# OChicken/GPQHE

Hardware: AMD Instinct MI355X
Metric: ciphertext he_mul/sec (RNS core: tensor 30 limbs + key-switch 45 limbs), N=2^16 (higher is better)
Workload: dtype u64; 1 GPU; he_mul RNS core, n=2^16, dimA=30, dimB=45, batch=64 ciphertexts per GPU (BASELINE configs[2]); he_rescale has no RNS-domain work in the reference; batch_per_gpu=64, total_batch=64, chunk=32, parallelism=ciphertext-per-GPU x1, no data-path collective, launcher=single process

## Files before the change

gpqhe_amd/_native.py:

```python
import ctypes as C
import os

_HERE = os.path.dirname(os.path.abspath(__file__))
LIB_PATH = os.path.join(_HERE, "libgpqhe_hip.so")


def use_variant(path):
    global LIB_PATH
    if _lib is not None:
        raise RuntimeError("use_variant(%r): the library is already loaded" % path)
    if not os.path.exists(path):
        raise FileNotFoundError(path)
    LIB_PATH = os.path.abspath(path)


u64 = C.c_uint64
vp = C.c_void_p

SIGNATURES = {
    "gpq_ctx_create": (C.c_int, [C.POINTER(vp), C.c_uint, C.c_uint, C.c_int]),
    "gpq_ctx_create_from_tables": (C.c_int, [C.POINTER(vp), C.c_uint, C.c_uint, C.POINTER(u64),
                                             C.POINTER(C.POINTER(u64)), C.POINTER(C.POINTER(u64)), C.c_int]),
    "gpq_ctx_destroy": (None, [vp]),
    "gpq_ctx_logn": (C.c_uint, [vp]),
    "gpq_ctx_nprimes": (C.c_uint, [vp]),
    "gpq_ctx_device": (C.c_int, [vp]),
    "gpq_ctx_const": (u64, [vp, C.c_uint, C.c_int]),
    "gpq_ctx_zetas": (C.POINTER(u64), [vp, C.c_uint, C.c_int]),
    "gpq_dimub": (C.c_uint, [C.c_uint, C.c_uint]),
    "gpq_last_error": (C.c_char_p, []),
    "gpq_malloc": (C.c_int, [C.POINTER(vp), C.c_size_t]),
    "gpq_free": (C.c_int, [vp]),
    "gpq_upload": (C.c_int, [vp, vp, C.c_size_t, vp]),
    "gpq_download": (C.c_int, [vp, vp, C.c_size_t, vp]),
    "gpq_copy": (C.c_int, [vp, vp, C.c_size_t, vp]),
    "gpq_stream_sync": (C.c_int, [vp]),
    "gpq_stream_wait": (C.c_int, [vp, vp]),
    "gpq_device_count": (C.c_int, []),
    "gpq_bind_thread_to_device": (C.c_int, [C.c_int]),
    "gpq_device_local_cpus": (C.c_int, [C.c_int, C.c_char_p, C.c_char_p, C.c_size_t]),
    "gpq_probe_stream": (C.c_int, [vp, vp, C.c_size_t, C.c_int, C.c_uint, C.c_uint, C.c_uint, vp]),
    "gpq_set_device": (C.c_int, [C.c_int]),
    "gpq_stream_create": (C.c_int, [C.POINTER(vp)]),
    "gpq_stream_destroy": (C.c_int, [vp]),
    "gpq_malloc_host": (C.c_int, [C.POINTER(vp), C.c_size_t]),
    "gpq_free_host": (C.c_int, [vp]),
    "gpq_ntt": (C.c_int, [vp, vp, C.c_uint, C.c_uint, vp]),
    "gpq_invntt": (C.c_int, [vp, vp, C.c_uint, C.c_uint, vp]),
    "gpq_ntt_reference": (C.c_int, [vp, vp, C.c_uint, C.c_uint, C.c_int, vp]),
    "gpq_rns_mul": (C.c_int, [vp, vp, vp, vp, C.c_uint, C.c_uint, vp]),
    "gpq_rns_add": (C.c_int, [vp, vp, vp, vp, C.c_uint, C.c_uint, vp]),
    "gpq_poly_mul_rns": (C.c_int, [vp, vp, vp, vp, C.c_uint, C.c_uint, vp]),
    "gpq_mulpt_rns": (C.c_int, [vp] * 6 + [C.c_uint, C.c_uint, vp]),
    "gpq_set_chunk": (C.c_int, [vp, C.c_uint]),
    "gpq_set_limb_block": (C.c_int, [vp, C.c_uint]),
    "gpq_set_limb_classes": (C.c_int, [vp, C.c_uint, C.c_uint]),
    "gpq_tensor_workspace_bytes": (C.c_size_t, [vp, C.c_uint, C.c_uint]),
    "gpq_keyswitch_workspace_bytes": (C.c_size_t, [vp, C.c_uint, C.c_uint]),
    "gpq_he_mul_tensor": (C.c_int, [vp] * 8 + [C.c_uint, C.c_uint, vp, vp]),
    "gpq_keyswitch": (C.c_int, [vp] * 6 + [C.c_uint, C.c_uint, vp, vp]),
    "gpq_big_words": (C.c_uint, [C.c_uint]),
    "gpq_ctx_phat_invmp": (u64, [vp, C.c_uint, C.c_uint]),
    "gpq_ctx_pbits": (C.c_uint, [vp, C.c_uint]),
    "gpq_rns_decompose": (C.c_int, [vp, vp, vp, C.c_uint, C.c_uint, C.c_uint, vp]),
    "gpq_rns_decompose_limbs": (C.c_int, [vp, vp, vp, C.c_uint, C.c_uint, C.c_uint, C.c_uint, vp]),
    "gpq_rns_reconstruct": (C.c_int, [vp, vp, C.c_uint, vp, C.c_uint, C.c_uint, C.c_uint, vp]),
    "gpq_rns_reconstruct_one": (C.c_int, [vp, C.POINTER(u64), C.c_uint, C.POINTER(u64), C.c_uint]),
    "gpq_set_exact_crt": (C.c_int, [vp, C.c_int]),
    "gpq_set_stream_bridge": (C.c_int, [vp, C.c_int]),
    "gpq_debug_force_redo": (C.c_int, [vp, C.c_uint]),
    "gpq_debug_zero_watch": (C.c_int, [vp, C.c_int]),
    "gpq_debug_zero_flags": (C.c_long, [vp, vp, vp, C.c_size_t]),
    "gpq_set_lazy_decompose": (C.c_int, [vp, C.c_int]),
    "gpq_set_nt_policy": (C.c_int, [vp, C.c_int]),
    "gpq_set_overlap": (C.c_int, [vp, C.c_int]),
    "gpq_last_lanes": (C.c_uint, [vp]),
    "gpq_debug_fail_peer": (C.c_int, [vp, C.c_int]),
    "gpq_debug_table_bytes": (C.c_size_t, [vp, C.c_int]),
    "gpq_set_fused_tail": (C.c_int, [vp, C.c_int]),
    "gpq_big_transpose": (C.c_int, [vp, vp, vp, C.c_uint, C.c_uint, C.c_int, vp]),
    "gpq_big_addsub": (C.c_int, [vp, vp, vp, vp, C.c_uint, C.c_uint, C.c_int, vp]),
    "gpq_set_prescale": (C.c_int, [vp, C.c_int]),
    "gpq_set_bridge_mfma": (C.c_int, [vp, C.c_int]),
    "gpq_poly_mul_workspace_bytes": (C.c_size_t, [vp, C.c_uint, C.c_uint]),
    "gpq_poly_mul": (C.c_int, [vp, vp, vp, vp, C.c_uint, C.c_uint, C.c_uint, C.c_uint, vp, vp]),
    "gpq_poly_mul_general_workspace_bytes": (C.c_size_t, [vp, C.c_uint, C.c_uint]),
    "gpq_rns_reconstruct_general": (C.c_int, [vp, vp, C.c_uint, vp, C.c_uint, C.c_uint, C.POINTER(u64), C.c_uint, vp, vp]),
    "gpq_poly_mul_general": (C.c_int, [vp, vp, vp, vp, C.c_uint, C.c_uint, C.POINTER(u64), C.c_uint, C.c_uint, vp, vp]),
    "gpq_he_rs": (C.c_int, [vp, vp, vp, C.c_uint, C.c_uint, C.c_uint, C.c_uint, vp]),
    "gpq_he_rescale": (C.c_int, [vp, vp, vp, C.c_uint, C.c_uint, C.c_uint, C.c_uint, vp]),
    "gpq_he_dims": (C.c_int, [vp, C.c_uint, C.c_uint] + [C.POINTER(C.c_uint)] * 4),
    "gpq_he_mul_workspace_bytes": (C.c_size_t, [vp, C.c_uint, C.c_uint, C.c_uint, C.c_uint, C.c_uint]),
    "gpq_he_mul": (C.c_int, [vp] * 9 + [C.c_uint] * 6 + [vp, vp]),
    "gpq_he_mul_rs": (C.c_int, [vp] * 9 + [C.c_uint] * 7 + [vp, vp]),
    "gpq_relin_tail_workspace_bytes": (C.c_size_t, [vp, C.c_uint, C.c_uint, C.c_uint, C.c_uint]),
    "gpq_relin_tail": (C.c_int, [vp, vp, vp, vp, C.c_uint, C.c_uint, C.c_uint, C.c_uint, C.c_uint, vp, vp]),
    "gpq_relin_tail_overwriting": (C.c_int, [vp, vp, vp, vp, C.c_uint, C.c_uint, C.c_uint, C.c_uint, C.c_uint, vp, vp]),
    "gpq_he_mulpt_workspace_bytes": (C.c_size_t, [vp, C.c_uint, C.c_uint]),
    "gpq_he_mulpt": (C.c_int, [vp] * 6 + [C.c_uint] * 4 + [vp, vp]),
    "gpq_poly_rot": (C.c_int, [vp, vp, vp, C.c_uint, C.c_uint, C.c_uint, vp]),
    "gpq_poly_conj": (C.c_int, [vp, vp, vp, C.c_uint, C.c_uint, vp]),
    "gpq_he_general_workspace_bytes": (C.c_size_t, [vp, C.c_uint, C.c_uint, C.c_uint, C.c_uint, C.c_uint]),
    "gpq_he_rs_general": (C.c_int, [vp, vp, vp, C.c_uint, C.c_ulonglong, C.POINTER(u64), C.c_uint, C.c_uint, vp, vp]),
    "gpq_relin_tail_general": (C.c_int, [vp, vp, vp, vp, C.c_uint, C.POINTER(u64), C.c_uint, C.c_uint, C.c_uint, C.c_uint, vp, vp]),
    "gpq_he_mul_general": (C.c_int, [vp] * 9 + [C.c_uint, C.POINTER(u64), C.c_uint, C.c_uint, C.c_uint, C.c_uint, C.c_uint, vp, vp]),
    "gpq_he_mulpt_general": (C.c_int, [vp] * 6 + [C.c_uint, C.POINTER(u64), C.c_uint, C.c_uint, C.c_uint, vp, vp]),
    "gpq_he_swk_general": (C.c_int, [vp] * 7 + [C.c_uint, C.POINTER(u64), C.c_uint, C.c_uint, C.c_uint, C.c_uint, vp, vp]),
    "gpq_big_add": (C.c_int, [vp, vp, vp, vp, C.c_uint, C.c_uint, C.c_uint, vp]),
    "gpq_big_sub": (C.c_int, [vp, vp, vp, vp, C.c_uint, C.c_uint, C.c_uint, vp]),
    "gpq_big_neg": (C.c_int, [vp, vp, vp, C.c_uint, C.c_uint, C.c_uint, vp]),
    "gpq_evk_pack": (C.c_int, [vp, vp, vp, C.c_uint, C.c_uint, C.c_uint, vp]),
    "gpq_he_genswk_workspace_bytes": (C.c_size_t, [vp, C.c_uint, C.c_uint, C.c_uint]),
    "gpq_he_genswk": (C.c_int, [vp] * 7 + [C.c_uint] * 4 + [vp, vp]),
    "gpq_he_swk_workspace_bytes": (C.c_size_t, [vp, C.c_uint, C.c_uint, C.c_uint, C.c_uint]),
    "gpq_he_swk": (C.c_int, [vp] * 7 + [C.c_uint] * 5 + [vp, vp]),
    "gpq_automorphism_index": (C.c_int, [C.c_uint, u64, vp]),
    "gpq_he_rot_hoisted_workspace_bytes": (C.c_size_t, [vp] + [C.c_uint] * 5),
    "gpq_he_rot_hoisted": (C.c_int, [vp] * 8 + [C.c_uint] * 6 + [vp, vp]),
    "gpq_he_gemv_workspace_bytes": (C.c_size_t, [vp] + [C.c_uint] * 6),
    "gpq_he_gemv": (C.c_int, [vp] * 8 + [C.c_uint] * 8 + [vp, vp]),
    "gpq_gemv_acc_dim": (C.c_uint, [C.c_uint] * 4),
    "gpq_gemv_plan_create": (C.c_int, [vp, C.POINTER(vp), vp, C.c_uint, C.c_uint, C.c_uint, C.c_uint, vp]),
    "gpq_gemv_plan_destroy": (None, [vp]),
    "gpq_gemv_plan_info": (C.c_int, [vp, C.POINTER(C.c_uint), C.POINTER(C.c_size_t), C.POINTER(C.c_uint), C.POINTER(C.c_int)]),
    "gpq_gemv_plan_rotations": (C.c_int, [vp, vp]),
    "gpq_shim_gemv_plan_cache": (None, [C.c_uint]),
    "gpq_gemv_inner_workspace_bytes": (C.c_size_t, [vp, vp, C.c_uint]),
    "gpq_gemv_inner": (C.c_int, [vp] * 6 + [C.c_uint] * 3 + [vp, vp]),
    "gpq_he_gemv_planned_workspace_bytes": (C.c_size_t, [vp, vp] + [C.c_uint] * 4),
    "gpq_he_gemv_planned": (C.c_int, [vp] * 8 + [C.c_uint] * 5 + [vp, vp]),
    "gpq_profile_enable": (C.c_int, [vp, C.c_int]),
    "gpq_profile_kernels": (C.c_int, []),
    "gpq_profile_kernel_name": (C.c_char_p, [C.c_int]),
    "gpq_profile_collect": (C.c_int, [vp, C.POINTER(C.c_double), C.POINTER(C.c_ulonglong)]),
    "gpq_timer_create": (C.c_int, [C.POINTER(vp)]),
    "gpq_timer_start": (C.c_int, [vp, vp]),
    "gpq_timer_stop": (C.c_int, [vp, vp]),
    "gpq_timer_elapsed_ms": (C.c_int, [vp, C.POINTER(C.c_float)]),
    "gpq_timer_destroy": (None, [vp]),
    "ntt": (None, [vp, vp]),
    "invntt": (None, [vp, vp]),
    "poly_ntt": (None, [vp, vp]),
    "poly_invntt": (None, [vp, vp]),
    "poly_rns_add": (None, [vp, vp, vp, vp]),
    "poly_rns_mul": (None, [vp, vp, vp, vp]),
    "montgomery_inv": (u64, [u64]),
    "barrett_inv": (u64, [u64]),
    "gpq_dropin_set_logn": (None, [C.c_uint]),
    "gpq_dropin_reset": (None, []),
    "gpq_mpi_shim_release": (None, []),
    "gpq_mpi_shim_forget_keys": (None, []),
    "gpq_mpi_shim_set_key_slots": (None, [C.c_uint]),
    "gpq_mpi_shim_set_key_check": (None, [C.c_int]),
    "gpq_mpi_shim_engine": (C.c_void_p, []),
    "gpq_compat_view": (C.c_void_p, [C.c_char_p]),
    "gpq_mpi_shim_resident_keys": (C.c_uint, []),
    "gpq_mpi_shim_set_poly_slots": (None, [C.c_uint]),
    "gpq_mpi_shim_resident_polys": (C.c_uint, []),
    "gpq_mpi_shim_poly_stats": (None, [C.POINTER(C.c_uint64), C.POINTER(C.c_uint64)]),
    "gpq_mpi_shim_forget_polys": (None, []),
    "gpq_mpi_shim_set_conversion_threads": (C.c_uint, [C.c_uint]),
    "gpq_mpi_shim_poly_bypass": (None, [C.c_int]),
    "gpq_mpi_shim_set_direct_mpi": (C.c_int, [C.c_int]),
    "gpq_mpi_shim_last_timing": (None, [C.POINTER(C.c_double)]),
    "gpq_fill_rns_chain": (C.c_int, [vp, C.c_uint, vp, C.c_int]),
    "gpq_release_rns_chain": (None, [vp]),
}
EXPORTED_ONLY = ["montgomery_reduce", "barrett_reduce",
                 "rns_decompose", "rns_reconstruct", "poly_rns2mpi", "poly_mul", "he_mul", "he_rs", "he_rescale", "he_moddown", "he_mulpt", "he_add", "he_sub", "he_addpt", "he_subpt", "he_neg", "he_copy_ct", "he_dec", "he_conj", "he_rot", "he_genrlk", "he_genck", "he_genrk",
                 "he_gemv", "he_sum", "he_idx",
                 ]
CTX_LIB_PATH = os.path.join(os.path.dirname(os.path.abspath(__file__)), "libgpqhe_hip_ctx.so")
CTX_EXPORTS = ["polyctx_init", "polyctx_exit", "hectx_init", "hectx_exit", "poly_mpi_alloc", "poly_mpi_free", "poly_rns_alloc", "poly_rns_free",
               "polyctx", "hectx", "GPQHE_TWO"]

_lib = None


def load():
    global _lib
    if _lib is not None:
        return _lib
    if not os.path.exists(LIB_PATH):
        raise ImportError(
            "gpqhe_amd: %s is missing -- build it with `make -C gpqhe_amd/csrc` "
            "(or __graft_entry__.build()); there is no CPU fallback" % LIB_PATH)
    try:
        import torch
    except ImportError:
        pass
    lib = C.CDLL(LIB_PATH)
    for name, (res, args) in SIGNATURES.items():
        fn = getattr(lib, name)
        fn.restype = res
        fn.argtypes = args
    for name in EXPORTED_ONLY:
        getattr(lib, name)
    _lib = lib
    return lib


class GpqError(RuntimeError):
    pass


def check(rc, what):
    if rc != 0:
        raise GpqError("%s failed (%d): %s" % (what, rc, load().gpq_last_error().decode()))
```

gpqhe_amd/csrc/bridge.hip:

```cpp
#include "../../include/gpqhe_hip.h"
#include "engine_internal.hpp"
#include "bridge_kernels.hpp"
#include "bridge_mfma.hpp"
#include "bridge_stream.hpp"

#include <algorithm>
#include <cstdlib>
#include <cstring>
#include <memory>
#include <new>

using namespace gpq;

#define HIP_TRY(expr)                                                                      \
  do {                                                                                     \
    hipError_t e_ = (expr);                                                                \
    if (e_ != hipSuccess) return gpq_fail(GPQ_ERR_HIP, "%s: %s", #expr, hipGetErrorString(e_)); \
  } while (0)

namespace {

typedef unsigned __int128 u128h;
typedef std::vector<uint64_t> Big;

struct LdsRaised {
  bool dev[64] = {};
  int raise(const void *fn, int bytes) {
    int d = 0;
    HIP_TRY(hipGetDevice(&d));
    if (d < 0 || d >= 64 || !dev[d]) {
      HIP_TRY(hipFuncSetAttribute(fn, hipFuncAttributeMaxDynamicSharedMemorySize, bytes));
      if (d >= 0 && d < 64) dev[d] = true;
    }
    return GPQ_OK;
  }
};


void mul_small(Big &a, uint64_t m) {
  uint64_t carry = 0;
  for (auto &w : a) { u128h t = (u128h)w * m + carry; w = (uint64_t)t; carry = (uint64_t)(t >> 64); }
  if (carry) a.push_back(carry);
}
uint64_t divmod_small(Big &a, uint64_t m) {
  uint64_t rem = 0;
  for (size_t i = a.size(); i-- > 0;) { u128h t = ((u128h)rem << 64) | a[i]; a[i] = (uint64_t)(t / m); rem = (uint64_t)(t % m); }
  while (a.size() > 1 && a.back() == 0) a.pop_back();
  return rem;
}
uint64_t mod_small(const Big &a, uint64_t m) { Big t = a; return divmod_small(t, m); }
void shr1(Big &a) {
  for (size_t i = 0; i < a.size(); ++i) a[i] = (a[i] >> 1) | (i + 1 < a.size() ? a[i + 1] << 63 : 0);
}
uint64_t powm(uint64_t b, uint64_t e, uint64_t m) {
  uint64_t r = 1;
  while (e) { if (e & 1) r = (uint64_t)((u128h)r * b % m); b = (uint64_t)((u128h)b * b % m); e >>= 1; }
  return r;
}
void put(std::vector<uint64_t> &dst, size_t off, const Big &v, size_t words) {
  for (size_t j = 0; j < words; ++j) dst[off + j] = j < v.size() ? v[j] : 0;
}

const int kWP[] = {8, 16, 32, 48, 56};

int cmp_big(const Big &a, const Big &b) {
  size_t na = a.size(), nb = b.size();
  while (na > 1 && a[na - 1] == 0) --na;
  while (nb > 1 && b[nb - 1] == 0) --nb;
  if (na != nb) return na < nb ? -1 : 1;
  for (size_t i = na; i-- > 0;) if (a[i] != b[i]) return a[i] < b[i] ? -1 : 1;
  return 0;
}
void sub_big(Big &a, const Big &b) {
  uint64_t bor = 0;
  for (size_t i = 0; i < a.size(); ++i) {
    const u128h d = (u128h)a[i] - (i < b.size() ? b[i] : 0) - bor;
    a[i] = (uint64_t)d; bor = (uint64_t)(d >> 64) & 1;
  }
}
Big floor_pow2_div(unsigned bits, const Big &m) {
  Big q((bits + 64) / 64, 0), rem(m.size() + 1, 0);
  for (int b = (int)bits; b >= 0; --b) {
    uint64_t c = b == (int)bits ? 1 : 0;
    for (size_t i = 0; i < rem.size(); ++i) { const uint64_t n = rem[i] >> 63; rem[i] = (rem[i] << 1) | c; c = n; }
    if (cmp_big(rem, m) >= 0) { sub_big(rem, m); q[b >> 6] |= 1ull << (b & 63); }
  }
  return q;
}

int get_basis(gpq_ctx *c, unsigned first, unsigned dim, gpq_bridge_basis **out) {
  const auto key = std::make_pair(first, dim);
  auto it = c->cache->bases.find(key);
  if (it != c->cache->bases.end()) { *out = &it->second; return GPQ_OK; }
  if (dim < 1 || first + dim > c->nprimes || dim > 63)
    return gpq_fail(GPQ_ERR_INVALID, "bridge: limbs %u..%u outside the chain of %u (at most 63 per basis)", first, first + dim, c->nprimes);
  Big P{1};
  for (unsigned d = 0; d < dim; ++d) mul_small(P, c->p[first + d]);
  int WP = 0;
  for (int w : kWP) if ((size_t)w >= P.size()) { WP = w; break; }
  if (!WP) return gpq_fail(GPQ_ERR_UNSUPPORTED, "bridge: P of %u limbs needs %zu words", dim, P.size());
  gpq_bridge_basis b;
  b.first = first; b.dim = dim; b.WP = WP; b.pbits = 64 * (unsigned)(P.size() - 1) + (64 - __builtin_clzll(P.back()));
  std::vector<uint64_t> phat((size_t)dim * WP), pinv(dim), pmult((size_t)6 * (WP + 1)), phalf(WP + 1);
  for (unsigned d = 0; d < dim; ++d) {
    const uint64_t pd = c->p[first + d];
    Big q = P;
    divmod_small(q, pd);
    put(phat, (size_t)d * WP, q, WP);
    pinv[d] = powm(mod_small(q, pd), pd - 2, pd);
  }
  Big h = P; shr1(h);
  put(phalf, 0, h, WP + 1);
  Big m = P;
  for (int k = 5; k >= 0; --k) { put(pmult, (size_t)k * (WP + 1), m, WP + 1); mul_small(m, 2); }
  DeviceScope on_device(c->device);
  HIP_TRY(gpq_table_malloc(c, (void **)&b.d_phat, phat.size() * 8));
  HIP_TRY(gpq_table_malloc(c, (void **)&b.d_phat_inv, pinv.size() * 8));
  HIP_TRY(gpq_table_malloc(c, (void **)&b.d_pmult, pmult.size() * 8));
  HIP_TRY(gpq_table_malloc(c, (void **)&b.d_phalf, phalf.size() * 8));
  HIP_TRY(hipMemcpy(b.d_phat, phat.data(), phat.size() * 8, hipMemcpyHostToDevice));
  HIP_TRY(hipMemcpy(b.d_phat_inv, pinv.data(), pinv.size() * 8, hipMemcpyHostToDevice));
  HIP_TRY(hipMemcpy(b.d_pmult, pmult.data(), pmult.size() * 8, hipMemcpyHostToDevice));
  HIP_TRY(hipMemcpy(b.d_phalf, phalf.data(), phalf.size() * 8, hipMemcpyHostToDevice));
  std::vector<uint64_t> inv128(2 * (size_t)dim);
  for (unsigned d = 0; d < dim; ++d) {
    const u128h q = ~(u128h)0 / c->p[first + d];
    inv128[2 * d] = (uint64_t)q; inv128[2 * d + 1] = (uint64_t)(q >> 64);
  }
  HIP_TRY(gpq_table_malloc(c, (void **)&b.d_inv128, inv128.size() * 8));
  HIP_TRY(hipMemcpy(b.d_inv128, inv128.data(), inv128.size() * 8, hipMemcpyHostToDevice));
  b.h_phat_inv = pinv;
  b.h_P = P;
  b.h_phat = phat;
  *out = &(c->cache->bases[key] = b);
  return GPQ_OK;
}

int get_relin(gpq_ctx *c, unsigned dimP, unsigned dimB, gpq_relin_tables **out) {
  const auto key = std::make_pair(dimP, dimB);
  auto it = c->cache->relins.find(key);
  if (it != c->cache->relins.end()) { *out = &it->second; return GPQ_OK; }
  gpq_bridge_basis *bp;
  int rc = get_basis(c, 0, dimP, &bp);
  if (rc) return rc;
  std::vector<uint64_t> pinv(dimB - dimP);
  for (unsigned d = dimP; d < dimB; ++d) pinv[d - dimP] = powm(mod_small(bp->h_P, c->p[d]), c->p[d] - 2, c->p[d]);
  gpq_relin_tables t;
  HIP_TRY(gpq_table_malloc(c, (void **)&t.d_pinv, pinv.size() * 8));
  HIP_TRY(hipMemcpy(t.d_pinv, pinv.data(), pinv.size() * 8, hipMemcpyHostToDevice));
  *out = &(c->cache->relins[key] = t);
  return GPQ_OK;
}

int get_scaled_tabs(gpq_ctx *c, gpq_bridge_basis *b, const LimbTab **out) {
  if (!b->d_tabs_scaled) {
    std::vector<LimbTab> t = c->h_tabs;
    auto pair_of = [](uint64_t w, uint64_t p) { return TwS{p - w, p - (uint64_t)(((u128h)w << 31) % p)}; };
    for (unsigned d = 0; d < b->dim; ++d) {
      LimbTab &e = t[b->first + d];
      const uint64_t p = e.k.p, s = b->h_phat_inv[d];
      e.ninv = (uint64_t)((u128h)e.ninv * s % p);
      e.winv1_ninv = (uint64_t)((u128h)e.winv1_ninv * s % p);
      if (b->first + d < c->nsplit_tables) { e.ninv_s = pair_of(e.ninv, p); e.winv1_ninv_s = pair_of(e.winv1_ninv, p); }
    }
    DeviceScope on_device(c->device);
    HIP_TRY(gpq_table_malloc(c, (void **)&b->d_tabs_scaled, t.size() * sizeof(LimbTab)));
    HIP_TRY(hipMemcpy(b->d_tabs_scaled, t.data(), t.size() * sizeof(LimbTab), hipMemcpyHostToDevice));
  }
  *out = b->d_tabs_scaled;
  return GPQ_OK;
}
struct ScaledInverse {
  gpq_ctx *c;
  ScaledInverse(gpq_ctx *ctx, const LimbTab *tabs) : c(ctx) { c->inv_tabs_override = tabs; }
  ~ScaledInverse() { c->inv_tabs_override = nullptr; }
};
inline bool can_prescale(const gpq_ctx *c) { return c->prescale && c->logn > 12 && !c->h_tabs.empty(); }

inline dim3 masked_grid(const FlagScope &sc, unsigned threads, unsigned n, unsigned polys) {
  if (sc.wave_any) return dim3((sc.waves + threads / 64 - 1) / (threads / 64));
  return dim3((n + threads - 1) / threads, polys);
}
template <int WP>
void launch_exact(const ReconstructArgs &a, unsigned n, unsigned batch, hipStream_t s) {
  hipLaunchKernelGGL((bridge_reconstruct<WP>), masked_grid(a.scope, 128, n, batch), dim3(128), 0, s, a);
}
template <int WL>
void launch_low(const ReconstructArgs &a, unsigned WPstride, unsigned char *redo, unsigned n, unsigned batch, hipStream_t s) {
  hipLaunchKernelGGL((bridge_reconstruct_low<WL>), dim3((n + 255) / 256, batch), dim3(256), 0, s, a, WPstride, redo);
}

void balanced_digits(const uint64_t *words, size_t nwords, int8_t *out, size_t nd) {
  unsigned carry = 0;
  for (size_t i = 0; i < nd; ++i) {
    const unsigned byte = i / 8 < nwords ? (unsigned)((words[i / 8] >> (8 * (i % 8))) & 0xff) : 0;
    const unsigned t = byte + carry;
    if (t >= 128) { out[i] = (int8_t)((int)t - 256); carry = 1; } else { out[i] = (int8_t)t; carry = 0; }
  }
}

int build_recon_mfma(gpq_ctx *c, const std::vector<uint64_t> &primes, const std::vector<uint64_t> &weight_inv, const std::vector<Big> &weight,
                     const Big &Pw, int WL, gpq_recon_mfma *tp, unsigned KSpad = 0, unsigned fcol0 = 0) {
  gpq_recon_mfma &t = *tp;
  const unsigned dim = (unsigned)primes.size(), NT = (8 * WL + 14 + 31) / 32, ncol = 32 * NT;
  t.KS = std::max((dim + 3) / 4, KSpad);
  if (!fcol0) fcol0 = 8u * WL;
  t.lds_bytes = (size_t)t.KS * NT * 1024 + (size_t)t.KS * 64;
  if (t.lds_bytes <= 156 * 1024) {
    std::vector<int8_t> bf((size_t)t.KS * NT * 1024, 0);
    std::vector<uint64_t> lk((size_t)t.KS * 8, 0), kc(WL + 2, 0), pm((size_t)65 * WL, 0);
    std::vector<int8_t> beta(8 * (size_t)WL), phi(8);
    Big sum_phat(WL, 0);
    u128h sum_inv = 0;
    for (unsigned d = 0; d < dim; ++d) {
      const uint64_t pd = primes[d];
      lk[2 * (size_t)d] = pd;
      lk[2 * (size_t)d + 1] = weight_inv[d];
      const Big &ph = weight[d];
      balanced_digits(ph.data(), ph.size() < (size_t)WL ? ph.size() : (size_t)WL, beta.data(), beta.size());
      const uint64_t inv = (uint64_t)((((u128h)1) << 104) / pd);
      balanced_digits(&inv, 1, phi.data(), 8);
      uint64_t cy = 0;
      for (int j = 0; j < WL; ++j) {
        const u128h s2 = (u128h)sum_phat[j] + ((size_t)j < ph.size() ? ph[j] : 0) + cy;
        sum_phat[j] = (uint64_t)s2; cy = (uint64_t)(s2 >> 64);
      }
      sum_inv += inv;
      for (unsigned i = 0; i < 8; ++i) {
        const unsigned k = 8 * d + i, s = k / 32, h = (k % 32) / 16, tt = k % 16;
        for (unsigned col = 0; col < ncol; ++col) {
          int8_t v = 0;
          if (col < 8u * WL) { if (col >= i) v = beta[col - i]; }
          else if (col >= fcol0) { const unsigned m = col - fcol0; if (m >= i && m - i < 8 && m < 14) v = phi[m - i]; }
          if (!v) continue;
          const unsigned nt = col / 32, lane = 32 * h + col % 32;
          bf[(((size_t)s * NT + nt) * 64 + lane) * 16 + tt] = v;
        }
      }
    }
    Big kcS = sum_phat;
    mul_small(kcS, 0x8080808080808080ull);
    for (int j = 0; j < WL; ++j) kc[j] = (size_t)j < kcS.size() ? kcS[j] : 0;
    const u128h lo = (u128h)(uint64_t)sum_inv * 0x8080808080808080ull;
    const u128h hi = (u128h)(uint64_t)(sum_inv >> 64) * 0x8080808080808080ull;
    const u128h kf = lo + (hi << 64);
    kc[WL] = (uint64_t)kf; kc[WL + 1] = (uint64_t)(kf >> 64);
    Big mP{0};
    for (unsigned m = 0; m <= 64; ++m) {
      uint64_t bw = 0;
      for (int j = 0; j < WL; ++j) {
        const u128h d2 = (u128h)((size_t)j < mP.size() ? mP[j] : 0) - kc[j] - bw;
        pm[(size_t)m * WL + j] = (uint64_t)d2; bw = (uint64_t)(d2 >> 64) & 1;
      }
      Big nxt(std::max(mP.size(), Pw.size()) + 1, 0);
      uint64_t cy = 0;
      for (size_t j = 0; j < nxt.size(); ++j) {
        const u128h s2 = (u128h)(j < mP.size() ? mP[j] : 0) + (j < Pw.size() ? Pw[j] : 0) + cy;
        nxt[j] = (uint64_t)s2; cy = (uint64_t)(s2 >> 64);
      }
      mP = nxt;
    }
    DeviceScope on_device(c->device);
    HIP_TRY(gpq_table_malloc(c, (void **)&t.d_bfrag, bf.size()));
    HIP_TRY(gpq_table_malloc(c, (void **)&t.d_lk, lk.size() * 8));
    HIP_TRY(gpq_table_malloc(c, (void **)&t.d_kc, kc.size() * 8));
    HIP_TRY(gpq_table_malloc(c, (void **)&t.d_pm, pm.size() * 8));
    HIP_TRY(hipMemcpy(t.d_bfrag, bf.data(), bf.size(), hipMemcpyHostToDevice));
    HIP_TRY(hipMemcpy(t.d_lk, lk.data(), lk.size() * 8, hipMemcpyHostToDevice));
    HIP_TRY(hipMemcpy(t.d_kc, kc.data(), kc.size() * 8, hipMemcpyHostToDevice));
    HIP_TRY(hipMemcpy(t.d_pm, pm.data(), pm.size() * 8, hipMemcpyHostToDevice));
  }
  return GPQ_OK;
}

int get_recon_mfma(gpq_ctx *c, gpq_bridge_basis *b, int WL, gpq_recon_mfma **out, unsigned KSpad = 0) {
  if (KSpad <= (b->dim + 3) / 4) KSpad = 0;
  const int key = WL + 1000 * (int)KSpad;
  auto it = b->mfma.find(key);
  if (it != b->mfma.end()) { *out = &it->second; return GPQ_OK; }
  gpq_recon_mfma t;
  std::vector<uint64_t> primes(b->dim);
  std::vector<Big> weight(b->dim);
  for (unsigned d = 0; d < b->dim; ++d) {
    primes[d] = c->p[b->first + d];
    weight[d].assign(b->h_phat.begin() + (size_t)d * b->WP, b->h_phat.begin() + (size_t)(d + 1) * b->WP);
  }
  if (int rc = build_recon_mfma(c, primes, b->h_phat_inv, weight, b->h_P, WL, &t, KSpad)) return rc;
  *out = &(b->mfma[key] = t);
  return GPQ_OK;
}

int get_addend_rows(gpq_ctx *c, gpq_bridge_basis *b, unsigned KSpad, gpq_recon_mfma **out) {
  const int key = 100016 + 1000 * (int)KSpad;
  auto it = b->mfma.find(key);
  if (it != b->mfma.end()) { *out = &it->second; return GPQ_OK; }
  auto shifted = [](const Big &v) {
    Big r = v;
    r.insert(r.begin(), 0);
    mul_small(r, 1ull << 40);
    return r;
  };
  std::vector<uint64_t> primes(b->dim);
  std::vector<Big> weight(b->dim);
  for (unsigned d = 0; d < b->dim; ++d) {
    primes[d] = c->p[b->first + d];
    weight[d] = shifted(Big(b->h_phat.begin() + (size_t)d * b->WP, b->h_phat.begin() + (size_t)(d + 1) * b->WP));
    weight[d].resize(weight[d].size() < 16 ? 16 : weight[d].size(), 0);
  }
  gpq_recon_mfma t;
  if (int rc = build_recon_mfma(c, primes, b->h_phat_inv, weight, shifted(b->h_P), 16, &t, KSpad, 144)) return rc;
  *out = &(b->mfma[key] = t);
  return GPQ_OK;
}

template <int WL>
int launch_low_mfma(const ReconMfmaArgs &a, size_t lds, hipStream_t s);
int launch_low_mfma16(const ReconMfmaArgs &a, size_t lds, hipStream_t s) { return launch_low_mfma<16>(a, lds, s); }
template <int WL>
int launch_low_mfma(const ReconMfmaArgs &a, size_t lds, hipStream_t s) {
  static LdsRaised raised;
  if (int rc = raised.raise(reinterpret_cast<const void *>(&bridge_reconstruct_low_mfma<WL>), 156 * 1024)) return rc;
  unsigned blocks = 256;
  if (blocks > (a.total_groups + 7) / 8) blocks = (a.total_groups + 7) / 8;
  hipLaunchKernelGGL((bridge_reconstruct_low_mfma<WL>), dim3(blocks), dim3(512), lds, s, a);
  return GPQ_OK;
}

// ... 409 lines not shown
}

extern "C" int gpq_rns_decompose_limbs(gpq_ctx *c, uint64_t *slab, const uint64_t *big, unsigned W, unsigned first, unsigned count,
                                       unsigned batch, void *stream) {
  int rc = check(c, count, batch, "gpq_rns_decompose_limbs");
  if (rc) return rc;
  if (!slab || !big || W < 1 || first + count > c->nprimes) return gpq_fail(GPQ_ERR_INVALID, "gpq_rns_decompose_limbs: bad arguments");
  if ((rc = launch_decompose(c, slab, big, W, first, count, batch, (hipStream_t)stream))) return rc;
  return launched("gpq_rns_decompose_limbs");
}

extern "C" size_t gpq_poly_mul_workspace_bytes(const gpq_ctx *c, unsigned dim, unsigned batch) {
  return 3ull * batch * ((size_t)dim << c->logn) * 8;
}

extern "C" int gpq_poly_mul(gpq_ctx *c, uint64_t *r, const uint64_t *a, const uint64_t *b, unsigned W, unsigned dim, unsigned logq,
                            unsigned batch, void *workspace, void *stream) {
  int rc = check(c, dim, batch, "gpq_poly_mul");
  if (rc) return rc;
  if (!r || !a || !b || !workspace || !logq) return gpq_fail(GPQ_ERR_INVALID, "gpq_poly_mul: bad arguments (q must be 2^logq, logq > 0)");
  const size_t poly = (size_t)dim << c->logn;
  uint64_t *sa = (uint64_t *)workspace, *sb = sa + batch * poly, *sr = sb + batch * poly;
  if ((rc = gpq_rns_decompose(c, sa, a, W, dim, batch, stream))) return rc;
  if ((rc = gpq_rns_decompose(c, sb, b, W, dim, batch, stream))) return rc;
  if ((rc = gpq_poly_mul_rns(c, sr, sa, sb, dim, batch, stream))) return rc;
  return gpq_rns_reconstruct(c, r, W, sr, dim, batch, logq, stream);
}

extern "C" int gpq_he_rs(gpq_ctx *c, uint64_t *c0, uint64_t *c1, unsigned W, unsigned logDelta, unsigned logql, unsigned batch, void *stream) {
  if (!c || !c0 || !c1 || W < 1 || batch < 1 || logql < 1 || logql > 64 * W)
    return gpq_fail(GPQ_ERR_INVALID, "gpq_he_rs: bad arguments");
  const dim3 grid((c->n + 255) / 256, batch), block(256);
  for (uint64_t *p : {c0, c1}) {
    RescaleArgs a{p, W, c->logn, logDelta, logql};
    ProfScope prof(c, GPQ_K_RESCALE, (hipStream_t)stream);
    hipLaunchKernelGGL(bridge_rescale, grid, block, 0, (hipStream_t)stream, a);
  }
  return launched("gpq_he_rs");
}
extern "C" int gpq_he_rescale(gpq_ctx *c, uint64_t *c0, uint64_t *c1, unsigned W, unsigned logDelta, unsigned logql, unsigned batch, void *stream) {
  return gpq_he_rs(c, c0, c1, W, logDelta, logql, batch, stream);
}

namespace {

struct TailPlan { unsigned Wr, cnt; size_t words, bytes; };

int tail_plan(gpq_ctx *c, unsigned W, unsigned dimP, unsigned dimB, unsigned polys, TailPlan *p) {
  gpq_bridge_basis *bp;
  int rc = get_basis(c, 0, dimP, &bp);
  if (rc) return rc;
  if (dimB <= dimP) return gpq_fail(GPQ_ERR_INVALID, "relin: dimB=%u must exceed dimP=%u", dimB, dimP);
  p->Wr = bp->pbits / 64 + 1;
  p->cnt = dimB - dimP;
  p->words = (size_t)polys * ((size_t)(p->Wr + 2 * p->cnt + W) << c->logn);
  p->bytes = p->words * 8 + ((size_t)polys << c->logn);
  return GPQ_OK;
}

int get_relin_front(gpq_ctx *c, unsigned dimP, unsigned dimB, gpq_relin_tables *rt, gpq_bridge_basis *bp, gpq_bridge_basis *bq) {
  if (rt->front_tried) return GPQ_OK;
  rt->front_tried = true;
  const unsigned cnt = dimB - dimP;
  if (dimP < 4 || dimP > 32 || cnt < 4 || bp->pbits < 160) return GPQ_OK;
  const unsigned KS = dimP <= 8 ? 2 : dimP <= 16 ? 4 : 8, NTp = (cnt + 3) / 4, NT = NTp + 1;
  const size_t lds = (size_t)NT * KS * 1024 + (size_t)(8 * KS + 12 * NTp) * 8;
  if (lds > kMfmaLdsMax) return GPQ_OK;
  std::vector<int8_t> bf((size_t)NT * KS * 1024, 0);
  std::vector<uint64_t> lk((size_t)8 * KS, 0), pk((size_t)12 * NTp, 0), tkp((size_t)cnt * 64, 0), kf(2, 0);
  std::vector<int8_t> bfw;
  std::vector<uint64_t> pkw((size_t)12 * NTp, 0), tkpw((size_t)cnt * 64, 0), wscale(cnt, 1);
  u128h sum_inv = 0;
  for (unsigned d = 0; d < dimP; ++d) {
    const uint64_t pd = c->p[d];
    lk[2 * (size_t)d] = pd;
    lk[2 * (size_t)d + 1] = bp->h_phat_inv[d];
    const uint64_t inv = (uint64_t)((((u128h)1) << 104) / pd);
    sum_inv += inv;
    int8_t phi[8];
    balanced_digits(&inv, 1, phi, 8);
    for (unsigned i = 0; i < 8; ++i) {
      const unsigned k = 8 * d + i, s = k / 32, h = (k % 32) / 16, tt = k % 16;
      for (unsigned m = i; m < 14 && m - i < 8; ++m)
        bf[(((size_t)(NT - 1) * KS + s) * 64 + 32 * h + m) * 16 + tt] = phi[m - i];
    }
  }
  const u128h kfv = (u128h)(uint64_t)sum_inv * 0x8080808080808080ull;
  kf[0] = (uint64_t)kfv; kf[1] = (uint64_t)(kfv >> 64);
  bfw = bf;
  for (int scaled = 0; scaled < 2; ++scaled) {
    std::vector<int8_t> &B = scaled ? bfw : bf;
    std::vector<uint64_t> &PK = scaled ? pkw : pk, &TK = scaled ? tkpw : tkp;
    for (unsigned j = 0; j < cnt; ++j) {
      const uint64_t pj = c->p[dimP + j];
      const uint64_t Pm0 = mod_small(bp->h_P, pj);
      const uint64_t Pinv = powm(Pm0, pj - 2, pj);
      const uint64_t wj = (uint64_t)((u128h)Pinv * bq->h_phat_inv[j] % pj);
      const uint64_t mulw = scaled ? wj : 1;
      const uint64_t Pm = (uint64_t)((u128h)Pm0 * mulw % pj);
      wscale[j] = wj;
      uint64_t sum_ph = 0;
      const unsigned nt = j / 4, pq = j % 4;
      for (unsigned d = 0; d < dimP; ++d) {
        Big ph(bp->h_phat.begin() + (size_t)d * bp->WP, bp->h_phat.begin() + (size_t)(d + 1) * bp->WP);
        uint64_t T = (uint64_t)((u128h)mod_small(ph, pj) * mulw % pj);
        sum_ph = (uint64_t)(((u128h)sum_ph + T) % pj);
        for (unsigned i = 0; i < 8; ++i) {
          int8_t dig[8];
          balanced8(T, dig);
          const unsigned k = 8 * d + i, s = k / 32, h = (k % 32) / 16, tt = k % 16;
          for (unsigned b = 0; b < 8; ++b) B[(((size_t)nt * KS + s) * 64 + 32 * h + 8 * pq + b) * 16 + tt] = dig[b];
          T = (uint64_t)(((u128h)T << 8) % pj);
        }
      }
      const uint64_t K = (uint64_t)((u128h)(0x8080808080808080ull % pj) * sum_ph % pj);
      const uint64_t off = 1ull << 50;
      PK[3 * (size_t)j] = pj;
      PK[3 * (size_t)j + 1] = off + (K + pj - off % pj) % pj;
      PK[3 * (size_t)j + 2] = wj;
      for (unsigned k = 0; k < 64; ++k) TK[(size_t)j * 64 + k] = (pj - (uint64_t)((u128h)k * Pm % pj)) % pj;
    }
  }
  std::vector<LimbTab> tw = c->h_tabs;
  if (!tw.empty()) {
    auto pair_of = [](uint64_t w, uint64_t p) { return TwS{p - w, p - (uint64_t)(((u128h)w << 31) % p)}; };
    for (unsigned d = 0; d < dimB; ++d) {
      LimbTab &e = tw[d];
      const uint64_t p = e.k.p, sc = d < dimP ? bp->h_phat_inv[d] : wscale[d - dimP];
      e.ninv = (uint64_t)((u128h)e.ninv * sc % p);
      e.winv1_ninv = (uint64_t)((u128h)e.winv1_ninv * sc % p);
      if (d < c->nsplit_tables) { e.ninv_s = pair_of(e.ninv, p); e.winv1_ninv_s = pair_of(e.winv1_ninv, p); }
    }
  }
  DeviceScope on_device(c->device);
  HIP_TRY(gpq_table_malloc(c, (void **)&rt->d_bfrag, bf.size()));
  HIP_TRY(gpq_table_malloc(c, (void **)&rt->d_lk, lk.size() * 8));
  HIP_TRY(gpq_table_malloc(c, (void **)&rt->d_pk, pk.size() * 8));
  HIP_TRY(gpq_table_malloc(c, (void **)&rt->d_tkp, tkp.size() * 8));
  HIP_TRY(gpq_table_malloc(c, (void **)&rt->d_kf, kf.size() * 8));
  HIP_TRY(hipMemcpy(rt->d_bfrag, bf.data(), bf.size(), hipMemcpyHostToDevice));
  HIP_TRY(hipMemcpy(rt->d_lk, lk.data(), lk.size() * 8, hipMemcpyHostToDevice));
  HIP_TRY(hipMemcpy(rt->d_pk, pk.data(), pk.size() * 8, hipMemcpyHostToDevice));
  HIP_TRY(hipMemcpy(rt->d_tkp, tkp.data(), tkp.size() * 8, hipMemcpyHostToDevice));
  HIP_TRY(hipMemcpy(rt->d_kf, kf.data(), kf.size() * 8, hipMemcpyHostToDevice));
  if (!tw.empty()) {
    HIP_TRY(gpq_table_malloc(c, (void **)&rt->d_bfrag_w, bfw.size()));
    HIP_TRY(gpq_table_malloc(c, (void **)&rt->d_pk_w, pkw.size() * 8));
    HIP_TRY(gpq_table_malloc(c, (void **)&rt->d_tkp_w, tkpw.size() * 8));
    HIP_TRY(gpq_table_malloc(c, (void **)&rt->d_tabs_w, tw.size() * sizeof(LimbTab)));
    HIP_TRY(hipMemcpy(rt->d_bfrag_w, bfw.data(), bfw.size(), hipMemcpyHostToDevice));
    HIP_TRY(hipMemcpy(rt->d_pk_w, pkw.data(), pkw.size() * 8, hipMemcpyHostToDevice));
    HIP_TRY(hipMemcpy(rt->d_tkp_w, tkpw.data(), tkpw.size() * 8, hipMemcpyHostToDevice));
    HIP_TRY(hipMemcpy(rt->d_tabs_w, tw.data(), tw.size() * sizeof(LimbTab), hipMemcpyHostToDevice));
  }
  rt->NT = NT; rt->KS = KS; rt->lds_bytes = lds;
  return GPQ_OK;
}

int get_tail_direct(gpq_ctx *c, unsigned dimP, unsigned dimB, gpq_relin_tables *rt) {
  if (rt->direct_tried) return GPQ_OK;
  rt->direct_tried = true;
  gpq_bridge_basis *bB, *bq;
  int rc;
  if (dimB > 60 || dimB - dimP < 4) return GPQ_OK;
  if ((rc = get_basis(c, 0, dimB, &bB)) || (rc = get_basis(c, dimP, dimB - dimP, &bq))) return rc;
  if (c->h_tabs.empty()) return GPQ_OK;
  constexpr int WL = 16;
  Big num = bq->h_P;
  num.insert(num.begin(), 0);
  mul_small(num, 1ull << 40);
  std::vector<uint64_t> primes(dimB), scale(dimB), unscale(dimB);
  std::vector<Big> weight(dimB);
  for (unsigned d = 0; d < dimB; ++d) {
    primes[d] = c->p[d];
    Big q = num;
    (void)divmod_small(q, primes[d]);
    q.resize(WL < (int)q.size() ? q.size() : WL, 0);
    weight[d] = q;
    scale[d] = bB->h_phat_inv[d];
    Big ph(bB->h_phat.begin() + (size_t)d * bB->WP, bB->h_phat.begin() + (size_t)(d + 1) * bB->WP);
    unscale[d] = mod_small(ph, primes[d]);
  }
  if ((rc = build_recon_mfma(c, primes, scale, weight, num, WL, &rt->direct))) return rc;
  if (!rt->direct.d_bfrag) return GPQ_OK;
  const LimbTab *tabs;
  if ((rc = get_scaled_tabs(c, bB, &tabs))) return rc;
  rt->d_tabs_direct = tabs;
  DeviceScope on_device(c->device);
  HIP_TRY(gpq_table_malloc(c, (void **)&rt->d_scale, dimB * 8));
  HIP_TRY(gpq_table_malloc(c, (void **)&rt->d_unscale, dimB * 8));
  HIP_TRY(hipMemcpy(rt->d_scale, scale.data(), dimB * 8, hipMemcpyHostToDevice));
  HIP_TRY(hipMemcpy(rt->d_unscale, unscale.data(), dimB * 8, hipMemcpyHostToDevice));
  return GPQ_OK;
}

int tail_prescale_mode(gpq_ctx *c, unsigned dimP, unsigned dimB, const LimbTab **tabs, int *mode) {
  *tabs = nullptr; *mode = 0;
  if (!can_prescale(c)) return GPQ_OK;
  gpq_bridge_basis *bp, *bq;
  gpq_relin_tables *rt;
  int rc;
  if ((rc = get_basis(c, 0, dimP, &bp)) || (rc = get_basis(c, dimP, dimB - dimP, &bq)) || (rc = get_relin(c, dimP, dimB, &rt))) return rc;
  if (c->bridge_mfma && c->logn >= 6 && (rc = get_relin_front(c, dimP, dimB, rt, bp, bq))) return rc;
  if (c->bridge_mfma && c->logn >= 6 && rt->d_bfrag && c->tail_direct && !c->exact_crt && !c->fuse_tail) {
    if ((rc = get_tail_direct(c, dimP, dimB, rt))) return rc;
    if (rt->direct.d_bfrag && rt->d_tabs_direct) { *tabs = rt->d_tabs_direct; *mode = 3; return GPQ_OK; }
  }
  if (c->bridge_mfma && c->logn >= 6 && rt->d_bfrag && rt->d_tabs_w && c->prescale_upper) { *tabs = rt->d_tabs_w; *mode = 2; return GPQ_OK; }
  *mode = 1;
  return get_scaled_tabs(c, bp, tabs);
}

template <int KS, int WL>
int launch_relin_tail_t(const RelinTailArgs &a, size_t lds, hipStream_t s) {
  static LdsRaised raised;
  if (int rc = raised.raise(reinterpret_cast<const void *>(&bridge_relin_tail_mfma<KS, WL>), (int)kMfmaLdsMax)) return rc;
  unsigned blocks = 256 * GPQ_TAIL_WAVES;
  if (blocks > (a.f.total_groups + 3) / 4) blocks = (a.f.total_groups + 3) / 4;
  hipLaunchKernelGGL((bridge_relin_tail_mfma<KS, WL>), dim3(blocks), dim3(256), lds, s, a);
  return GPQ_OK;
}

template <int KS>
int launch_relin_front_t(const RelinFrontArgs &a, size_t lds, hipStream_t s) {
  static LdsRaised raised;
  if (int rc = raised.raise(reinterpret_cast<const void *>(&bridge_relin_front_mfma<KS>), (int)kMfmaLdsMax)) return rc;
  unsigned per_cu = (unsigned)((160 * 1024) / lds);
  if (per_cu > 3) per_cu = 3;
  if (per_cu < 1) per_cu = 1;
  unsigned blocks = 256 * per_cu;
  if (blocks > (a.total_groups + 3) / 4) blocks = (a.total_groups + 3) / 4;
  if (a.scope.wave_any) blocks = (a.scope.waves + 3) / 4;
  hipLaunchKernelGGL((bridge_relin_front_mfma<KS>), dim3(blocks), dim3(256), lds, s, a);
  return GPQ_OK;
}
int launch_relin_front(const gpq_ctx *c, unsigned KS, const RelinFrontArgs &f, size_t lds, hipStream_t s) {
  ProfScope prof(c, f.only ? GPQ_K_BRIDGE_EXACT : GPQ_K_RELIN_FRONT, s);
  switch (KS) {
    case 2: return launch_relin_front_t<2>(f, lds, s);
    case 4: return launch_relin_front_t<4>(f, lds, s);
    default: return launch_relin_front_t<8>(f, lds, s);
  }
}

struct TailD { const uint64_t *hat; gpq_bridge_basis *bA; unsigned dimA; uint64_t *scratch; };

template <int KST, int KSD, bool DCRT, int R>
int launch_tail_stream_t(const TailStreamArgs &a, size_t lds, unsigned blocks, hipStream_t s) {
  static LdsRaised raised;
  if (int rc = raised.raise(reinterpret_cast<const void *>(&bridge_tail_stream<KST, KSD, DCRT, R>), (int)kStreamLdsMax)) return rc;
  hipLaunchKernelGGL((bridge_tail_stream<KST, KSD, DCRT, R>), dim3(blocks), dim3(512), lds, s, a);
  return GPQ_OK;
}

int get_tail_direct_padded(gpq_ctx *c, unsigned dimP, unsigned dimB, gpq_relin_tables *rt, unsigned KST, gpq_recon_mfma **out) {
  if (KST <= (dimB + 3) / 4) { *out = &rt->direct; return GPQ_OK; }
  auto it = rt->direct_padded.find(KST);
  if (it != rt->direct_padded.end()) { *out = &it->second; return GPQ_OK; }
  gpq_bridge_basis *bB, *bq;
  int rc;
  if ((rc = get_basis(c, 0, dimB, &bB)) || (rc = get_basis(c, dimP, dimB - dimP, &bq))) return rc;
  Big num = bq->h_P;
  num.insert(num.begin(), 0);
  mul_small(num, 1ull << 40);
  std::vector<uint64_t> primes(dimB), scale(dimB);
  std::vector<Big> weight(dimB);
  for (unsigned d = 0; d < dimB; ++d) {
    primes[d] = c->p[d];
    Big q = num;
    (void)divmod_small(q, primes[d]);
    q.resize(16 < q.size() ? q.size() : 16, 0);
    weight[d] = q;
    scale[d] = bB->h_phat_inv[d];
  }
  gpq_recon_mfma t;
  if ((rc = build_recon_mfma(c, primes, scale, weight, num, 16, &t, KST))) return rc;
  *out = &(rt->direct_padded[KST] = t);
  return GPQ_OK;
}

int tail_stream(gpq_ctx *c, gpq_relin_tables *rt, Two<uint64_t> out, const uint64_t *chat, Two<const uint64_t> dbig, const TailD *dh, unsigned W,
                unsigned dimP, unsigned dimB, unsigned logql, unsigned polys, unsigned char *tie, unsigned char *amb, hipStream_t s, FlagScope *scope, bool *done,
                unsigned rs = 0) {
  *done = false;
  const unsigned need = (logql + 63) / 64;
  if (!c->stream_bridge || W > 14 || W < need || logql > 896) return GPQ_OK;
  int KST, KSD = 0;
  if (dh) {
    if (!stream_fast_ok(c, dh->bA, logql)) return GPQ_OK;
    if (dimB <= 32 && dh->dimA <= 16) { KST = 8; KSD = 4; }
    else if (dimB <= 48 && dh->dimA <= 32) { KST = 12; KSD = 8; }
    else return GPQ_OK;
  } else {
    if (dimB <= 24) KST = 6; else if (dimB <= 48) KST = 12; else return GPQ_OK;
  }
  gpq_recon_mfma *tt, *td = nullptr;
  int rc;
  if ((rc = get_tail_direct_padded(c, dimP, dimB, rt, KST, &tt))) return rc;
  if (dh && (rc = get_addend_rows(c, dh->bA, KSD, &td))) return rc;
  if (!tt->d_bfrag || tt->KS != (unsigned)KST || (dh && (!td->d_bfrag || td->KS != (unsigned)KSD))) return GPQ_OK;
  const size_t lds = (size_t)(KST + KSD) * 5 * 1024 + (size_t)2 * 65 * kTailRow * 8;
  if (lds > kStreamLdsMax) return GPQ_OK;
  if ((rc = ensure_redo(c, (size_t)polys << c->logn, s)) || (rc = ensure_wave_any(c, s))) return rc;
  const unsigned groups = (c->n >> 6) * polys, blocks = stream_blocks(groups);
  const size_t chat_bytes = ((size_t)polys * dimB << c->logn) * 8, dhat_bytes = dh ? ((size_t)polys * dh->dimA << c->logn) * 8 : 0;
  if (chat_bytes >= 0xfffff000ull || dhat_bytes >= 0xfffff000ull) return GPQ_OK;
// ... 1002 lines not shown
```

gpqhe_amd/csrc/engine.hip:

```cpp
#include "../../include/gpqhe_hip.h"
#include "engine_internal.hpp"
#include "ntt_kernels.hpp"

#include <cmath>
#include <cstdlib>
#include <cstdarg>
#include <cstdio>
#include <cstring>
#include <new>
#include <type_traits>

using namespace gpq;

static thread_local char g_err[512] = "";

int gpq_fail(int code, const char *fmt, ...) {
  va_list ap;
  va_start(ap, fmt);
  vsnprintf(g_err, sizeof g_err, fmt, ap);
  va_end(ap);
  return code;
}
extern "C" const char *gpq_last_error(void) { return g_err; }

#include <dlfcn.h>
#include <atomic>
namespace {
typedef int (*roctx_push_t)(const char *);
typedef int (*roctx_pop_t)(void);
std::atomic<int> g_roctx_state{0};
roctx_push_t g_roctx_push = nullptr;
roctx_pop_t g_roctx_pop = nullptr;
bool roctx_ready() {
  int st = g_roctx_state.load(std::memory_order_acquire);
  if (st == 0) {
    void *h = RTLD_DEFAULT;
    void *push = dlsym(h, "roctxRangePushA");
    for (const char *lib : {"librocprofiler-sdk-roctx.so.1", "libroctx64.so.4"}) {
      if (push) break;
      if ((h = dlopen(lib, RTLD_NOW | RTLD_NOLOAD))) push = dlsym(h, "roctxRangePushA");
    }
    if (push) {
      g_roctx_push = (roctx_push_t)push;
      g_roctx_pop = (roctx_pop_t)dlsym(h, "roctxRangePop");
    }
    st = (g_roctx_push && g_roctx_pop) ? 1 : 2;
    g_roctx_state.store(st, std::memory_order_release);
  }
  return st == 1;
}
}
void gpq_range_push(const char *name) { if (roctx_ready()) (void)g_roctx_push(name); }
void gpq_range_pop() { if (roctx_ready()) (void)g_roctx_pop(); }

#define HIP_TRY(expr)                                                                      \
  do {                                                                                     \
    hipError_t e_ = (expr);                                                                \
    if (e_ != hipSuccess) return gpq_fail(GPQ_ERR_HIP, "%s: %s", #expr, hipGetErrorString(e_)); \
  } while (0)

constexpr unsigned kMaxPolysPerLaunch = 16384;

namespace {

typedef unsigned __int128 u128h;

inline uint64_t mulm(uint64_t a, uint64_t b, uint64_t m) { return (uint64_t)((u128h)a * b % m); }

uint64_t powm(uint64_t b, uint64_t e, uint64_t m) {
  uint64_t r = 1 % m;
  b %= m;
  while (e) {
    if (e & 1) r = mulm(r, b, m);
    b = mulm(b, b, m);
    e >>= 1;
  }
  return r;
}

bool is_prime_u64(uint64_t n) {
  if (n < 2) return false;
  for (uint64_t sp : {2ull, 3ull, 5ull, 7ull, 11ull, 13ull}) {
    if (n % sp == 0) return n == sp;
  }
  uint64_t d = n - 1;
  int s = __builtin_ctzll(d);
  d >>= s;
  for (uint64_t a : {2ull, 325ull, 9375ull, 28178ull, 450775ull, 9780504ull, 1795265022ull}) {
    uint64_t x = powm(a, d, n);
    if (x == 0 || x == 1 || x == n - 1) continue;
    bool witness = true;
    for (int r = 1; r < s && witness; ++r) {
      x = mulm(x, x, n);
      if (x == n - 1) witness = false;
    }
    if (witness) return false;
  }
  return true;
}

std::vector<uint64_t> prime_factors(uint64_t m) {
  std::vector<uint64_t> f;
  auto strip = [&](uint64_t d) {
    if (m % d == 0) {
      f.push_back(d);
      while (m % d == 0) m /= d;
    }
  };
  strip(2);
  strip(3);
  for (uint64_t d = 5; d * d <= m; d += 6) {
    strip(d);
    strip(d + 2);
  }
  if (m > 1) f.push_back(m);
  return f;
}

uint64_t least_generator(uint64_t p) {
  const std::vector<uint64_t> f = prime_factors(p - 1);
  for (uint64_t g = 2; g < p; ++g) {
    bool ok = true;
    for (uint64_t q : f)
      if (powm(g, (p - 1) / q, p) == 1) { ok = false; break; }
    if (ok) return g;
  }
  return 0;
}

inline uint32_t bitrev(uint32_t v, unsigned bits) {
  return bits ? (__builtin_bitreverse32(v) >> (32 - bits)) : 0;
}

uint64_t inv_mod_2_64(uint64_t q) {
  uint64_t x = q;
  for (int i = 0; i < 6; ++i) x *= 2 - q * x;
  return x;
}

}

static int alloc_zero_flags(gpq_ctx *c);
static int upload_tables(gpq_ctx *c) {
  const size_t n = c->n, np = c->nprimes;
  int ndev = 0;
  HIP_TRY(hipGetDeviceCount(&ndev));
  if (c->device < 0 || c->device >= ndev) return gpq_fail(GPQ_ERR_INVALID, "device %d outside 0..%d", c->device, ndev - 1);
  DeviceScope on_device(c->device);
  if (!c->cache) c->cache = new (std::nothrow) gpq_table_cache();
  if (!c->cache) return gpq_fail(GPQ_ERR_NOMEM, "out of host memory");
  HIP_TRY(gpq_table_malloc(c, (void **)&c->d_w, np * n * sizeof(uint64_t)));
  HIP_TRY(gpq_table_malloc(c, (void **)&c->d_winv, np * n * sizeof(uint64_t)));
  HIP_TRY(gpq_table_malloc(c, (void **)&c->d_tabs, np * sizeof(LimbTab)));
  std::vector<uint64_t> wstd(np * n), wistd(np * n);
  std::vector<LimbTab> tabs(np);
  for (size_t d = 0; d < np; ++d) {
    const uint64_t p = c->p[d];
    if (p <= (1ull << 59) || p - (1ull << 59) >= GPQ_FOLD_CMAX)
      return gpq_fail(GPQ_ERR_UNSUPPORTED, "prime %llu is not 2^59 + c with c < %u", (unsigned long long)p, GPQ_FOLD_CMAX);
    const uint64_t pinv = c->pinv_mont[d];
    auto from_mont = [&](uint64_t z) {
      const uint64_t u = z * pinv;
      const uint64_t t = (uint64_t)(((u128h)u * p) >> 64);
      return t ? p - t : 0;
    };
    for (size_t i = 0; i < n; ++i) {
      wstd[d * n + i] = from_mont(c->zetas[d * n + i]);
      wistd[d * n + i] = from_mont(c->zetas_inv[d * n + i]);
    }
    LimbTab &t = tabs[d];
    t.k.p = p; t.k.p2 = 2 * p; t.k.p4 = 4 * p; t.k.c = (uint32_t)(p - (1ull << 59)); t.k.c1 = t.k.c + 1;
    t.k.kx0 = t.k.c1; t.k.kx1 = (uint64_t)t.k.c1 - 4 * p; t.k.ky = 4 * p - 2 * (uint64_t)t.k.c1;
    t.k.kys = 2 * p - 2 * (uint64_t)t.k.c1;
    t.k.p3 = 3 * p; t.k.np3 = (uint64_t)0 - 3 * p; t.k.kx1x = (uint64_t)t.k.c1 - 3 * p; t.k.kyx = 3 * p - 2 * (uint64_t)t.k.c1;
    t.k.np = (uint64_t)0 - p; t.k.np2 = (uint64_t)0 - 2 * p; t.k.np4 = (uint64_t)0 - 4 * p;
    t.ninv = from_mont(c->ninv_mont[d]);
    t.winv1_ninv = n >= 2 ? mulm(wistd[d * n + 1], t.ninv, p) : t.ninv;
    t.ninv_s = t.winv1_ninv_s = TwS{0, 0};
  }
  c->nsplit = 0;
  while (c->nsplit < np && c->p[c->nsplit] - (1ull << 59) < GPQ_SPLIT_CMAX) ++c->nsplit;
  c->nwide = 0;
  while (c->nwide < c->nsplit && c->p[c->nwide] - (1ull << 59) < GPQ_WIDE_CMAX) ++c->nwide;
  c->nsplit_tables = c->nsplit; c->nwide_max = c->nwide;
  c->low9 = c->logn == 17;
  if (c->nsplit) {
    const size_t ns = c->nsplit;
    std::vector<TwS> ws(ns * n), wis(ns * n);
    auto pair_of = [](uint64_t w, uint64_t p) { return TwS{p - w, p - (uint64_t)(((u128h)w << 31) % p)}; };
    for (size_t d = 0; d < ns; ++d) {
      const uint64_t p = c->p[d];
      for (size_t i = 0; i < n; ++i) {
        ws[d * n + i] = pair_of(wstd[d * n + i], p);
        wis[d * n + i] = pair_of(wistd[d * n + i], p);
      }
      tabs[d].ninv_s = pair_of(tabs[d].ninv, p);
      tabs[d].winv1_ninv_s = pair_of(tabs[d].winv1_ninv, p);
    }
    HIP_TRY(gpq_table_malloc(c, (void **)&c->d_ws, ns * n * sizeof(TwS)));
    HIP_TRY(gpq_table_malloc(c, (void **)&c->d_winvs, ns * n * sizeof(TwS)));
    HIP_TRY(hipMemcpy(c->d_ws, ws.data(), ns * n * sizeof(TwS), hipMemcpyHostToDevice));
    HIP_TRY(hipMemcpy(c->d_winvs, wis.data(), ns * n * sizeof(TwS), hipMemcpyHostToDevice));
  }
  HIP_TRY(hipMemcpy(c->d_w, wstd.data(), np * n * 8, hipMemcpyHostToDevice));
  HIP_TRY(hipMemcpy(c->d_winv, wistd.data(), np * n * 8, hipMemcpyHostToDevice));
  HIP_TRY(hipMemcpy(c->d_tabs, tabs.data(), np * sizeof(LimbTab), hipMemcpyHostToDevice));
  c->h_tabs = tabs;
  return alloc_zero_flags(c);
}

static int alloc_zero_flags(gpq_ctx *c) {
  DeviceScope on_device(c->device);
  HIP_TRY(hipMalloc((void **)&c->d_zflag, 4096 * sizeof(unsigned)));
  HIP_TRY(hipMemset(c->d_zflag, 0, 4096 * sizeof(unsigned)));
  HIP_TRY(hipStreamSynchronize(nullptr));
  c->zflag_cap = 4096;
  return GPQ_OK;
}

static void fill_scalar_constants(gpq_ctx *c, size_t d) {
  const uint64_t p = c->p[d];
  c->pinv_mont[d] = inv_mod_2_64(p);
  c->pinv_barr[d] = (uint64_t)(((u128h)1 << (2 * (64 - __builtin_clzll(p)))) / p);
  const uint64_t r_mod_p = (uint64_t)(((u128h)1 << 64) % p);
  c->ninv_mont[d] = mulm(powm(c->n, p - 2, p), r_mod_p, p);
}

extern "C" int gpq_ctx_create(gpq_ctx **out, unsigned logn, unsigned nprimes, int device) {
  if (!out || logn < 1 || logn > 17 || nprimes < 1 || nprimes > 4096)
    return gpq_fail(GPQ_ERR_INVALID, "gpq_ctx_create: logn=%u nprimes=%u out of range", logn, nprimes);
  gpq_ctx *c = new (std::nothrow) gpq_ctx();
  if (!c) return gpq_fail(GPQ_ERR_NOMEM, "out of host memory");
  c->device = device; c->logn = logn; c->n = 1u << logn; c->nprimes = nprimes;
  const size_t n = c->n;
  c->p.resize(nprimes); c->pinv_mont.resize(nprimes); c->pinv_barr.resize(nprimes);
  c->ninv_mont.resize(nprimes); c->psi.resize(nprimes);
  c->zetas.resize((size_t)nprimes * n); c->zetas_inv.resize((size_t)nprimes * n);
  uint64_t p = (1ull << 59) + 1;
  for (size_t d = 0; d < nprimes; ++d) {
    do p += 2 * n; while (!is_prime_u64(p));
    c->p[d] = p;
    fill_scalar_constants(c, d);
    const uint64_t psi = powm(least_generator(p), (p - 1) / (2 * n), p);
    const uint64_t psi_inv = powm(psi, p - 2, p);
    const uint64_t r_mod_p = (uint64_t)(((u128h)1 << 64) % p);
    c->psi[d] = psi;
    uint64_t pw = r_mod_p, pwi = r_mod_p;
    for (uint32_t i = 0; i < n; ++i) {
      const uint32_t j = bitrev(i, logn);
      c->zetas[d * n + j] = pw;
      c->zetas_inv[d * n + j] = pwi;
      pw = mulm(pw, psi, p);
      pwi = mulm(pwi, psi_inv, p);
    }
  }
  int rc = upload_tables(c);
  if (rc != GPQ_OK) { gpq_ctx_destroy(c); return rc; }
  *out = c;
  return GPQ_OK;
}

extern "C" int gpq_ctx_create_from_tables(gpq_ctx **out, unsigned logn, unsigned nprimes, const uint64_t *primes,
                                          const uint64_t *const *zetas_mont, const uint64_t *const *zetas_inv_mont,
                                          int device) {
  if (!out || !primes || !zetas_mont || !zetas_inv_mont || logn < 1 || logn > 17 || nprimes < 1)
    return gpq_fail(GPQ_ERR_INVALID, "gpq_ctx_create_from_tables: bad arguments");
  gpq_ctx *c = new (std::nothrow) gpq_ctx();
  if (!c) return gpq_fail(GPQ_ERR_NOMEM, "out of host memory");
  c->device = device; c->logn = logn; c->n = 1u << logn; c->nprimes = nprimes;
  const size_t n = c->n;
  c->p.assign(primes, primes + nprimes);
  c->pinv_mont.resize(nprimes); c->pinv_barr.resize(nprimes); c->ninv_mont.resize(nprimes); c->psi.assign(nprimes, 0);
  c->zetas.resize((size_t)nprimes * n); c->zetas_inv.resize((size_t)nprimes * n);
  for (size_t d = 0; d < nprimes; ++d) {
    if (!(c->p[d] & 1)) { delete c; return gpq_fail(GPQ_ERR_INVALID, "even modulus"); }
    fill_scalar_constants(c, d);
    memcpy(&c->zetas[d * n], zetas_mont[d], n * 8);
    memcpy(&c->zetas_inv[d * n], zetas_inv_mont[d], n * 8);
  }
  int rc = upload_tables(c);
  if (rc != GPQ_OK) { gpq_ctx_destroy(c); return rc; }
  *out = c;
  return GPQ_OK;
}

int gpq_ctx_clone(const gpq_ctx *c, gpq_ctx **out) {
  gpq_ctx *q = new (std::nothrow) gpq_ctx();
  if (!q) return gpq_fail(GPQ_ERR_NOMEM, "out of host memory");
  q->device = c->device; q->logn = c->logn; q->n = c->n; q->nprimes = c->nprimes;
  q->p = c->p; q->pinv_mont = c->pinv_mont; q->pinv_barr = c->pinv_barr; q->ninv_mont = c->ninv_mont; q->psi = c->psi;
  q->overlap = 0;
  q->tables_of = c;
  q->d_w = c->d_w; q->d_winv = c->d_winv; q->d_ws = c->d_ws; q->d_winvs = c->d_winvs; q->d_tabs = c->d_tabs;
  q->h_tabs = c->h_tabs;
  q->nsplit = c->nsplit; q->nsplit_tables = c->nsplit_tables; q->nwide = c->nwide; q->nwide_max = c->nwide_max; q->low9 = c->low9;
  q->cache = c->cache;
  int rc = alloc_zero_flags(q);
  if (rc != GPQ_OK) { gpq_ctx_destroy(q); return rc; }
  *out = q;
  return GPQ_OK;
}

extern "C" void gpq_ctx_destroy(gpq_ctx *c) {
  if (!c) return;
  if (c->peer) {
    if (c->peer_stream) (void)hipStreamSynchronize(c->peer_stream);
    gpq_ctx_destroy(c->peer);
  }
  if (c->peer_stream) (void)hipStreamDestroy(c->peer_stream);
  if (c->ev_fork) (void)hipEventDestroy(c->ev_fork);
  if (c->ev_join) (void)hipEventDestroy(c->ev_join);
  if (c->peer_ws) (void)hipFree(c->peer_ws);
  if (!c->tables_of) {
    if (c->d_w) (void)hipFree(c->d_w);
    if (c->d_winv) (void)hipFree(c->d_winv);
    if (c->d_ws) (void)hipFree(c->d_ws);
    if (c->d_winvs) (void)hipFree(c->d_winvs);
    if (c->d_tabs) (void)hipFree(c->d_tabs);
  }
  if (c->d_zflag) (void)hipFree(c->d_zflag);
  if (c->d_zwatch) (void)hipFree(c->d_zwatch);
  gpq_bridge_release(c);
  for (gpq_prof_rec &r : c->prof) { (void)hipEventDestroy(r.a); (void)hipEventDestroy(r.b); }
  for (hipEvent_t e : c->prof_pool) (void)hipEventDestroy(e);
  delete c;
}

extern "C" size_t gpq_debug_table_bytes(const gpq_ctx *c, int which) {
  if (!c) return 0;
  if (which == 0) return c->cache && !c->tables_of ? c->cache->device_bytes : 0;
  if (which == 1) return c->peer && !c->peer->tables_of && c->peer->cache ? c->peer->cache->device_bytes : 0;
  if (which == 2) return c->peer ? 1 : 0;
  if (which == 3) return c->peer ? (size_t)(c->peer->d_w == c->d_w && c->peer->d_winv == c->d_winv && c->peer->d_ws == c->d_ws && c->peer->d_winvs == c->d_winvs &&
                                            c->peer->d_tabs == c->d_tabs && c->peer->cache == c->cache) : 0;
  return 0;
}

extern "C" unsigned gpq_ctx_logn(const gpq_ctx *c) { return c->logn; }
extern "C" unsigned gpq_ctx_nprimes(const gpq_ctx *c) { return c->nprimes; }
extern "C" int gpq_ctx_device(const gpq_ctx *c) { return c->device; }
extern "C" uint64_t gpq_ctx_const(const gpq_ctx *c, unsigned d, int which) {
  if (d >= c->nprimes) return 0;
  switch (which) {
    case 0: return c->p[d];
    case 1: return c->pinv_mont[d];
    case 2: return c->pinv_barr[d];
    case 3: return c->ninv_mont[d];
    case 4: return c->psi[d];
  }
  return 0;
}
extern "C" const uint64_t *gpq_ctx_zetas(const gpq_ctx *c, unsigned d, int inverse) {
  if (d >= c->nprimes) return nullptr;
  return (inverse ? c->zetas_inv.data() : c->zetas.data()) + (size_t)d * c->n;
}
extern "C" unsigned gpq_dimub(unsigned logn, unsigned logq) { return (1 + logn + 4 * logq) / 59 + 1; }
// ... 517 lines not shown
  for (unsigned k0 = 0; k0 < batch; k0 += chunk) {
    const unsigned polys = (batch - k0 < chunk) ? batch - k0 : chunk;
    if (lane.c && ((k0 / chunk) & 1)) {
      const size_t o = k0 * poly;
      if ((rc = gpq_keyswitch(lane.c, c0 + o, c1 + o, x + o, evk0, evk1, dim, polys, lane.ws, lane.s))) return rc;
      continue;
    }
    for (unsigned l0 = 0; l0 < dim; l0 += lblock) {
      const unsigned limbs = dim - l0 < lblock ? dim - l0 : lblock;
      const size_t loff = (size_t)l0 << c->logn;
      StageRange stage("gpq_keyswitch: strided fwd / keyswitch_mid8x2 / strided inv x2");
      const unsigned nt = nt_for(c, polys, limbs, 3);
      PassArgs f = make_args(c, dim, 1, nt);
      f.limb0 = l0;
      f.src[0] = x + k0 * poly + loff; f.dst[0] = ws + loff;
      if ((rc = launch_strided<false>(c, f, limbs, polys, s))) return rc;
      KeyswitchArgs m;
      m.p = make_args(c, dim, 1, nt);
      m.p.limb0 = l0;
      m.p.src[0] = f.dst[0]; m.p.dst[0] = c0 + k0 * poly + loff; m.p.dst[1] = c1 + k0 * poly + loff;
      m.evk0 = evk0 + loff; m.evk1 = evk1 + loff;
      if ((rc = for_limb_ranges<true>(c, m.p, limbs, &m.evk0, &m.evk1, [&](auto tag, const PassArgs &a, unsigned nl) {
            using TW = decltype(tag);
            KeyswitchArgs ka{a, m.evk0, m.evk1};
            ProfScope prof(c, GPQ_K_KEYSWITCH_MID, s);
            const dim3 block(CONTIG_WAVES * 64);
            with_nt(a.nt, [&](auto nt) {
              constexpr bool NT = decltype(nt)::value;
              if (polys / 2) {
                if (c->low9) hipLaunchKernelGGL((keyswitch_mid8x2<TW, 9, true, NT>), dim3(c->n >> 11, polys / 2, nl), block, 0, s, ka, 0u);
                else hipLaunchKernelGGL((keyswitch_mid8x2<TW, 8, true, NT>), dim3(c->n >> 11, polys / 2, nl), block, 0, s, ka, 0u);
              }
              if (polys & 1) {
                if (c->low9) hipLaunchKernelGGL((keyswitch_mid8x2<TW, 9, false, NT>), dim3(c->n >> 11, 1, nl), block, 0, s, ka, polys - 1);
                else hipLaunchKernelGGL((keyswitch_mid8x2<TW, 8, false, NT>), dim3(c->n >> 11, 1, nl), block, 0, s, ka, polys - 1);
              }
            });
            return (int)GPQ_OK;
          }))) return rc;
      PassArgs b = make_args(c, dim, 2, nt);
      b.limb0 = l0;
      if (c->inv_tabs_override) b.tabs = c->inv_tabs_override;
      for (int i = 0; i < 2; ++i) { b.src[i] = m.p.dst[i]; b.dst[i] = m.p.dst[i]; }
      if ((rc = launch_strided<true>(c, b, limbs, polys, s))) return rc;
    }
  }
  const unsigned lanes_used = lane.c ? 2u : 1u;
  if ((rc = gpq_peer_join(c, s, lane))) return rc;
  c->last_lanes = lanes_used;
  return after_launch("gpq_keyswitch");
}

extern "C" int gpq_automorphism_index(unsigned logn, uint64_t g, uint32_t *idx) {
  if (logn < 1 || logn > 17 || !(g & 1) || !idx) return gpq_fail(GPQ_ERR_INVALID, "gpq_automorphism_index: logn in [1, 17], odd g, idx");
  const uint64_t n = 1ull << logn, m = 2 * n, gm = g & (m - 1);
  auto brv = [logn](uint64_t x) { uint64_t r = 0; for (unsigned b = 0; b < logn; ++b) r |= ((x >> b) & 1) << (logn - 1 - b); return r; };
  for (uint64_t j = 0; j < n; ++j) idx[j] = (uint32_t)brv((((2 * brv(j) + 1) * gm) & (m - 1)) >> 1);
  return GPQ_OK;
}

int gpq_hoist_forward(gpq_ctx *c, uint64_t *slab, unsigned dim, unsigned polys, hipStream_t s) {
  PassArgs a = make_args(c, dim, 1, nt_for(c, polys, dim, 1));
  a.src[0] = a.dst[0] = slab;
  int rc;
  if (!two_pass(c)) {
    for (unsigned k0 = 0; k0 < polys; k0 += kMaxPolysPerLaunch) {
      const unsigned cnt = polys - k0 < kMaxPolysPerLaunch ? polys - k0 : kMaxPolysPerLaunch;
      a.src[0] = a.dst[0] = slab + (size_t)k0 * ((size_t)dim << c->logn);
      if ((rc = launch_small<false>(c, a, dim, cnt, s))) return rc;
    }
    return after_launch("gpq_he_rot_hoisted: forward transform");
  }
  if ((rc = launch_strided<false>(c, a, dim, polys, s))) return rc;
  if ((rc = launch_contig<false>(c, a, dim, polys, s))) return rc;
  return after_launch("gpq_he_rot_hoisted: forward transform");
}

int gpq_keyswitch_rotated(gpq_ctx *c, uint64_t *c0, uint64_t *c1, const uint64_t *X, const uint64_t *evk0, const uint64_t *evk1,
                          unsigned dim, unsigned polys, unsigned g, void *workspace, hipStream_t s) {
  const size_t poly = (size_t)dim << c->logn;
  int rc;
  if (!two_pass(c)) {
    uint64_t *ws = (uint64_t *)workspace;
    const size_t rows = (size_t)polys * dim;
    for (size_t r0 = 0; r0 < rows; r0 += 65535) {
      const unsigned cnt = rows - r0 < 65535 ? (unsigned)(rows - r0) : 65535u;
      ProfScope prof(c, GPQ_K_AUTOMORPHISM_GATHER, s);
      hipLaunchKernelGGL(automorphism_gather, dim3((c->n + 255) / 256, cnt), dim3(256), 0, s, X + (r0 << c->logn), ws + (r0 << c->logn), c->logn, g);
    }
    for (unsigned k = 0; k < polys; ++k) {
      if ((rc = gpq_rns_mul(c, c0 + k * poly, ws + k * poly, evk0, dim, 1, s))) return rc;
      if ((rc = gpq_rns_mul(c, c1 + k * poly, ws + k * poly, evk1, dim, 1, s))) return rc;
    }
    if ((rc = gpq_invntt(c, c0, dim, polys, s))) return rc;
    return gpq_invntt(c, c1, dim, polys, s);
  }
  const unsigned nt = nt_for(c, polys, dim, 3);
  KeyswitchArgs m;
  m.p = make_args(c, dim, 1, nt);
  m.p.src[0] = X; m.p.dst[0] = c0; m.p.dst[1] = c1;
  m.evk0 = evk0; m.evk1 = evk1;
  if ((rc = for_limb_ranges<true>(c, m.p, dim, &m.evk0, &m.evk1, [&](auto tag, const PassArgs &a, unsigned nl) {
        using TW = decltype(tag);
        KeyswitchArgs ka{a, m.evk0, m.evk1};
        ProfScope prof(c, GPQ_K_KEYSWITCH_ROT_MID, s);
        const dim3 block(CONTIG_WAVES * 64);
        with_nt(a.nt, [&](auto ntv) {
          constexpr bool NT = decltype(ntv)::value;
          if (polys / 2) {
            if (c->low9) hipLaunchKernelGGL((keyswitch_rot_mid8x2<TW, 9, true, NT>), dim3(c->n >> 11, polys / 2, nl), block, 0, s, ka, 0u, g);
            else hipLaunchKernelGGL((keyswitch_rot_mid8x2<TW, 8, true, NT>), dim3(c->n >> 11, polys / 2, nl), block, 0, s, ka, 0u, g);
          }
          if (polys & 1) {
            if (c->low9) hipLaunchKernelGGL((keyswitch_rot_mid8x2<TW, 9, false, NT>), dim3(c->n >> 11, 1, nl), block, 0, s, ka, polys - 1, g);
            else hipLaunchKernelGGL((keyswitch_rot_mid8x2<TW, 8, false, NT>), dim3(c->n >> 11, 1, nl), block, 0, s, ka, polys - 1, g);
          }
        });
        return (int)GPQ_OK;
      }))) return rc;
  PassArgs b = make_args(c, dim, 2, nt);
  if (c->inv_tabs_override) b.tabs = c->inv_tabs_override;
  b.src[0] = b.dst[0] = c0; b.src[1] = b.dst[1] = c1;
  if ((rc = launch_strided<true>(c, b, dim, polys, s))) return rc;
  return after_launch("gpq_he_rot_hoisted: key switch");
}

int gpq_gemv_mac(gpq_ctx *c, uint64_t *acc0, uint64_t *acc1, const uint64_t *r0, const uint64_t *r1, const uint64_t *diag,
                 const void *terms, unsigned nterms, unsigned dim, unsigned polys, hipStream_t s) {
  constexpr int BT = 4;
  GemvMacArgs a{c->d_tabs, r0, r1, diag, acc0, acc1, (const uint2 *)terms, nterms, polys, dim, c->logn};
  const dim3 grid((polys + BT - 1) / BT, c->n >= 512 ? c->n / 512 : 1, dim);
  ProfScope prof(c, GPQ_K_GEMV_MAC, s);
  with_nt(nt_for(c, (size_t)polys * (nterms ? nterms : 1), dim, 2), [&](auto nt) {
    hipLaunchKernelGGL((gemv_mac<BT, decltype(nt)::value>), grid, dim3(256), 0, s, a);
  });
  return after_launch("gemv_mac");
}

extern "C" int gpq_set_nt_policy(gpq_ctx *c, int mode) {
  if (!c) return gpq_fail(GPQ_ERR_INVALID, "gpq_set_nt_policy: null context");
  if (mode < -1 || mode > 1) return gpq_fail(GPQ_ERR_INVALID, "gpq_set_nt_policy: mode %d (want -1 by working set, 0 never, 1 always)", mode);
  c->nt_mode = mode;
  return GPQ_OK;
}

extern "C" int gpq_set_limb_classes(gpq_ctx *c, unsigned wide, unsigned split) {
  if (!c) return gpq_fail(GPQ_ERR_INVALID, "gpq_set_limb_classes: null context");
  c->nsplit = split < c->nsplit_tables ? split : c->nsplit_tables;
  c->nwide = wide < c->nwide_max ? wide : c->nwide_max;
  if (c->nwide > c->nsplit) c->nwide = c->nsplit;
  return GPQ_OK;
}

extern "C" int gpq_set_limb_block(gpq_ctx *c, unsigned limbs) {
  if (!c) return gpq_fail(GPQ_ERR_INVALID, "gpq_set_limb_block: null context");
  c->limb_block = limbs;
  return GPQ_OK;
}

extern "C" int gpq_set_chunk(gpq_ctx *c, unsigned chunk) {
  if (!c || chunk < 1 || chunk > kMaxPolysPerLaunch) return gpq_fail(GPQ_ERR_INVALID, "gpq_set_chunk: bad arguments");
  c->chunk = chunk;
  return GPQ_OK;
}

extern "C" int gpq_profile_enable(gpq_ctx *c, int on) {
  if (!c) return gpq_fail(GPQ_ERR_INVALID, "gpq_profile_enable: null context");
  c->prof_on = on != 0;
  return GPQ_OK;
}
namespace {
typedef unsigned v4w __attribute__((ext_vector_type(4)));
template <int U, int KIND>
__global__ void probe_stream(v4w *__restrict__ dst, const v4w *__restrict__ src, size_t n16) {
  const size_t stride = (size_t)gridDim.x * blockDim.x;
  size_t i = (size_t)blockIdx.x * blockDim.x + threadIdx.x;
  v4w sink = v4w{0, 0, 0, 0};
  for (; i + (U - 1) * stride < n16; i += U * stride) {
    v4w v[U];
#pragma unroll
    for (int u = 0; u < U; ++u) v[u] = KIND == 2 ? v4w{(unsigned)i, 1u, 2u, 3u} : __builtin_nontemporal_load(&src[i + u * stride]);
#pragma unroll
    for (int u = 0; u < U; ++u) {
      if (KIND == 1) sink ^= v[u];
      else __builtin_nontemporal_store(v[u], &dst[i + u * stride]);
    }
  }
  for (; i < n16; i += stride) {
    if (KIND == 1) sink ^= src[i];
    else dst[i] = KIND == 2 ? v4w{(unsigned)i, 1u, 2u, 3u} : src[i];
  }
  if (KIND == 1 && (sink[0] ^ sink[1] ^ sink[2] ^ sink[3]) == 0x9e3779b9u) dst[0] = sink;
}
template <int KIND>
int launch_probe(void *dst, const void *src, size_t bytes, unsigned blocks, unsigned threads, unsigned unroll, hipStream_t s) {
  const size_t n16 = bytes / 16;
  switch (unroll) {
    case 1: hipLaunchKernelGGL((probe_stream<1, KIND>), dim3(blocks), dim3(threads), 0, s, (v4w *)dst, (const v4w *)src, n16); break;
    case 2: hipLaunchKernelGGL((probe_stream<2, KIND>), dim3(blocks), dim3(threads), 0, s, (v4w *)dst, (const v4w *)src, n16); break;
    case 4: hipLaunchKernelGGL((probe_stream<4, KIND>), dim3(blocks), dim3(threads), 0, s, (v4w *)dst, (const v4w *)src, n16); break;
    case 8: hipLaunchKernelGGL((probe_stream<8, KIND>), dim3(blocks), dim3(threads), 0, s, (v4w *)dst, (const v4w *)src, n16); break;
    default: return gpq_fail(GPQ_ERR_INVALID, "gpq_probe_stream: unroll must be 1, 2, 4 or 8");
  }
  return GPQ_OK;
}
}

extern "C" int gpq_probe_stream(void *dst, const void *src, size_t bytes, int kind, unsigned blocks, unsigned threads, unsigned unroll, void *stream) {
  if (!dst || !src || bytes < 16 || (bytes & 15) || blocks < 1 || threads < 64 || threads > 1024 || (threads & 63) || kind < 0 || kind > 2)
    return gpq_fail(GPQ_ERR_INVALID, "gpq_probe_stream: bad arguments");
  int rc = kind == 0 ? launch_probe<0>(dst, src, bytes, blocks, threads, unroll, (hipStream_t)stream)
         : kind == 1 ? launch_probe<1>(dst, src, bytes, blocks, threads, unroll, (hipStream_t)stream)
                     : launch_probe<2>(dst, src, bytes, blocks, threads, unroll, (hipStream_t)stream);
  if (rc) return rc;
  hipError_t e = hipGetLastError();
  return e == hipSuccess ? GPQ_OK : gpq_fail(GPQ_ERR_HIP, "gpq_probe_stream: launch failed: %s", hipGetErrorString(e));
}

extern "C" int gpq_profile_kernels(void) { return GPQ_K_COUNT; }
extern "C" const char *gpq_profile_kernel_name(int k) { return (k >= 0 && k < GPQ_K_COUNT) ? kKernelNames[k] : ""; }

extern "C" int gpq_profile_collect(gpq_ctx *c, double *total_ms, unsigned long long *launches) {
  if (!c || !total_ms || !launches) return gpq_fail(GPQ_ERR_INVALID, "gpq_profile_collect: bad arguments");
  for (int k = 0; k < GPQ_K_COUNT; ++k) { total_ms[k] = 0; launches[k] = 0; }
  for (gpq_prof_rec &r : c->prof) {
    float ms = 0;
    HIP_TRY(hipEventSynchronize(r.b));
    HIP_TRY(hipEventElapsedTime(&ms, r.a, r.b));
    total_ms[r.kernel] += ms;
    launches[r.kernel] += 1;
    c->prof_pool.push_back(r.a);
    c->prof_pool.push_back(r.b);
  }
  c->prof.clear();
  return GPQ_OK;
}

struct gpq_timer { hipEvent_t a, b; };

extern "C" int gpq_timer_create(gpq_timer **t) {
  gpq_timer *x = new (std::nothrow) gpq_timer();
  if (!x) return gpq_fail(GPQ_ERR_NOMEM, "out of host memory");
  HIP_TRY(hipEventCreate(&x->a));
  HIP_TRY(hipEventCreate(&x->b));
  *t = x;
  return GPQ_OK;
}
extern "C" int gpq_timer_start(gpq_timer *t, void *stream) { HIP_TRY(hipEventRecord(t->a, (hipStream_t)stream)); return GPQ_OK; }
extern "C" int gpq_timer_stop(gpq_timer *t, void *stream) { HIP_TRY(hipEventRecord(t->b, (hipStream_t)stream)); return GPQ_OK; }
extern "C" int gpq_timer_elapsed_ms(gpq_timer *t, float *ms) {
  HIP_TRY(hipEventSynchronize(t->b));
  HIP_TRY(hipEventElapsedTime(ms, t->a, t->b));
  return GPQ_OK;
}
extern "C" void gpq_timer_destroy(gpq_timer *t) {
  if (!t) return;
  (void)hipEventDestroy(t->a);
  (void)hipEventDestroy(t->b);
  delete t;
}
```

gpqhe_amd/csrc/engine_internal.hpp:

```cpp
#pragma once
#include <cstdio>
#include <map>
#include <set>
#include <string>
#include <vector>
#include "tables.hpp"

struct gpq_prof_rec { int kernel; hipEvent_t a, b; };
enum { GPQ_K_STRIDED_FWD = 0, GPQ_K_STRIDED_INV, GPQ_K_CONTIG_FWD, GPQ_K_CONTIG_INV, GPQ_K_TENSOR_MID,
       GPQ_K_KEYSWITCH_MID, GPQ_K_POINTWISE, GPQ_K_SMALL, GPQ_K_REFERENCE,
       GPQ_K_DECOMPOSE, GPQ_K_RECONSTRUCT, GPQ_K_RELIN_FRONT, GPQ_K_RELIN_TAIL_FUSED, GPQ_K_BRIDGE_EXACT, GPQ_K_RESCALE, GPQ_K_RELIN_TAIL_DIRECT,
       GPQ_K_CRT_DECOMPOSE, GPQ_K_TAIL_STREAM,
       GPQ_K_KEYSWITCH_ROT_MID, GPQ_K_AUTOMORPHISM_GATHER,
       GPQ_K_GEMV_MAC, GPQ_K_COUNT };

struct gpq_recon_mfma {
  void *d_bfrag = nullptr;
  uint64_t *d_lk = nullptr, *d_kc = nullptr, *d_pm = nullptr;
  unsigned KS = 0;
  size_t lds_bytes = 0;
};

struct gpq_bridge_basis {
  unsigned first = 0, dim = 0, pbits = 0;
  int WP = 0;
  uint64_t *d_phat = nullptr, *d_phat_inv = nullptr, *d_pmult = nullptr, *d_phalf = nullptr, *d_inv128 = nullptr;
  std::vector<uint64_t> h_phat_inv;
  std::vector<uint64_t> h_P;
  std::vector<uint64_t> h_phat;
  std::map<int, gpq_recon_mfma> mfma;
  gpq::LimbTab *d_tabs_scaled = nullptr;
};

struct gpq_decomp_mfma {
  void *d_bfrag = nullptr;
  uint64_t *d_pk = nullptr;
  unsigned NT = 0, KS = 0;
  size_t lds_bytes = 0;
};

struct gpq_relin_tables {
  uint64_t *d_pinv = nullptr;
  bool front_tried = false;
  void *d_bfrag = nullptr;
  uint64_t *d_lk = nullptr, *d_pk = nullptr, *d_tkp = nullptr, *d_kf = nullptr;
  unsigned NT = 0, KS = 0;
  size_t lds_bytes = 0;
  void *d_bfrag_w = nullptr;
  uint64_t *d_pk_w = nullptr, *d_tkp_w = nullptr;
  gpq::LimbTab *d_tabs_w = nullptr;
  bool direct_tried = false;
  gpq_recon_mfma direct;
  std::map<unsigned, gpq_recon_mfma> direct_padded;
  const gpq::LimbTab *d_tabs_direct = nullptr;
  uint64_t *d_scale = nullptr, *d_unscale = nullptr;
};

struct gpq_table_cache {
  std::map<std::pair<unsigned, unsigned>, gpq_bridge_basis> bases;
  std::map<std::pair<unsigned, unsigned>, gpq_relin_tables> relins;
  std::map<std::pair<std::pair<unsigned, unsigned>, unsigned>, gpq_decomp_mfma> decomps;
  size_t device_bytes = 0;
};

struct gpq_ctx {
  int device = 0;
  unsigned logn = 0, n = 0, nprimes = 0;
  unsigned chunk = 32;
  unsigned limb_block = 0;
  std::vector<uint64_t> p, pinv_mont, pinv_barr, ninv_mont, psi;
  std::vector<uint64_t> zetas, zetas_inv;
  uint64_t *d_w = nullptr, *d_winv = nullptr;
  gpq::TwS *d_ws = nullptr, *d_winvs = nullptr;
  unsigned nsplit = 0;
  unsigned nsplit_tables = 0;
  bool low9 = false;
  unsigned nwide = 0, nwide_max = 0;
  gpq::LimbTab *d_tabs = nullptr;
  std::vector<gpq::LimbTab> h_tabs;
  const gpq::LimbTab *inv_tabs_override = nullptr;
  gpq_table_cache *cache = nullptr;
  const gpq_ctx *tables_of = nullptr;
  bool bridge_mfma = true;
  unsigned char *d_redo = nullptr;
  size_t redo_cap = 0;
  std::vector<void *> retired;
  unsigned *d_wave_any = nullptr;
  bool lazy_decompose = true;
  unsigned debug_force_redo = 0;
  int nt_mode = -1;
  bool stream_bridge = true;
  bool exact_crt = false;
  bool prescale = true;
  bool prescale_upper = true;
  bool tail_direct = true;
  bool fuse_tail = false;
  int overlap = -1;
  bool peer_failed = false;
  size_t peer_ws_declined = 0;
  int debug_peer_fail = 0;
  unsigned last_lanes = 1;
  std::set<unsigned long long> peer_warm;
  gpq_ctx *peer = nullptr;
  hipStream_t peer_stream = nullptr;
  hipEvent_t ev_fork = nullptr, ev_join = nullptr;
  void *peer_ws = nullptr;
  size_t peer_ws_bytes = 0;
  unsigned *d_zflag = nullptr;
  size_t zflag_cap = 0;
  unsigned *d_zwatch = nullptr;
  size_t zwatch_cap = 0, zwatch_count = 0;
  bool prof_on = false;
  std::vector<gpq_prof_rec> prof;
  std::vector<hipEvent_t> prof_pool;
};

struct DeviceScope {
  int prev = -1;
  explicit DeviceScope(int device) { if (hipGetDevice(&prev) != hipSuccess) prev = -1; (void)hipSetDevice(device); }
  ~DeviceScope() { if (prev >= 0) (void)hipSetDevice(prev); }
};

void gpq_range_push(const char *name);
void gpq_range_pop();
struct StageRange {
  explicit StageRange(const char *name) { gpq_range_push(name); }
  ~StageRange() { gpq_range_pop(); }
  StageRange(const StageRange &) = delete;
  StageRange &operator=(const StageRange &) = delete;
};

struct ProfScope {
  gpq_ctx *c; hipStream_t s; gpq_prof_rec r; bool on;
  ProfScope(const gpq_ctx *cc, int kernel, hipStream_t st) : c(const_cast<gpq_ctx *>(cc)), s(st), on(cc->prof_on) {
    if (!on) return;
    auto get = [&]() { hipEvent_t e; if (!c->prof_pool.empty()) { e = c->prof_pool.back(); c->prof_pool.pop_back(); } else (void)hipEventCreate(&e); return e; };
    r.kernel = kernel; r.a = get(); r.b = get();
    (void)hipEventRecord(r.a, s);
  }
  ~ProfScope() {
    if (!on) return;
    (void)hipEventRecord(r.b, s);
    c->prof.push_back(r);
  }
  ProfScope(const ProfScope &) = delete;
  ProfScope &operator=(const ProfScope &) = delete;
};

int gpq_fail(int code, const char *fmt, ...);
int gpq_ctx_clone(const gpq_ctx *c, gpq_ctx **out);
int gpq_hoist_forward(gpq_ctx *c, uint64_t *slab, unsigned dim, unsigned polys, hipStream_t s);
int gpq_keyswitch_rotated(gpq_ctx *c, uint64_t *c0, uint64_t *c1, const uint64_t *X, const uint64_t *evk0, const uint64_t *evk1,
                          unsigned dim, unsigned polys, unsigned g, void *workspace, hipStream_t s);
int gpq_gemv_mac(gpq_ctx *c, uint64_t *acc0, uint64_t *acc1, const uint64_t *r0, const uint64_t *r1, const uint64_t *diag,
                 const void *terms, unsigned nterms, unsigned dim, unsigned polys, hipStream_t s);
inline hipError_t gpq_table_malloc(gpq_ctx *c, void **p, size_t bytes) {
  hipError_t e = hipMalloc(p, bytes);
  if (e == hipSuccess && c->cache) c->cache->device_bytes += bytes;
  return e;
}
void gpq_bridge_release(gpq_ctx *c);

struct PeerLane {
  gpq_ctx *c = nullptr;
  hipStream_t s = nullptr;
  void *ws = nullptr;
  gpq_ctx *owner = nullptr;
  hipStream_t caller = nullptr;
  PeerLane() = default;
  PeerLane(const PeerLane &) = delete;
  PeerLane &operator=(const PeerLane &) = delete;
  inline int join();
  ~PeerLane() { (void)join(); }
};
inline void gpq_mirror_settings(gpq_ctx *q, const gpq_ctx *c) {
  q->chunk = c->chunk; q->limb_block = c->limb_block; q->nsplit = c->nsplit; q->nwide = c->nwide;
  q->bridge_mfma = c->bridge_mfma; q->lazy_decompose = c->lazy_decompose; q->debug_force_redo = c->debug_force_redo; q->nt_mode = c->nt_mode;
  q->stream_bridge = c->stream_bridge; q->exact_crt = c->exact_crt; q->prescale = c->prescale; q->prescale_upper = c->prescale_upper;
  q->tail_direct = c->tail_direct; q->fuse_tail = c->fuse_tail;
}
constexpr size_t kPeerAutoWorkspaceBytes = (size_t)16 << 30;
template <typename Bytes>
int gpq_peer_lane(gpq_ctx *c, hipStream_t s, unsigned long long key, Bytes bytes, PeerLane *lane) {
  if (c->overlap == 0 || c->peer_failed || c->prof_on || c->inv_tabs_override) return GPQ_OK;
  hipStreamCaptureStatus cap = hipStreamCaptureStatusNone;
  if (hipStreamIsCapturing(s, &cap) != hipSuccess) { (void)hipGetLastError(); return GPQ_OK; }
  const bool capturing = cap != hipStreamCaptureStatusNone;
  if (capturing && (!c->peer || !c->peer_warm.count(key))) return GPQ_OK;
  const size_t need = bytes(c);
  if (!need) return GPQ_OK;
  if (c->overlap < 0 && need > kPeerAutoWorkspaceBytes) return GPQ_OK;
  if (c->peer_ws_declined && need >= c->peer_ws_declined) return GPQ_OK;
  auto give_up = [&](const char *what) {
    (void)hipGetLastError();
    c->peer_failed = true;
    fprintf(stderr, "gpqhe_hip: second lane unavailable (%s): this context continues on one lane\n", what);
    return (int)GPQ_OK;
  };
  if (!c->peer) {
    if (c->debug_peer_fail == 1) return give_up("gpq_debug_fail_peer");
    if (!c->peer_stream && hipStreamCreateWithFlags(&c->peer_stream, hipStreamNonBlocking) != hipSuccess) return give_up("hipStreamCreateWithFlags");
    if (!c->ev_fork && hipEventCreateWithFlags(&c->ev_fork, hipEventDisableTiming) != hipSuccess) return give_up("hipEventCreateWithFlags");
    if (!c->ev_join && hipEventCreateWithFlags(&c->ev_join, hipEventDisableTiming) != hipSuccess) return give_up("hipEventCreateWithFlags");
    if (gpq_ctx_clone(c, &c->peer) != GPQ_OK) { c->peer = nullptr; return give_up("peer context"); }
  }
  gpq_mirror_settings(c->peer, c);
  if (need > c->peer_ws_bytes) {
    if (capturing) return GPQ_OK;
    void *fresh = nullptr;
    if (c->debug_peer_fail == 2 || hipMalloc(&fresh, need) != hipSuccess) {
      (void)hipGetLastError();
      c->peer_ws_declined = need;
      fprintf(stderr, "gpqhe_hip: no room for a second lane's workspace of %zu bytes: shapes of this size run on one lane\n", need);
      return GPQ_OK;
    }
// ... 25 lines not shown
```

gpqhe_amd/csrc/modarith.hpp:

```cpp
#pragma once
#include <hip/hip_runtime.h>
#include <stdint.h>

#define GPQ_FOLD_CMAX 319000000u
#define GPQ_SPLIT_CMAX 306000000u
#define GPQ_WIDE_CMAX 134217000u
static_assert(7ull * (1ull << 29) * GPQ_SPLIT_CMAX < (1ull << 60), "GPQ_SPLIT_CMAX: the single fold of mulmod_split no longer finishes below 3p");
static_assert(12ull * GPQ_SPLIT_CMAX < (1ull << 32), "GPQ_SPLIT_CMAX: th of mulmod_lazy(left < 2p, right < 6p) no longer fits 32 bits");
static_assert(12ull * GPQ_SPLIT_CMAX * GPQ_SPLIT_CMAX < (1ull << 60), "GPQ_SPLIT_CMAX: a product of the split class no longer leaves below 4p");
static_assert(GPQ_WIDE_CMAX <= (1u << 27) && GPQ_WIDE_CMAX <= GPQ_SPLIT_CMAX && GPQ_SPLIT_CMAX <= GPQ_FOLD_CMAX, "butterfly classes must nest: wide <= split <= 7-mad");

#ifndef GPQ_PIN_VOLATILE
#define GPQ_PIN_VOLATILE volatile
#endif

namespace gpq {

typedef unsigned __int128 u128;

struct PrimeK {
  uint64_t p;
  uint64_t p2, p4;
  uint64_t kx0, kx1;
  uint64_t ky;
  uint64_t kys;
  uint64_t p3, np3;
  uint64_t kx1x, kyx;
  uint64_t np, np2, np4;
  uint32_t c;
  uint32_t c1;
};

__device__ __forceinline__ uint64_t mad_u64(uint32_t a, uint32_t b, uint64_t acc) {
  return (uint64_t)a * b + acc;
}
__device__ __forceinline__ uint64_t pack64(uint32_t lo, uint32_t hi) { return ((uint64_t)hi << 32) | lo; }
__device__ __forceinline__ uint32_t not_low27(uint32_t x) { return __builtin_amdgcn_bitop3_b32(x, 0x7ffffffu, x, 0x0c); }

template <bool PIN>
__device__ __forceinline__ uint64_t mulmod_raw_t(uint64_t a, uint64_t w, const PrimeK &k) {
  const uint32_t a0 = (uint32_t)a, a1 = (uint32_t)(a >> 32), w0 = (uint32_t)w, w1 = (uint32_t)(w >> 32);
  const uint64_t m00 = mad_u64(a0, w0, 0);
  uint64_t mid = mad_u64(a0, w1, (uint32_t)(m00 >> 32));
  if (PIN) asm GPQ_PIN_VOLATILE("" : "+v"(mid));
  mid = mad_u64(a1, w0, mid);
  const uint64_t hi = mad_u64(a1, w1, (uint32_t)(mid >> 32));
  const uint32_t midlo = (uint32_t)mid, hilo = (uint32_t)hi, hihi = (uint32_t)(hi >> 32);
  const uint32_t xh0 = __builtin_amdgcn_alignbit(hilo, midlo, 27);
  const uint32_t xh1 = __builtin_amdgcn_alignbit(hihi, hilo, 27);
  const uint64_t xl = pack64((uint32_t)m00, midlo & 0x7ffffffu);
  const uint64_t t0 = mad_u64(k.c, xh0, 0);
  const uint64_t t1 = mad_u64(k.c, xh1, (uint32_t)(t0 >> 32));
  const uint32_t t1lo = (uint32_t)t1, t1hi = (uint32_t)(t1 >> 32);
  const uint32_t th = __builtin_amdgcn_alignbit(t1hi, t1lo, 27);
  const uint64_t ntl = pack64(~(uint32_t)t0, not_low27(t1lo));
  return mad_u64(k.c, th, xl) + ntl;
}

#ifndef GPQ_PIN_CT
#define GPQ_PIN_CT true
#endif
#ifndef GPQ_PIN_GS
#define GPQ_PIN_GS true
#endif
__device__ __forceinline__ uint64_t mulmod_raw(uint64_t a, uint64_t w, const PrimeK &k) { return mulmod_raw_t<false>(a, w, k); }

__device__ __forceinline__ uint64_t mulmod_lazy(uint64_t a, uint64_t w, const PrimeK &k) {
  return mulmod_raw(a, w, k) + k.c1;
}

__device__ __forceinline__ uint64_t csub_by(uint64_t x, uint64_t m, uint64_t neg_m) { return x + (x >= m ? neg_m : (uint64_t)0); }
__device__ __forceinline__ uint64_t csub1(uint64_t x, const PrimeK &k) { return csub_by(x, k.p, k.np); }
__device__ __forceinline__ uint64_t csub2(uint64_t x, const PrimeK &k) { return csub_by(x, k.p2, k.np2); }
__device__ __forceinline__ uint64_t csub4(uint64_t x, const PrimeK &k) { return csub_by(x, k.p4, k.np4); }
__device__ __forceinline__ uint64_t csub3(uint64_t x, const PrimeK &k) { return csub_by(x, k.p3, k.np3); }

__device__ __forceinline__ uint64_t canon8(uint64_t x, const PrimeK &k) {
  return csub1(csub2(csub4(x, k), k), k);
}
__device__ __forceinline__ uint64_t canon4(uint64_t x, const PrimeK &k) {
  return csub1(csub2(x, k), k);
}

__device__ __forceinline__ void ct_bfly(uint64_t &x, uint64_t &y, uint64_t w, const PrimeK &k) {
  const uint64_t t = mulmod_raw_t<GPQ_PIN_CT>(y, w, k);
  const uint64_t xs = x + (x >= k.p4 ? k.kx1 : k.kx0);
  x = xs + t;
  y = xs + k.ky - t;
}

__device__ __forceinline__ void gs_bfly(uint64_t &x, uint64_t &y, uint64_t w, const PrimeK &k) {
  const uint64_t v = x + y;
  const uint64_t d = x + k.p4 - y;
  x = csub4(v, k);
  y = mulmod_raw_t<GPQ_PIN_GS>(d, w, k) + k.c1;
}

typedef ulonglong2 TwS;

struct alignas(16) TwW { uint64_t x, y; };

template <typename W>
__device__ __forceinline__ uint64_t mulmod_split(uint64_t a, const W &w, const PrimeK &k) {
  const uint32_t al = (uint32_t)a & 0x7fffffffu;
  const uint32_t ah = __builtin_amdgcn_alignbit((uint32_t)(a >> 32), (uint32_t)a, 31);
  uint64_t t0 = mad_u64(al, (uint32_t)w.x, 0);
  t0 = mad_u64(ah, (uint32_t)w.y, t0);
  asm GPQ_PIN_VOLATILE("" : "+v"(t0));
  uint64_t t1 = mad_u64(al, (uint32_t)(w.x >> 32), (uint32_t)(t0 >> 32));
  asm GPQ_PIN_VOLATILE("" : "+v"(t1));
  t1 = mad_u64(ah, (uint32_t)(w.y >> 32), t1);
  const uint32_t t1lo = (uint32_t)t1, t1hi = (uint32_t)(t1 >> 32);
  const uint32_t th = __builtin_amdgcn_alignbit(t1hi, t1lo, 27);
  const uint64_t ntl = pack64(~(uint32_t)t0, not_low27(t1lo));
  return mad_u64(k.c, th, ntl);
}

__device__ __forceinline__ void ct_bfly(uint64_t &x, uint64_t &y, const TwS &w, const PrimeK &k) {
  const uint64_t t = mulmod_split(y, w, k);
  const uint64_t xs = x + (x >= k.p3 ? k.kx1x : k.kx0);
  x = xs + t;
  y = xs + k.kyx - t;
}
template <typename W>
__device__ __forceinline__ void gs_bfly_split(uint64_t &x, uint64_t &y, const W &w, const PrimeK &k) {
  const uint64_t v = x + y;
  const uint64_t d = x + k.p3 - y;
  x = csub3(v, k);
  y = mulmod_split(d, w, k) + k.c1;
}
__device__ __forceinline__ void gs_bfly(uint64_t &x, uint64_t &y, const TwS &w, const PrimeK &k) { gs_bfly_split(x, y, w, k); }

template <bool CSUB>
__device__ __forceinline__ void gs_bfly_wide(uint64_t &x, uint64_t &y, const TwW &w, const PrimeK &k) {
  const uint64_t v = x + y;
  const uint64_t d = x + k.p4 - y;
  x = CSUB ? csub4(v, k) : v;
  y = mulmod_split(d, w, k) + k.c1;
}
__device__ __forceinline__ void gs_bfly(uint64_t &x, uint64_t &y, const TwW &w, const PrimeK &k) { gs_bfly_wide<true>(x, y, w, k); }

template <bool CSUB>
__device__ __forceinline__ void ct_bfly_wide(uint64_t &x, uint64_t &y, const TwW &w, const PrimeK &k) {
  const uint64_t t = mulmod_split(y, w, k);
  const uint64_t xs = x + (CSUB ? (x >= k.p4 ? k.kx1 : k.kx0) : k.kx0);
  x = xs + t;
  y = xs + k.kys - t;
}

__device__ __forceinline__ uint64_t mulmod_canon(uint64_t a, uint64_t b, const PrimeK &k) {
  return canon4(mulmod_lazy(a, b, k), k);
}
__device__ __forceinline__ uint64_t canon_fold(uint64_t v, uint64_t p, uint32_t c) {
  const int q = (int)(v >> 59);
  int64_t r = (int64_t)(-(int)c) * q + (int64_t)(v & ((1ull << 59) - 1));
  r += (r >> 63) & (int64_t)p;
  return (uint64_t)r;
}

__device__ __forceinline__ uint64_t mulmod_canon_lazy(uint64_t a, uint64_t b, const PrimeK &k) {
  return canon4(mulmod_lazy(a, b, k), k);
}
__device__ __forceinline__ uint64_t addmod_canon(uint64_t a, uint64_t b, const PrimeK &k) {
  return canon4(a + b, k);
}

}
```

gpqhe_amd/csrc/ntt_kernels.hpp:

```cpp
#pragma once
#include "modarith.hpp"
#include "tables.hpp"

namespace gpq {

template <bool NT> __device__ __forceinline__ uint64_t slab_ld(const uint64_t *p) {
  if constexpr (NT) return __builtin_nontemporal_load(p);
  else return *p;
}
template <bool NT> __device__ __forceinline__ void slab_st(uint64_t *p, uint64_t v) {
  if constexpr (NT) __builtin_nontemporal_store(v, p);
  else *p = v;
}


constexpr int tw_count(int EL, int BHI, int BLO) { return (1 << (EL - BLO)) - (1 << (EL - BHI - 1)); }

constexpr int tw_off(int EL, int BHI, int b) { return (1 << (EL - b - 1)) - (1 << (EL - BHI - 1)); }

template <int EL, int BHI, int B, int BLO, bool UNIFORM, int NTW, typename TW>
__device__ __forceinline__ void load_tw_bits(TW (&tw)[NTW], unsigned ibase, int rs, unsigned logn,
                                             const TW *__restrict__ w) {
  const int sh = rs + B + 1;
  const TW *wp = w + (1u << (logn - sh)) + (UNIFORM ? 0u : (ibase >> sh));
#pragma unroll
  for (int j = 0; j < (1 << (EL - B - 1)); ++j) tw[tw_off(EL, BHI, B) + j] = wp[j];
  if constexpr (B > BLO) load_tw_bits<EL, BHI, B - 1, BLO, UNIFORM>(tw, ibase, rs, logn, w);
}

template <int EL, int BHI, int BLO, bool UNIFORM, typename TW>
__device__ __forceinline__ void load_tw(TW (&tw)[tw_count(EL, BHI, BLO)], unsigned ibase, int rs, unsigned logn,
                                        const TW *__restrict__ w) {
  load_tw_bits<EL, BHI, BHI, BLO, UNIFORM>(tw, ibase, rs, logn, w);
}

template <int S, typename TW>
__device__ __forceinline__ void ct_stage(uint64_t &x, uint64_t &y, const TW &w, const PrimeK &k) { ct_bfly(x, y, w, k); }
template <int S>
__device__ __forceinline__ void ct_stage(uint64_t &x, uint64_t &y, const TwW &w, const PrimeK &k) { ct_bfly_wide<(S & 1) == 0>(x, y, w, k); }

template <int EL, int BHI, int B, int BLO, int RS, int NTW, typename TW>
__device__ __forceinline__ void ct_bits(uint64_t (&x)[1 << EL], const TW (&tw)[NTW], const PrimeK &k) {
#pragma unroll
  for (int e = 0; e < (1 << EL); ++e)
    if (!(e & (1 << B))) ct_stage<RS + B>(x[e], x[e + (1 << B)], tw[tw_off(EL, BHI, B) + (e >> (B + 1))], k);
  if constexpr (B > BLO) ct_bits<EL, BHI, B - 1, BLO, RS>(x, tw, k);
}
template <int EL, int BHI, int BLO, int RS, typename TW>
__device__ __forceinline__ void ct_group(uint64_t (&x)[1 << EL], const TW (&tw)[tw_count(EL, BHI, BLO)],
                                         const PrimeK &k) {
  ct_bits<EL, BHI, BHI, BLO, RS>(x, tw, k);
}

template <bool BOTH_PRODUCT_LEGS, typename TW>
__device__ __forceinline__ void gs_stage(uint64_t &x, uint64_t &y, const TW &w, const PrimeK &k) { gs_bfly(x, y, w, k); }
template <bool BOTH_PRODUCT_LEGS>
__device__ __forceinline__ void gs_stage(uint64_t &x, uint64_t &y, const TwW &w, const PrimeK &k) { gs_bfly_wide<!BOTH_PRODUCT_LEGS>(x, y, w, k); }

template <int EL, int BHI, int B, int NTH, bool CANON_IN, int NTW, typename TW>
__device__ __forceinline__ void gs_bits(uint64_t (&x)[1 << EL], const TW (&tw)[NTW], const PrimeK &k) {
#pragma unroll
  for (int e = 0; e < (1 << EL); ++e)
    if (!(e & (1 << B))) {
      const TW &w = tw[tw_off(EL, BHI, B) + (e >> (B + 1))];
      if ((CANON_IN && NTH < 2) || (NTH > 0 && B > 0 && ((e >> (B > 0 ? B - 1 : 0)) & 1))) gs_stage<true>(x[e], x[e + (1 << B)], w, k);
      else gs_stage<false>(x[e], x[e + (1 << B)], w, k);
    }
  if constexpr (B < BHI) gs_bits<EL, BHI, B + 1, NTH + 1, CANON_IN>(x, tw, k);
}
template <int EL, int BHI, int BLO, bool CANON_IN = false, typename TW>
__device__ __forceinline__ void gs_group(uint64_t (&x)[1 << EL], const TW (&tw)[tw_count(EL, BHI, BLO)],
                                         const PrimeK &k) {
  gs_bits<EL, BHI, BLO, 0, CANON_IN>(x, tw, k);
}

template <typename TW> struct LastK;
template <> struct LastK<uint64_t> {
  uint64_t ninv, winv1_ninv;
  __device__ __forceinline__ explicit LastK(const LimbTab &t) : ninv(t.ninv), winv1_ninv(t.winv1_ninv) {}
};
template <> struct LastK<TwS> {
  TwS ninv, winv1_ninv;
  __device__ __forceinline__ explicit LastK(const LimbTab &t) : ninv(t.ninv_s), winv1_ninv(t.winv1_ninv_s) {}
};
__device__ __forceinline__ void gs_last(uint64_t &x, uint64_t &y, const LastK<uint64_t> &t, const PrimeK &k) {
  const uint64_t s = x + y;
  const uint64_t d = x + k.p4 - y;
  x = canon4(mulmod_lazy(s, t.ninv, k), k);
  y = canon4(mulmod_lazy(d, t.winv1_ninv, k), k);
}
__device__ __forceinline__ void gs_last(uint64_t &x, uint64_t &y, const LastK<TwS> &t, const PrimeK &k) {
  const uint64_t s = x + y;
  const uint64_t d = x + k.p3 - y;
  x = canon4(mulmod_split(s, t.ninv, k) + k.c1, k);
  y = canon4(mulmod_split(d, t.winv1_ninv, k) + k.c1, k);
}

template <typename TW> struct TwTraits;
template <> struct TwTraits<uint64_t> {
  __device__ static __forceinline__ const uint64_t *table(const PassArgs &a, bool inv) { return inv ? a.winv : a.w; }
  __device__ static __forceinline__ uint64_t canon_fwd(uint64_t x, const PrimeK &k) { return canon8(x, k); }
  __device__ static __forceinline__ uint64_t canon_inv(uint64_t x, const PrimeK &k) { return canon4(x, k); }
  __device__ static __forceinline__ uint64_t inv_from4(uint64_t x, const PrimeK &) { return x; }
  __device__ static __forceinline__ uint64_t inv_from8(uint64_t x, const PrimeK &k) { return csub4(x, k); }
  __device__ static __forceinline__ uint64_t left(uint64_t x, const PrimeK &k) { return csub2(csub4(x, k), k); }
  __device__ static __forceinline__ uint64_t right(uint64_t x, const PrimeK &k) { return csub4(x, k); }
};
template <> struct TwTraits<TwS> {
  __device__ static __forceinline__ const TwS *table(const PassArgs &a, bool inv) { return inv ? a.winvs : a.ws; }
  __device__ static __forceinline__ uint64_t canon_fwd(uint64_t x, const PrimeK &k) { return canon_fold(x, k.p, k.c); }
  __device__ static __forceinline__ uint64_t canon_inv(uint64_t x, const PrimeK &k) { return canon4(x, k); }
  __device__ static __forceinline__ uint64_t inv_from4(uint64_t x, const PrimeK &k) { return csub2(x, k); }
  __device__ static __forceinline__ uint64_t inv_from8(uint64_t x, const PrimeK &k) { return csub2(csub4(x, k), k); }
  __device__ static __forceinline__ uint64_t left(uint64_t x, const PrimeK &k) { return csub2(csub4(x, k), k); }
  __device__ static __forceinline__ uint64_t right(uint64_t x, const PrimeK &) { return x; }
};

template <> struct LastK<TwW> : LastK<TwS> {
  __device__ __forceinline__ explicit LastK(const LimbTab &t) : LastK<TwS>(t) {}
};
__device__ __forceinline__ void gs_last(uint64_t &x, uint64_t &y, const LastK<TwW> &t, const PrimeK &k) {
  const uint64_t s = x + y;
  const uint64_t d = x + k.p4 - y;
  x = csub1(mulmod_split(s, t.ninv, k) + k.c1, k);
  y = csub1(mulmod_split(d, t.winv1_ninv, k) + k.c1, k);
}
template <> struct TwTraits<TwW> {
  __device__ static __forceinline__ const TwW *table(const PassArgs &a, bool inv) { return reinterpret_cast<const TwW *>(inv ? a.winvs : a.ws); }
  __device__ static __forceinline__ uint64_t canon_fwd(uint64_t x, const PrimeK &k) { return canon_fold(x, k.p, k.c); }
  __device__ static __forceinline__ uint64_t canon_inv(uint64_t x, const PrimeK &k) { return canon4(x, k); }
  __device__ static __forceinline__ uint64_t inv_from4(uint64_t x, const PrimeK &) { return x; }
  __device__ static __forceinline__ uint64_t inv_from8(uint64_t x, const PrimeK &k) { return csub4(x, k); }
  __device__ static __forceinline__ uint64_t left(uint64_t x, const PrimeK &k) { return csub4(x, k); }
  __device__ static __forceinline__ uint64_t right(uint64_t x, const PrimeK &) { return x; }
};

__device__ __forceinline__ void zero_watch(uint32_t &m, uint64_t x) {
  const uint32_t t = (uint32_t)x | (uint32_t)(x >> 32);
  m = t < m ? t : m;
}
__device__ __forceinline__ void zero_note(const PassArgs &a, uint32_t m, unsigned poly, unsigned limb_in_launch) {
  if (m == 0 && a.zflag) atomicOr(a.zflag + (size_t)poly * a.zstride + limb_in_launch, 1u);
}

#ifndef GPQ_STRIDED_CB
#define GPQ_STRIDED_CB 4
#endif
template <int M1, int EL>
struct StridedGeom {
  static constexpr int CB = M1 <= 8 ? GPQ_STRIDED_CB : 4;
  static constexpr int C = 1 << CB;
  static constexpr int E = 1 << EL;
  static constexpr int T = 1 << (M1 + CB - EL);
  static constexpr int S2 = M1 - EL;
  static constexpr int BB = S2 > 0 ? S2 - 1 : 0;
  static constexpr int LDS_ELEMS = (1 << (M1 + CB)) + ((S2 > 0) ? (C << S2) : 0);
  __device__ static __forceinline__ unsigned pad(unsigned l) { return l + ((l >> (EL + CB)) << CB); }
};

template <int M1, int EL, bool INV, bool CANON_OUT, typename TW, int CW = 8, bool NT = false>
__global__ __launch_bounds__((StridedGeom<M1, EL>::T)) void strided_pass(PassArgs a) {
  using G = StridedGeom<M1, EL>;
  constexpr int E = G::E;
  constexpr unsigned logn = M1 + CW;
  __shared__ uint64_t lds[G::S2 > 0 ? G::LDS_ELEMS : 1];

  unsigned bx = blockIdx.x, by = blockIdx.y, bz = blockIdx.z;
  if (!INV) {
    const unsigned lin = blockIdx.x + gridDim.x * (blockIdx.y + gridDim.y * blockIdx.z), tot = gridDim.x * gridDim.y * gridDim.z;
    const unsigned logical = (lin & 7) * (tot >> 3) + (lin >> 3);
    bx = logical % gridDim.x; by = (logical / gridDim.x) % gridDim.y; bz = logical / (gridDim.x * gridDim.y);
  }
  const unsigned limb = a.limb0 + bz;
  const LimbTab &tab = a.tabs[limb];
  const PrimeK k = tab.k;
  const LastK<TW> last(tab);
  const TW *__restrict__ wt = TwTraits<TW>::table(a, INV) + ((size_t)limb << logn);
  const unsigned slab = by % a.nslab, poly = by / a.nslab;
  const size_t off = (size_t)poly * a.poly_stride + ((size_t)bz << logn);
  const uint64_t *__restrict__ src = a.src[slab] + off;
  uint64_t *__restrict__ dst = a.dst[slab] + off;

  const unsigned tid = threadIdx.x;
  constexpr int CB = G::CB;
  const unsigned col = (bx << CB) + (tid & (G::C - 1));
  const unsigned q = tid >> CB;
  const unsigned iA = (q << CW) + col, iB = (q << (EL + CW)) + col;
  constexpr unsigned strideA = 1u << (G::S2 + CW), strideB = 1u << CW;
  uint64_t x[E];
  TW twB[tw_count(EL, G::BB, 0)];

  if (!INV) {
    TW twA[tw_count(EL, EL - 1, 0)];
#pragma unroll
    for (int e = 0; e < E; ++e) x[e] = slab_ld<NT>(&src[iA + e * strideA]);
    load_tw<EL, EL - 1, 0, true>(twA, iA, G::S2 + CW, logn, wt);
    if (G::S2 > 0) load_tw<EL, G::BB, 0, false>(twB, iB, CW, logn, wt);
    ct_group<EL, EL - 1, 0, G::S2 + CW>(x, twA, k);
    if (G::S2 > 0) {
#pragma unroll
      for (int e = 0; e < E; ++e) lds[G::pad(tid + e * G::T)] = x[e];
      __syncthreads();
#pragma unroll
      for (int e = 0; e < E; ++e) x[e] = lds[G::pad((q << (EL + CB)) + (e << CB) + (tid & (G::C - 1)))];
      ct_group<EL, G::BB, 0, CW>(x, twB, k);
#pragma unroll
      for (int e = 0; e < E; ++e) slab_st<NT>(&dst[iB + e * strideB], CANON_OUT ? TwTraits<TW>::canon_fwd(x[e], k) : x[e]);
    } else {
#pragma unroll
      for (int e = 0; e < E; ++e) slab_st<NT>(&dst[iA + e * strideA], CANON_OUT ? TwTraits<TW>::canon_fwd(x[e], k) : x[e]);
    }
  } else {
    TW twA[tw_count(EL, (EL > 1 ? EL - 2 : 0), 0)];
    if (G::S2 > 0) {
#pragma unroll
      for (int e = 0; e < E; ++e) x[e] = slab_ld<NT>(&src[iB + e * strideB]);
      load_tw<EL, G::BB, 0, false>(twB, iB, CW, logn, wt);
      if (EL > 1) load_tw<EL, (EL > 1 ? EL - 2 : 0), 0, true>(twA, iA, G::S2 + CW, logn, wt);
      gs_group<EL, G::BB, 0>(x, twB, k);
#pragma unroll
      for (int e = 0; e < E; ++e) lds[G::pad((q << (EL + CB)) + (e << CB) + (tid & (G::C - 1)))] = x[e];
      __syncthreads();
#pragma unroll
      for (int e = 0; e < E; ++e) x[e] = lds[G::pad(tid + e * G::T)];
    } else {
#pragma unroll
      for (int e = 0; e < E; ++e) x[e] = slab_ld<NT>(&src[iA + e * strideA]);
      if (EL > 1) load_tw<EL, (EL > 1 ? EL - 2 : 0), 0, true>(twA, iA, G::S2 + CW, logn, wt);
    }
    if (EL > 1) gs_group<EL, (EL > 1 ? EL - 2 : 0), 0>(x, twA, k);
#pragma unroll
    for (int e = 0; e < E / 2; ++e) gs_last(x[e], x[e + E / 2], last, k);
#pragma unroll
    for (int e = 0; e < E; ++e) slab_st<NT>(&dst[iA + e * strideA], x[e]);
  }
}

constexpr int CONTIG_WAVES = 4;
constexpr int CONTIG_LDS_PER_WAVE = 1024 + 64;

__device__ __forceinline__ void wave_lds_sync() {
  __builtin_amdgcn_fence(__ATOMIC_RELEASE, "wavefront");
  __builtin_amdgcn_wave_barrier();
  __builtin_amdgcn_fence(__ATOMIC_ACQUIRE, "wavefront");
}

struct ContigLane {
  unsigned j, blk, hbase, lbase;
  uint64_t *lds;
  __device__ __forceinline__ ContigLane(uint64_t *wave_lds) {
    const unsigned lane = threadIdx.x & 63;
    j = lane & 15; blk = lane >> 4;
    hbase = (blk << 8) + j;
    lbase = (blk << 8) + (j << 4);
    lds = wave_lds;
  }
  __device__ static __forceinline__ unsigned pad(unsigned l) { return l + (l >> 4); }
  __device__ __forceinline__ void h_to_l(uint64_t (&x)[16]) const {
#pragma unroll
    for (int e = 0; e < 16; ++e) lds[pad(hbase + 16 * e)] = x[e];
    wave_lds_sync();
#pragma unroll
    for (int e = 0; e < 16; ++e) x[e] = lds[pad(lbase + e)];
    wave_lds_sync();
  }
  __device__ __forceinline__ void l_to_h(uint64_t (&x)[16]) const {
#pragma unroll
    for (int e = 0; e < 16; ++e) lds[pad(lbase + e)] = x[e];
    wave_lds_sync();
#pragma unroll
    for (int e = 0; e < 16; ++e) x[e] = lds[pad(hbase + 16 * e)];
    wave_lds_sync();
  }
};

template <typename TW>
struct ContigTw {
  TW t[15];
  __device__ __forceinline__ void load_h(const ContigLane &ln, unsigned wave0, unsigned logn, const TW *__restrict__ w) {
    load_tw<4, 3, 0, false>(t, wave0 + ln.hbase, 4, logn, w);
  }
  __device__ __forceinline__ void load_l(const ContigLane &ln, unsigned wave0, unsigned logn, const TW *__restrict__ w) {
    load_tw<4, 3, 0, false>(t, wave0 + ln.lbase, 0, logn, w);
  }
};

template <bool NT> __device__ __forceinline__ void load_h(uint64_t (&x)[16], const uint64_t *__restrict__ p, const ContigLane &ln) {
#pragma unroll
  for (int e = 0; e < 16; ++e) x[e] = slab_ld<NT>(&p[ln.hbase + 16 * e]);
}
template <bool NT> __device__ __forceinline__ void store_h(uint64_t *__restrict__ p, const uint64_t (&x)[16], const ContigLane &ln) {
#pragma unroll
  for (int e = 0; e < 16; ++e) slab_st<NT>(&p[ln.hbase + 16 * e], x[e]);
}
__device__ __forceinline__ void load_l(uint64_t (&x)[16], const uint64_t *__restrict__ p, const ContigLane &ln) {
  const ulonglong2 *v = reinterpret_cast<const ulonglong2 *>(p + ln.lbase);
#pragma unroll
  for (int e = 0; e < 8; ++e) { ulonglong2 t = v[e]; x[2 * e] = t.x; x[2 * e + 1] = t.y; }
}
struct ContigBlock {
  unsigned wave0;
  unsigned limb;
  size_t off;
  size_t toff;
  unsigned slab, poly;
  __device__ __forceinline__ ContigBlock(const PassArgs &a) {
    const unsigned wave = threadIdx.x >> 6;
    wave0 = (blockIdx.x * CONTIG_WAVES + wave) << 10;
    limb = a.limb0 + blockIdx.z;
    slab = blockIdx.y % a.nslab; poly = blockIdx.y / a.nslab;
    off = (size_t)poly * a.poly_stride + ((size_t)blockIdx.z << a.logn) + wave0;
    toff = (size_t)limb << a.logn;
  }
};

#ifndef GPQ_CONTIG_POLYS
#define GPQ_CONTIG_POLYS 2
#endif
constexpr int CONTIG_POLYS = GPQ_CONTIG_POLYS;

#ifndef GPQ_CONTIG_MINWAVES
#define GPQ_CONTIG_MINWAVES 3
#endif
template <bool INV, typename TW, bool NT = false>
__global__ __launch_bounds__(CONTIG_WAVES * 64, (sizeof(TW) == 8 ? 2 : GPQ_CONTIG_MINWAVES)) void contig_pass(PassArgs a, unsigned polys) {
  using TT = TwTraits<TW>;
  __shared__ uint64_t lds[CONTIG_WAVES * CONTIG_LDS_PER_WAVE];
  ContigLane ln(lds + (threadIdx.x >> 6) * CONTIG_LDS_PER_WAVE);
  const unsigned wave0 = (blockIdx.x * CONTIG_WAVES + (threadIdx.x >> 6)) << 10;
  const unsigned limb = a.limb0 + blockIdx.z;
  const LimbTab &tab = a.tabs[limb];
  const PrimeK k = tab.k;
  const unsigned p0 = blockIdx.y * CONTIG_POLYS;
  const unsigned cnt = polys - p0 < CONTIG_POLYS ? polys - p0 : CONTIG_POLYS;
  const size_t off = (size_t)p0 * a.poly_stride + ((size_t)blockIdx.z << a.logn) + wave0;
  const uint64_t *__restrict__ src = a.src[0] + off;
  uint64_t *__restrict__ dst = a.dst[0] + off;
  const TW *__restrict__ wt = TT::table(a, INV) + ((size_t)limb << a.logn);
  if constexpr (sizeof(TW) == 8) {
    uint64_t x[16], nx[16];
    ContigTw<TW> twh, twl;
    load_h<NT>(x, src, ln);
    twh.load_h(ln, wave0, a.logn, wt);
    twl.load_l(ln, wave0, a.logn, wt);
    for (unsigned i = 0; i < cnt; ++i) {
      if (i + 1 < cnt) load_h<NT>(nx, src + (size_t)(i + 1) * a.poly_stride, ln);
      if (!INV) {
        ct_group<4, 3, 0, 4>(x, twh.t, k);
        ln.h_to_l(x);
        ct_group<4, 3, 0, 0>(x, twl.t, k);
        ln.l_to_h(x);
        uint32_t zm = ~0u;
#pragma unroll
        for (int e = 0; e < 16; ++e) { x[e] = TT::canon_fwd(x[e], k); zero_watch(zm, x[e]); }
        zero_note(a, zm, p0 + i, blockIdx.z);
      } else {
        ln.h_to_l(x);
        gs_group<4, 3, 0, true>(x, twl.t, k);
        ln.l_to_h(x);
        gs_group<4, 3, 0>(x, twh.t, k);
      }
      store_h<NT>(dst + (size_t)i * a.poly_stride, x, ln);
#pragma unroll
      for (int e = 0; e < 16; ++e) x[e] = nx[e];
    }
  } else {
    uint64_t x[CONTIG_POLYS][16];
    ContigTw<TW> tw;
#pragma unroll
    for (int j = 0; j < CONTIG_POLYS; ++j)
      if (j < (int)cnt) load_h<NT>(x[j], src + (size_t)j * a.poly_stride, ln);
    if (!INV) {
      tw.load_h(ln, wave0, a.logn, wt);
#pragma unroll
      for (int j = 0; j < CONTIG_POLYS; ++j) if (j < (int)cnt) ct_group<4, 3, 0, 4>(x[j], tw.t, k);
      tw.load_l(ln, wave0, a.logn, wt);
#pragma unroll
      for (int j = 0; j < CONTIG_POLYS; ++j)
        if (j < (int)cnt) {
          ln.h_to_l(x[j]);
          ct_group<4, 3, 0, 0>(x[j], tw.t, k);
          ln.l_to_h(x[j]);
          uint32_t zm = ~0u;
#pragma unroll
          for (int e = 0; e < 16; ++e) { x[j][e] = TT::canon_fwd(x[j][e], k); zero_watch(zm, x[j][e]); }
          zero_note(a, zm, p0 + j, blockIdx.z);
          store_h<NT>(dst + (size_t)j * a.poly_stride, x[j], ln);
        }
    } else {
      tw.load_l(ln, wave0, a.logn, wt);
#pragma unroll
      for (int j = 0; j < CONTIG_POLYS; ++j)
        if (j < (int)cnt) {
          ln.h_to_l(x[j]);
          gs_group<4, 3, 0, true>(x[j], tw.t, k);
          ln.l_to_h(x[j]);
        }
      tw.load_h(ln, wave0, a.logn, wt);
#pragma unroll
      for (int j = 0; j < CONTIG_POLYS; ++j)
        if (j < (int)cnt) {
          gs_group<4, 3, 0>(x[j], tw.t, k);
          store_h<NT>(dst + (size_t)j * a.poly_stride, x[j], ln);
        }
    }
  }
}

struct KeyswitchArgs { PassArgs p; const uint64_t *evk0; const uint64_t *evk1; };

constexpr int LANE8_LDS_PER_WAVE = 576;

template <int LOW>
struct Lane8 {
  static constexpr int JB = LOW - 3;
  static constexpr int MB = LOW - 6;
  static constexpr int LHI = LOW - 7;
  unsigned hk, mk, lk;
  uint64_t *lds;
  __device__ __forceinline__ Lane8(uint64_t *wave_lds) {
    const unsigned lane = threadIdx.x & 63, j = lane & ((1u << JB) - 1), blk = lane >> JB;
    hk = (blk << LOW) + j;
    mk = (blk << LOW) + ((j >> MB) << JB) + (j & ((1u << MB) - 1));
    lk = (blk << LOW) + (j << 3);
    lds = wave_lds;
  }
  __device__ static __forceinline__ unsigned pad1(unsigned l) { return l + ((l >> JB) << MB); }
  __device__ static __forceinline__ unsigned pad2(unsigned l) { return l + (l >> 3); }
  __device__ __forceinline__ void h_to_m(uint64_t (&x)[8]) const {
#pragma unroll
    for (int e = 0; e < 8; ++e) lds[pad1(hk + (e << JB))] = x[e];
    wave_lds_sync();
#pragma unroll
    for (int e = 0; e < 8; ++e) x[e] = lds[pad1(mk + (e << MB))];
    wave_lds_sync();
  }
  __device__ __forceinline__ void m_to_l(uint64_t (&x)[8]) const {
#pragma unroll
    for (int e = 0; e < 8; ++e) lds[pad2(mk + (e << MB))] = x[e];
    wave_lds_sync();
#pragma unroll
    for (int e = 0; e < 8; ++e) x[e] = lds[pad2(lk + e)];
    wave_lds_sync();
  }
  __device__ __forceinline__ void l_to_m(uint64_t (&x)[8]) const {
#pragma unroll
    for (int e = 0; e < 8; ++e) lds[pad2(lk + e)] = x[e];
    wave_lds_sync();
#pragma unroll
    for (int e = 0; e < 8; ++e) x[e] = lds[pad2(mk + (e << MB))];
    wave_lds_sync();
  }
  __device__ __forceinline__ void m_to_h(uint64_t (&x)[8]) const {
#pragma unroll
    for (int e = 0; e < 8; ++e) lds[pad1(mk + (e << MB))] = x[e];
    wave_lds_sync();
#pragma unroll
    for (int e = 0; e < 8; ++e) x[e] = lds[pad1(hk + (e << JB))];
    wave_lds_sync();
  }
  __device__ __forceinline__ void l_to_h(uint64_t (&x)[8]) const {
#pragma unroll
    for (int e = 0; e < 8; ++e) lds[pad2(lk + e)] = x[e];
    wave_lds_sync();
#pragma unroll
    for (int e = 0; e < 8; ++e) x[e] = lds[pad2(hk + (e << JB))];
    wave_lds_sync();
  }
  __device__ __forceinline__ void h_to_l(uint64_t (&x)[8]) const {
#pragma unroll
    for (int e = 0; e < 8; ++e) lds[pad2(hk + (e << JB))] = x[e];
    wave_lds_sync();
#pragma unroll
    for (int e = 0; e < 8; ++e) x[e] = lds[pad2(lk + e)];
    wave_lds_sync();
  }
  __device__ __forceinline__ void load_l(uint64_t (&x)[8], const uint64_t *__restrict__ p) const {
    const ulonglong2 *v = reinterpret_cast<const ulonglong2 *>(p + lk);
#pragma unroll
    for (int e = 0; e < 4; ++e) { ulonglong2 t = v[e]; x[2 * e] = t.x; x[2 * e + 1] = t.y; }
  }
  template <typename TW> __device__ static __forceinline__ void ct_h(uint64_t (&x)[8], const TW (&t)[7], const PrimeK &k) { ct_group<3, 2, 0, LOW - 3>(x, t, k); }
  template <typename TW> __device__ static __forceinline__ void ct_m(uint64_t (&x)[8], const TW (&t)[7], const PrimeK &k) { ct_group<3, 2, 0, LOW - 6>(x, t, k); }
  template <typename TW> __device__ static __forceinline__ void ct_l(uint64_t (&x)[8], const TW (&u)[tw_count(3, LHI, 0)], const PrimeK &k) { ct_group<3, LHI, 0, 0>(x, u, k); }
  template <typename TW> __device__ static __forceinline__ void gs_hm(uint64_t (&x)[8], const TW (&t)[7], const PrimeK &k) { gs_group<3, 2, 0>(x, t, k); }
  template <typename TW> __device__ static __forceinline__ void gs_l(uint64_t (&x)[8], const TW (&u)[tw_count(3, LHI, 0)], const PrimeK &k) { gs_group<3, LHI, 0>(x, u, k); }
  template <typename TW> __device__ static __forceinline__ void gs_l_canon(uint64_t (&x)[8], const TW (&u)[tw_count(3, LHI, 0)], const PrimeK &k) { gs_group<3, LHI, 0, true>(x, u, k); }
};

template <int LOW, bool NT>
struct Lane8N : Lane8<LOW> {
  using Lane8<LOW>::hk;
  using Lane8<LOW>::JB;
  __device__ __forceinline__ Lane8N(uint64_t *wave_lds) : Lane8<LOW>(wave_lds) {}
  __device__ __forceinline__ void load_h(uint64_t (&x)[8], const uint64_t *__restrict__ p) const {
#pragma unroll
    for (int e = 0; e < 8; ++e) x[e] = slab_ld<NT>(&p[hk + (e << JB)]);
  }
  __device__ __forceinline__ void store_h(uint64_t *__restrict__ p, const uint64_t (&x)[8]) const {
#pragma unroll
    for (int e = 0; e < 8; ++e) slab_st<NT>(&p[hk + (e << JB)], x[e]);
  }
};

template <typename TW, int LOW>
struct Tw8 {
  using L8 = Lane8<LOW>;
  TW t[7];
  TW u[tw_count(3, L8::LHI, 0)];
  __device__ __forceinline__ void load_h(const L8 &ln, unsigned wave0, unsigned logn, const TW *__restrict__ w) {
    load_tw<3, 2, 0, false>(t, wave0 + ln.hk, LOW - 3, logn, w);
  }
  __device__ __forceinline__ void load_m(const L8 &ln, unsigned wave0, unsigned logn, const TW *__restrict__ w) {
    load_tw<3, 2, 0, false>(t, wave0 + ln.mk, LOW - 6, logn, w);
  }
  __device__ __forceinline__ void load_l(const L8 &ln, unsigned wave0, unsigned logn, const TW *__restrict__ w) {
    load_tw<3, L8::LHI, 0, false>(u, wave0 + ln.lk, 0, logn, w);
  }
};

struct Block8 {
  unsigned wave0, limb;
  size_t off, toff;
  __device__ __forceinline__ Block8(const PassArgs &a) {
    wave0 = (blockIdx.x * CONTIG_WAVES + (threadIdx.x >> 6)) << 9;
    limb = a.limb0 + blockIdx.z;
    off = (size_t)blockIdx.y * a.poly_stride + ((size_t)blockIdx.z << a.logn) + wave0;
    toff = (size_t)limb << a.logn;
  }
};

#ifndef GPQ_MID8_MINWAVES
#define GPQ_MID8_MINWAVES 3
#endif
template <typename TW, int LOW, bool NT = false>
__global__ __launch_bounds__(CONTIG_WAVES * 64, GPQ_MID8_MINWAVES) void tensor_mid8(PassArgs a) {
  using TT = TwTraits<TW>;
  using L8 = Lane8N<LOW, NT>;
  __shared__ uint64_t lds[CONTIG_WAVES * LANE8_LDS_PER_WAVE];
  L8 ln(lds + (threadIdx.x >> 6) * LANE8_LDS_PER_WAVE);
  const Block8 cb(a);
  const PrimeK k = a.tabs[cb.limb].k;
  const TW *__restrict__ wf = TT::table(a, false) + cb.toff, *__restrict__ wi = TT::table(a, true) + cb.toff;
  uint64_t a0[8], a1[8], b0[8], b1[8];
  Tw8<TW, LOW> tw;
  ln.load_h(a0, a.src[0] + cb.off);
  tw.load_h(ln, cb.wave0, a.logn, wf);
  ln.load_h(b0, a.src[2] + cb.off);
  ln.load_h(a1, a.src[1] + cb.off);
  ln.load_h(b1, a.src[3] + cb.off);
  L8::ct_h(a0, tw.t, k);
  L8::ct_h(b0, tw.t, k);
  L8::ct_h(a1, tw.t, k);
  L8::ct_h(b1, tw.t, k);
  tw.load_m(ln, cb.wave0, a.logn, wf);
  ln.h_to_m(a0); L8::ct_m(a0, tw.t, k);
  ln.h_to_m(b0); L8::ct_m(b0, tw.t, k);
  ln.h_to_m(a1); L8::ct_m(a1, tw.t, k);
  ln.h_to_m(b1); L8::ct_m(b1, tw.t, k);
  tw.load_l(ln, cb.wave0, a.logn, wf);
  ln.m_to_l(a0); L8::ct_l(a0, tw.u, k);
  ln.m_to_l(b0); L8::ct_l(b0, tw.u, k);
  ln.m_to_l(a1); L8::ct_l(a1, tw.u, k);
  ln.m_to_l(b1); L8::ct_l(b1, tw.u, k);
  tw.load_l(ln, cb.wave0, a.logn, wi);
  uint64_t d1[8];
#pragma unroll
  for (int e = 0; e < 8; ++e) {
    const uint64_t u0 = TT::left(a0[e], k), u1 = TT::left(a1[e], k);
    const uint64_t v0 = TT::right(b0[e], k), v1 = TT::right(b1[e], k);
    a0[e] = TT::inv_from4(mulmod_lazy(u0, v0, k), k);
    d1[e] = TT::inv_from8(mulmod_lazy(u0, v1, k) + mulmod_lazy(u1, v0, k), k);
    a1[e] = TT::inv_from4(mulmod_lazy(u1, v1, k), k);
  }
  L8::gs_l(a0, tw.u, k); ln.l_to_m(a0);
  L8::gs_l(d1, tw.u, k); ln.l_to_m(d1);
  L8::gs_l(a1, tw.u, k); ln.l_to_m(a1);
  tw.load_m(ln, cb.wave0, a.logn, wi);
  L8::gs_hm(a0, tw.t, k); ln.m_to_h(a0);
  L8::gs_hm(d1, tw.t, k); ln.m_to_h(d1);
  L8::gs_hm(a1, tw.t, k); ln.m_to_h(a1);
  tw.load_h(ln, cb.wave0, a.logn, wi);
  L8::gs_hm(a0, tw.t, k);
  ln.store_h(a.dst[0] + cb.off, a0);
  L8::gs_hm(d1, tw.t, k);
  ln.store_h(a.dst[1] + cb.off, d1);
  L8::gs_hm(a1, tw.t, k);
  ln.store_h(a.dst[2] + cb.off, a1);
}

template <typename TW, int LOW, bool NT = false>
__global__ __launch_bounds__(CONTIG_WAVES * 64, GPQ_MID8_MINWAVES) void tensor_sq_mid8(PassArgs a) {
  using TT = TwTraits<TW>;
  using L8 = Lane8N<LOW, NT>;
  __shared__ uint64_t lds[CONTIG_WAVES * LANE8_LDS_PER_WAVE];
  L8 ln(lds + (threadIdx.x >> 6) * LANE8_LDS_PER_WAVE);
  const Block8 cb(a);
  const PrimeK k = a.tabs[cb.limb].k;
  const TW *__restrict__ wf = TT::table(a, false) + cb.toff, *__restrict__ wi = TT::table(a, true) + cb.toff;
  uint64_t a0[8], a1[8];
  Tw8<TW, LOW> tw;
  ln.load_h(a0, a.src[0] + cb.off);
  tw.load_h(ln, cb.wave0, a.logn, wf);
  ln.load_h(a1, a.src[1] + cb.off);
  L8::ct_h(a0, tw.t, k);
  L8::ct_h(a1, tw.t, k);
  tw.load_m(ln, cb.wave0, a.logn, wf);
  ln.h_to_m(a0); L8::ct_m(a0, tw.t, k);
  ln.h_to_m(a1); L8::ct_m(a1, tw.t, k);
  tw.load_l(ln, cb.wave0, a.logn, wf);
  ln.m_to_l(a0); L8::ct_l(a0, tw.u, k);
  ln.m_to_l(a1); L8::ct_l(a1, tw.u, k);
  tw.load_l(ln, cb.wave0, a.logn, wi);
  uint64_t d1[8];
#pragma unroll
  for (int e = 0; e < 8; ++e) {
    const uint64_t u0 = TT::left(a0[e], k), u1 = TT::left(a1[e], k);
    const uint64_t v0 = TT::right(a0[e], k), v1 = TT::right(a1[e], k);
    const uint64_t cross = mulmod_lazy(u0, v1, k);
    a0[e] = TT::inv_from4(mulmod_lazy(u0, v0, k), k);
    d1[e] = TT::inv_from8(cross + cross, k);
    a1[e] = TT::inv_from4(mulmod_lazy(u1, v1, k), k);
  }
  L8::gs_l(a0, tw.u, k); ln.l_to_m(a0);
  L8::gs_l(d1, tw.u, k); ln.l_to_m(d1);
  L8::gs_l(a1, tw.u, k); ln.l_to_m(a1);
  tw.load_m(ln, cb.wave0, a.logn, wi);
  L8::gs_hm(a0, tw.t, k); ln.m_to_h(a0);
  L8::gs_hm(d1, tw.t, k); ln.m_to_h(d1);
  L8::gs_hm(a1, tw.t, k); ln.m_to_h(a1);
  tw.load_h(ln, cb.wave0, a.logn, wi);
  L8::gs_hm(a0, tw.t, k);
  ln.store_h(a.dst[0] + cb.off, a0);
  L8::gs_hm(d1, tw.t, k);
  ln.store_h(a.dst[1] + cb.off, d1);
  L8::gs_hm(a1, tw.t, k);
  ln.store_h(a.dst[2] + cb.off, a1);
}

template <typename TW, int LOW, bool NT = false>
__global__ __launch_bounds__(CONTIG_WAVES * 64, 4) void polymul_mid8(PassArgs a) {
  using TT = TwTraits<TW>;
  using L8 = Lane8N<LOW, NT>;
  __shared__ uint64_t lds[CONTIG_WAVES * LANE8_LDS_PER_WAVE];
  L8 ln(lds + (threadIdx.x >> 6) * LANE8_LDS_PER_WAVE);
  const Block8 cb(a);
  const PrimeK k = a.tabs[cb.limb].k;
  const TW *__restrict__ wf = TT::table(a, false) + cb.toff, *__restrict__ wi = TT::table(a, true) + cb.toff;
  uint64_t x[8], y[8];
  Tw8<TW, LOW> tw;
  ln.load_h(x, a.src[0] + cb.off);
  tw.load_h(ln, cb.wave0, a.logn, wf);
  ln.load_h(y, a.src[1] + cb.off);
  L8::ct_h(x, tw.t, k);
  L8::ct_h(y, tw.t, k);
  tw.load_m(ln, cb.wave0, a.logn, wf);
  ln.h_to_m(x); L8::ct_m(x, tw.t, k);
  ln.h_to_m(y); L8::ct_m(y, tw.t, k);
  tw.load_l(ln, cb.wave0, a.logn, wf);
  ln.m_to_l(x); L8::ct_l(x, tw.u, k);
  ln.m_to_l(y); L8::ct_l(y, tw.u, k);
  tw.load_l(ln, cb.wave0, a.logn, wi);
#pragma unroll
  for (int e = 0; e < 8; ++e) x[e] = TT::inv_from4(mulmod_lazy(TT::left(x[e], k), TT::right(y[e], k), k), k);
  L8::gs_l(x, tw.u, k); ln.l_to_m(x);
  tw.load_m(ln, cb.wave0, a.logn, wi);
  L8::gs_hm(x, tw.t, k); ln.m_to_h(x);
  tw.load_h(ln, cb.wave0, a.logn, wi);
  L8::gs_hm(x, tw.t, k);
  ln.store_h(a.dst[0] + cb.off, x);
}

template <typename TW, int LOW, bool NT = false>
__global__ __launch_bounds__(CONTIG_WAVES * 64, 3) void mulpt_mid8(PassArgs a) {
  using TT = TwTraits<TW>;
  using L8 = Lane8N<LOW, NT>;
  __shared__ uint64_t lds[CONTIG_WAVES * LANE8_LDS_PER_WAVE];
  L8 ln(lds + (threadIdx.x >> 6) * LANE8_LDS_PER_WAVE);
  const Block8 cb(a);
  const PrimeK k = a.tabs[cb.limb].k;
  const TW *__restrict__ wf = TT::table(a, false) + cb.toff, *__restrict__ wi = TT::table(a, true) + cb.toff;
  uint64_t m[8], x[8], y[8];
  Tw8<TW, LOW> tw;
  ln.load_h(m, a.src[0] + cb.off);
  tw.load_h(ln, cb.wave0, a.logn, wf);
  ln.load_h(x, a.src[1] + cb.off);
  ln.load_h(y, a.src[2] + cb.off);
  L8::ct_h(m, tw.t, k);
  L8::ct_h(x, tw.t, k);
  L8::ct_h(y, tw.t, k);
  tw.load_m(ln, cb.wave0, a.logn, wf);
  ln.h_to_m(m); L8::ct_m(m, tw.t, k);
  ln.h_to_m(x); L8::ct_m(x, tw.t, k);
  ln.h_to_m(y); L8::ct_m(y, tw.t, k);
  tw.load_l(ln, cb.wave0, a.logn, wf);
  ln.m_to_l(m); L8::ct_l(m, tw.u, k);
  ln.m_to_l(x); L8::ct_l(x, tw.u, k);
  ln.m_to_l(y); L8::ct_l(y, tw.u, k);
  tw.load_l(ln, cb.wave0, a.logn, wi);
#pragma unroll
  for (int e = 0; e < 8; ++e) {
    const uint64_t u = TT::left(m[e], k);
    x[e] = TT::inv_from4(mulmod_lazy(u, TT::right(x[e], k), k), k);
    y[e] = TT::inv_from4(mulmod_lazy(u, TT::right(y[e], k), k), k);
  }
  L8::gs_l(x, tw.u, k); ln.l_to_m(x);
  L8::gs_l(y, tw.u, k); ln.l_to_m(y);
  tw.load_m(ln, cb.wave0, a.logn, wi);
  L8::gs_hm(x, tw.t, k); ln.m_to_h(x);
  L8::gs_hm(y, tw.t, k); ln.m_to_h(y);
  tw.load_h(ln, cb.wave0, a.logn, wi);
  L8::gs_hm(x, tw.t, k);
  ln.store_h(a.dst[0] + cb.off, x);
  L8::gs_hm(y, tw.t, k);
  ln.store_h(a.dst[1] + cb.off, y);
}

template <typename TW, int LOW, bool TWO = true, bool NT = false>
__global__ __launch_bounds__(CONTIG_WAVES * 64, 3) void keyswitch_mid8x2(KeyswitchArgs ka, unsigned first) {
  using TT = TwTraits<TW>;
  using L8 = Lane8N<LOW, NT>;
  __shared__ uint64_t lds[CONTIG_WAVES * LANE8_LDS_PER_WAVE];
  const PassArgs &a = ka.p;
  L8 ln(lds + (threadIdx.x >> 6) * LANE8_LDS_PER_WAVE);
  const unsigned wave0 = (blockIdx.x * CONTIG_WAVES + (threadIdx.x >> 6)) << 9;
  const unsigned limb = a.limb0 + blockIdx.z;
  const PrimeK k = a.tabs[limb].k;
  const size_t toff = (size_t)limb << a.logn;
  const TW *__restrict__ wf = TT::table(a, false) + toff, *__restrict__ wi = TT::table(a, true) + toff;
  const unsigned p0 = first + 2 * blockIdx.y;
  constexpr bool two = TWO;
  const size_t off0 = (size_t)p0 * a.poly_stride + ((size_t)blockIdx.z << a.logn) + wave0;
  const size_t off1 = two ? off0 + a.poly_stride : off0;
  const size_t koff = ((size_t)blockIdx.z << a.logn) + wave0;
  uint64_t x0[8], x1[8], e0[8], e1[8];
  Tw8<TW, LOW> tw;
  ln.load_h(x0, a.src[0] + off0);
  tw.load_h(ln, wave0, a.logn, wf);
  if constexpr (two) ln.load_h(x1, a.src[0] + off1);
  L8::ct_h(x0, tw.t, k);
  if constexpr (two) L8::ct_h(x1, tw.t, k);
  tw.load_m(ln, wave0, a.logn, wf);
  ln.h_to_m(x0); L8::ct_m(x0, tw.t, k);
  if constexpr (two) { ln.h_to_m(x1); L8::ct_m(x1, tw.t, k); }
  tw.load_l(ln, wave0, a.logn, wf);
  ln.m_to_l(x0); L8::ct_l(x0, tw.u, k);
  if constexpr (two) { ln.m_to_l(x1); L8::ct_l(x1, tw.u, k); }
  ln.load_l(e0, ka.evk0 + koff);
  ln.load_l(e1, ka.evk1 + koff);
  tw.load_l(ln, wave0, a.logn, wi);
  uint64_t y0[8], y1[8];
#pragma unroll
  for (int e = 0; e < 8; ++e) {
    const uint64_t u0 = TT::right(x0[e], k);
    x0[e] = TT::inv_from4(mulmod_lazy(u0, e0[e], k), k);
    y0[e] = TT::inv_from4(mulmod_lazy(u0, e1[e], k), k);
  }
  if constexpr (two) {
#pragma unroll
    for (int e = 0; e < 8; ++e) {
      const uint64_t u1 = TT::right(x1[e], k);
      x1[e] = TT::inv_from4(mulmod_lazy(u1, e0[e], k), k);
      y1[e] = TT::inv_from4(mulmod_lazy(u1, e1[e], k), k);
    }
  }
  L8::gs_l(x0, tw.u, k); ln.l_to_m(x0);
  L8::gs_l(y0, tw.u, k); ln.l_to_m(y0);
  if constexpr (two) {
    L8::gs_l(x1, tw.u, k); ln.l_to_m(x1);
    L8::gs_l(y1, tw.u, k); ln.l_to_m(y1);
  }
  tw.load_m(ln, wave0, a.logn, wi);
  L8::gs_hm(x0, tw.t, k); ln.m_to_h(x0);
  L8::gs_hm(y0, tw.t, k); ln.m_to_h(y0);
  if constexpr (two) {
    L8::gs_hm(x1, tw.t, k); ln.m_to_h(x1);
    L8::gs_hm(y1, tw.t, k); ln.m_to_h(y1);
  }
  tw.load_h(ln, wave0, a.logn, wi);
  L8::gs_hm(x0, tw.t, k);
  ln.store_h(a.dst[0] + off0, x0);
  L8::gs_hm(y0, tw.t, k);
  ln.store_h(a.dst[1] + off0, y0);
  if constexpr (two) {
    L8::gs_hm(x1, tw.t, k);
    ln.store_h(a.dst[0] + off1, x1);
    L8::gs_hm(y1, tw.t, k);
    ln.store_h(a.dst[1] + off1, y1);
  }
}

__device__ __forceinline__ unsigned automorphism_src(unsigned j, unsigned logn, unsigned g) {
  const unsigned mask2n = (2u << logn) - 1;
  const unsigned e = (((__brev(j) >> (32 - logn)) << 1) | 1u) * g & mask2n;
  return __brev(e >> 1) >> (32 - logn);
}

template <typename TW, int LOW, bool TWO = true, bool NT = false>
__global__ __launch_bounds__(CONTIG_WAVES * 64, 3) void keyswitch_rot_mid8x2(KeyswitchArgs ka, unsigned first, unsigned g) {
  using TT = TwTraits<TW>;
  using L8 = Lane8N<LOW, NT>;
  __shared__ uint64_t lds[CONTIG_WAVES * LANE8_LDS_PER_WAVE];
  const PassArgs &a = ka.p;
  L8 ln(lds + (threadIdx.x >> 6) * LANE8_LDS_PER_WAVE);
  const unsigned wave0 = (blockIdx.x * CONTIG_WAVES + (threadIdx.x >> 6)) << 9;
  const unsigned limb = a.limb0 + blockIdx.z;
  const PrimeK k = a.tabs[limb].k;
  const size_t toff = (size_t)limb << a.logn;
  const TW *__restrict__ wi = TT::table(a, true) + toff;
  const unsigned p0 = first + 2 * blockIdx.y;
  constexpr bool two = TWO;
  const size_t off0 = (size_t)p0 * a.poly_stride + ((size_t)blockIdx.z << a.logn) + wave0;
  const size_t off1 = two ? off0 + a.poly_stride : off0;
  const size_t koff = ((size_t)blockIdx.z << a.logn) + wave0;
  const unsigned src0 = automorphism_src(wave0, a.logn, g) & ~511u;
  const size_t soff0 = off0 - wave0 + src0, soff1 = off1 - wave0 + src0;
  unsigned sl[8];
#pragma unroll
  for (int e = 0; e < 8; ++e) sl[e] = automorphism_src(wave0 + ln.lk + e, a.logn, g) & 511u;
  auto gather = [&](uint64_t (&x)[8], size_t soff) {
    ln.load_h(x, a.src[0] + soff);
#pragma unroll
    for (int e = 0; e < 8; ++e) ln.lds[L8::pad2(ln.hk + (e << L8::JB))] = x[e];
    wave_lds_sync();
#pragma unroll
    for (int e = 0; e < 8; ++e) x[e] = ln.lds[L8::pad2(sl[e])];
    wave_lds_sync();
  };
  uint64_t x0[8], x1[8], e0[8], e1[8];
  Tw8<TW, LOW> tw;
  gather(x0, soff0);
  if constexpr (two) gather(x1, soff1);
  ln.load_l(e0, ka.evk0 + koff);
  ln.load_l(e1, ka.evk1 + koff);
  tw.load_l(ln, wave0, a.logn, wi);
  uint64_t y0[8], y1[8];
#pragma unroll
  for (int e = 0; e < 8; ++e) {
    const uint64_t u0 = TT::right(x0[e], k);
    x0[e] = TT::inv_from4(mulmod_lazy(u0, e0[e], k), k);
    y0[e] = TT::inv_from4(mulmod_lazy(u0, e1[e], k), k);
  }
  if constexpr (two) {
#pragma unroll
    for (int e = 0; e < 8; ++e) {
      const uint64_t u1 = TT::right(x1[e], k);
      x1[e] = TT::inv_from4(mulmod_lazy(u1, e0[e], k), k);
      y1[e] = TT::inv_from4(mulmod_lazy(u1, e1[e], k), k);
    }
  }
  L8::gs_l(x0, tw.u, k); ln.l_to_m(x0);
  L8::gs_l(y0, tw.u, k); ln.l_to_m(y0);
  if constexpr (two) {
    L8::gs_l(x1, tw.u, k); ln.l_to_m(x1);
    L8::gs_l(y1, tw.u, k); ln.l_to_m(y1);
  }
  tw.load_m(ln, wave0, a.logn, wi);
  L8::gs_hm(x0, tw.t, k); ln.m_to_h(x0);
  L8::gs_hm(y0, tw.t, k); ln.m_to_h(y0);
  if constexpr (two) {
    L8::gs_hm(x1, tw.t, k); ln.m_to_h(x1);
    L8::gs_hm(y1, tw.t, k); ln.m_to_h(y1);
  }
  tw.load_h(ln, wave0, a.logn, wi);
  L8::gs_hm(x0, tw.t, k);
  ln.store_h(a.dst[0] + off0, x0);
  L8::gs_hm(y0, tw.t, k);
  ln.store_h(a.dst[1] + off0, y0);
  if constexpr (two) {
    L8::gs_hm(x1, tw.t, k);
    ln.store_h(a.dst[0] + off1, x1);
    L8::gs_hm(y1, tw.t, k);
    ln.store_h(a.dst[1] + off1, y1);
  }
}

__global__ __launch_bounds__(256) void automorphism_gather(const uint64_t *__restrict__ src, uint64_t *__restrict__ dst, unsigned logn, unsigned g) {
  const unsigned j = blockIdx.x * 256 + threadIdx.x;
  if (j >= (1u << logn)) return;
  const size_t row = (size_t)blockIdx.y << logn;
  dst[row + j] = src[row + automorphism_src(j, logn, g)];
}

typedef unsigned long long v2u64 __attribute__((ext_vector_type(2)));
struct GemvMacArgs {
  const LimbTab *tabs;
  const uint64_t *r0, *r1;
  const uint64_t *diag;
  uint64_t *acc0, *acc1;
  const uint2 *terms;
  unsigned nterms, polys, dim, logn;
};
template <bool NT>
__device__ __forceinline__ v2u64 gemv_ld16(const v2u64 *p) {
  if constexpr (NT) return __builtin_nontemporal_load(p);
  else return *p;
}
template <int BT, bool NT>
__global__ __launch_bounds__(256) void gemv_mac(GemvMacArgs a) {
  const PrimeK k = a.tabs[blockIdx.z].k;
  const unsigned i2 = 2 * (blockIdx.y * 256 + threadIdx.x);
  if (i2 >= (1u << a.logn)) return;
  const unsigned b0 = blockIdx.x * BT, cnt = a.polys - b0 < (unsigned)BT ? a.polys - b0 : (unsigned)BT;
  const size_t limb_off = ((size_t)blockIdx.z << a.logn) + i2, poly = (size_t)a.dim << a.logn;
  v2u64 s0[BT], s1[BT];
#pragma unroll
  for (int b = 0; b < BT; ++b) s0[b] = s1[b] = v2u64{0, 0};
  for (unsigned t = 0; t < a.nterms; ++t) {
    const uint2 e = a.terms[t];
    const v2u64 d = *reinterpret_cast<const v2u64 *>(a.diag + (size_t)e.y * poly + limb_off);
    const size_t roff = ((size_t)e.x * a.polys + b0) * poly + limb_off;
#pragma unroll
    for (int b = 0; b < BT; ++b)
      if (b < (int)cnt) {
        const v2u64 *p0 = reinterpret_cast<const v2u64 *>(a.r0 + roff + b * poly), *p1 = reinterpret_cast<const v2u64 *>(a.r1 + roff + b * poly);
        const v2u64 u = gemv_ld16<NT>(p0), v = gemv_ld16<NT>(p1);
        s0[b].x = csub4(s0[b].x + mulmod_lazy(u.x, d.x, k), k);
        s0[b].y = csub4(s0[b].y + mulmod_lazy(u.y, d.y, k), k);
        s1[b].x = csub4(s1[b].x + mulmod_lazy(v.x, d.x, k), k);
        s1[b].y = csub4(s1[b].y + mulmod_lazy(v.y, d.y, k), k);
      }
  }
#pragma unroll
  for (int b = 0; b < BT; ++b)
    if (b < (int)cnt) {
      const size_t o = (size_t)(b0 + b) * poly + limb_off;
      *reinterpret_cast<v2u64 *>(a.acc0 + o) = v2u64{canon4(s0[b].x, k), canon4(s0[b].y, k)};
      *reinterpret_cast<v2u64 *>(a.acc1 + o) = v2u64{canon4(s1[b].x, k), canon4(s1[b].y, k)};
    }
}

constexpr int CONTIG8_POLYS = 2;
template <bool INV, typename TW, int LOW, bool NT = false>
__global__ __launch_bounds__(CONTIG_WAVES * 64, 4) void contig_pass8(PassArgs a, unsigned polys) {
  using TT = TwTraits<TW>;
  using L8 = Lane8N<LOW, NT>;
  __shared__ uint64_t lds[CONTIG_WAVES * LANE8_LDS_PER_WAVE];
  L8 ln(lds + (threadIdx.x >> 6) * LANE8_LDS_PER_WAVE);
  const unsigned wave0 = (blockIdx.x * CONTIG_WAVES + (threadIdx.x >> 6)) << 9;
  const unsigned limb = a.limb0 + blockIdx.z;
  const PrimeK k = a.tabs[limb].k;
  const unsigned p0 = blockIdx.y * CONTIG8_POLYS;
  const unsigned cnt = polys - p0 < CONTIG8_POLYS ? polys - p0 : CONTIG8_POLYS;
  const size_t off = (size_t)p0 * a.poly_stride + ((size_t)blockIdx.z << a.logn) + wave0;
  const uint64_t *__restrict__ src = a.src[0] + off;
  uint64_t *__restrict__ dst = a.dst[0] + off;
  const TW *__restrict__ wt = TT::table(a, INV) + ((size_t)limb << a.logn);
  uint64_t x[CONTIG8_POLYS][8];
  Tw8<TW, LOW> tw;
#pragma unroll
  for (int j = 0; j < CONTIG8_POLYS; ++j)
    if (j < (int)cnt) ln.load_h(x[j], src + (size_t)j * a.poly_stride);
  if (!INV) {
    tw.load_h(ln, wave0, a.logn, wt);
#pragma unroll
    for (int j = 0; j < CONTIG8_POLYS; ++j) if (j < (int)cnt) L8::ct_h(x[j], tw.t, k);
    tw.load_m(ln, wave0, a.logn, wt);
#pragma unroll
    for (int j = 0; j < CONTIG8_POLYS; ++j) if (j < (int)cnt) { ln.h_to_m(x[j]); L8::ct_m(x[j], tw.t, k); }
    tw.load_l(ln, wave0, a.logn, wt);
#pragma unroll
    for (int j = 0; j < CONTIG8_POLYS; ++j)
      if (j < (int)cnt) {
        ln.m_to_l(x[j]);
        L8::ct_l(x[j], tw.u, k);
        uint32_t zm = ~0u;
#pragma unroll
        for (int e = 0; e < 8; ++e) { x[j][e] = TT::canon_fwd(x[j][e], k); zero_watch(zm, x[j][e]); }
        zero_note(a, zm, p0 + j, blockIdx.z);
        ln.l_to_h(x[j]);
        ln.store_h(dst + (size_t)j * a.poly_stride, x[j]);
      }
  } else {
    tw.load_l(ln, wave0, a.logn, wt);
#pragma unroll
    for (int j = 0; j < CONTIG8_POLYS; ++j) if (j < (int)cnt) { ln.h_to_l(x[j]); L8::gs_l_canon(x[j], tw.u, k); }
    tw.load_m(ln, wave0, a.logn, wt);
#pragma unroll
    for (int j = 0; j < CONTIG8_POLYS; ++j) if (j < (int)cnt) { ln.l_to_m(x[j]); L8::gs_hm(x[j], tw.t, k); }
    tw.load_h(ln, wave0, a.logn, wt);
#pragma unroll
    for (int j = 0; j < CONTIG8_POLYS; ++j)
      if (j < (int)cnt) {
        ln.m_to_h(x[j]);
        L8::gs_hm(x[j], tw.t, k);
        ln.store_h(dst + (size_t)j * a.poly_stride, x[j]);
      }
  }
}

template <bool MUL>
__global__ __launch_bounds__(256) void pointwise(PassArgs a) {
  const LimbTab &tab = a.tabs[a.limb0 + blockIdx.z];
  const PrimeK k = tab.k;
  const unsigned i2 = 2 * (blockIdx.x * 256 + threadIdx.x);
  if (i2 >= (1u << a.logn)) return;
  const size_t off = (size_t)blockIdx.y * a.poly_stride + ((size_t)blockIdx.z << a.logn) + i2;
  const ulonglong2 u = *reinterpret_cast<const ulonglong2 *>(a.src[0] + off);
  const ulonglong2 v = *reinterpret_cast<const ulonglong2 *>(a.src[1] + off);
  ulonglong2 r;
  if (MUL) { r.x = mulmod_canon(u.x, v.x, k); r.y = mulmod_canon(u.y, v.y, k); }
  else     { r.x = addmod_canon(u.x, v.x, k); r.y = addmod_canon(u.y, v.y, k); }
  *reinterpret_cast<ulonglong2 *>(a.dst[0] + off) = r;
}

constexpr int SMALL_MAX_LOGN = 12;

template <bool INV, typename TW>
__global__ __launch_bounds__(256) void small_ntt(PassArgs a) {
  using TT = TwTraits<TW>;
  __shared__ uint64_t s[1 << SMALL_MAX_LOGN];
  const LimbTab &tab = a.tabs[a.limb0 + blockIdx.z];
  const PrimeK k = tab.k;
  const LastK<TW> last(tab);
  const unsigned n = 1u << a.logn;
  const TW *__restrict__ wt = TT::table(a, INV) + ((size_t)(a.limb0 + blockIdx.z) << a.logn);
  const unsigned slab = blockIdx.y % a.nslab, poly = blockIdx.y / a.nslab;
  const size_t off = (size_t)poly * a.poly_stride + ((size_t)blockIdx.z << a.logn);
  const uint64_t *__restrict__ src = a.src[slab] + off;
  uint64_t *__restrict__ dst = a.dst[slab] + off;
  for (unsigned i = threadIdx.x; i < n; i += 256) s[i] = src[i];
  __syncthreads();
  if (!INV) {
    for (unsigned len = n >> 1; len >= 1; len >>= 1) {
      for (unsigned b = threadIdx.x; b < (n >> 1); b += 256) {
        const unsigned blk = b / len, j = blk * 2 * len + (b % len);
        uint64_t x = s[j], y = s[j + len];
        ct_bfly(x, y, wt[n / (2 * len) + blk], k);
        s[j] = TT::canon_fwd(x, k); s[j + len] = TT::canon_fwd(y, k);
      }
      __syncthreads();
    }
  } else {
    for (unsigned len = 1; len < (n >> 1); len <<= 1) {
      for (unsigned b = threadIdx.x; b < (n >> 1); b += 256) {
        const unsigned blk = b / len, j = blk * 2 * len + (b % len);
        uint64_t x = s[j], y = s[j + len];
        gs_bfly(x, y, wt[n / (2 * len) + blk], k);
        s[j] = TT::canon_inv(x, k); s[j + len] = TT::canon_inv(y, k);
      }
      __syncthreads();
    }
    if (n >= 2) {
      for (unsigned b = threadIdx.x; b < (n >> 1); b += 256) {
        uint64_t x = s[b], y = s[b + (n >> 1)];
        gs_last(x, y, last, k);
        s[b] = x; s[b + (n >> 1)] = y;
      }
      __syncthreads();
    }
  }
  uint32_t zm = ~0u;
  for (unsigned i = threadIdx.x; i < n; i += 256) { dst[i] = s[i]; zero_watch(zm, s[i]); }
  if (!INV && a.nslab == 1) zero_note(a, zm, blockIdx.y, blockIdx.z);
}

__device__ __forceinline__ uint64_t ref_fqmul(uint64_t a, uint64_t w, const PrimeK &k) {
  if (a >= 2 * k.p4) a %= k.p;
  return mulmod_canon(a, w, k);
}
template <bool INV>
__device__ void ref_transform_limb(uint64_t *__restrict__ v, unsigned logn, const uint64_t *__restrict__ w, const LimbTab &tab) {
  const PrimeK k = tab.k;
  const uint64_t q = k.p;
  const unsigned n = 1u << logn, half = n >> 1, T = blockDim.x;
  if (!INV) {
    for (unsigned ls = logn; ls-- > 0;) {
      const unsigned len = 1u << ls;
      for (unsigned b = threadIdx.x; b < half; b += T) {
        const unsigned blk = b >> ls, j = (blk << (ls + 1)) + (b & (len - 1));
        const uint64_t zeta = w[(n >> (ls + 1)) + blk];
        const uint64_t x = v[j];
        const uint64_t t = ref_fqmul(v[j + len], zeta, k);
        v[j + len] = (x >= t) ? x - t : x - t + q;
        v[j] = (x <= q - t) ? x + t : x + t - q;
      }
      __syncthreads();
    }
  } else {
    for (unsigned ls = 0; ls < logn; ++ls) {
      const unsigned len = 1u << ls;
      for (unsigned b = threadIdx.x; b < half; b += T) {
        const unsigned blk = b >> ls, j = (blk << (ls + 1)) + (b & (len - 1));
        const uint64_t zeta_inv = w[(n >> (ls + 1)) + blk];
        const uint64_t t = v[j], y = v[j + len];
        v[j] = (y <= q - t) ? t + y : t + y - q;
        const uint64_t d = (y <= t) ? t - y : t - y + q;
        v[j + len] = ref_fqmul(d, zeta_inv, k);
      }
      __syncthreads();
    }
    for (unsigned i = threadIdx.x; i < n; i += T) v[i] = ref_fqmul(v[i], tab.ninv, k);
    __syncthreads();
  }
}

__global__ __launch_bounds__(1024) void ref_zero_redo(PassArgs a, unsigned polys, unsigned limbs, unsigned mode) {
  const unsigned total = polys * limbs;
  for (unsigned idx = blockIdx.x; idx < total; idx += gridDim.x) {
    const unsigned poly = idx / limbs, z = idx % limbs;
    unsigned *flag = a.zflag + (size_t)poly * a.zstride + z;
    if (mode == 0 && *flag == 0) continue;
    const unsigned limb = a.limb0 + z;
    const LimbTab &tab = a.tabs[limb];
    uint64_t *v = a.dst[0] + (size_t)poly * a.poly_stride + ((size_t)z << a.logn);
    const size_t toff = (size_t)limb << a.logn;
    if (mode != 1) ref_transform_limb<true>(v, a.logn, a.winv + toff, tab);
    if (mode != 2) ref_transform_limb<false>(v, a.logn, a.w + toff, tab);
    if (mode == 0) { __syncthreads(); if (threadIdx.x == 0) *flag = 0; }
  }
}

}
```

include/gpqhe_hip.h:

```cpp
#ifndef GPQHE_HIP_H
#define GPQHE_HIP_H

#include <stddef.h>
#include <stdint.h>

#ifdef __cplusplus
extern "C" {
#endif

#define GPQ_OK 0
#define GPQ_ERR_INVALID (-1)
#define GPQ_ERR_HIP (-2)
#define GPQ_ERR_UNSUPPORTED (-3)
#define GPQ_ERR_NOMEM (-4)

typedef struct gpq_ctx gpq_ctx;

int gpq_ctx_create(gpq_ctx **out, unsigned logn, unsigned nprimes, int device);

int gpq_ctx_create_from_tables(gpq_ctx **out, unsigned logn, unsigned nprimes, const uint64_t *primes,
                               const uint64_t *const *zetas_mont, const uint64_t *const *zetas_inv_mont, int device);
void gpq_ctx_destroy(gpq_ctx *ctx);

unsigned gpq_ctx_logn(const gpq_ctx *ctx);
unsigned gpq_ctx_nprimes(const gpq_ctx *ctx);
int gpq_ctx_device(const gpq_ctx *ctx);
uint64_t gpq_ctx_const(const gpq_ctx *ctx, unsigned d, int which);
const uint64_t *gpq_ctx_zetas(const gpq_ctx *ctx, unsigned d, int inverse);

unsigned gpq_dimub(unsigned logn, unsigned logq);

const char *gpq_last_error(void);

int gpq_malloc(void **dptr, size_t bytes);
int gpq_free(void *dptr);
int gpq_upload(void *dst_dev, const void *src_host, size_t bytes, void *stream);
int gpq_download(void *dst_host, const void *src_dev, size_t bytes, void *stream);
int gpq_copy(void *dst_dev, const void *src_dev, size_t bytes, void *stream);
int gpq_stream_sync(void *stream);
int gpq_stream_wait(void *waiter, void *on);
int gpq_device_count(void);
int gpq_probe_stream(void *dst, const void *src, size_t bytes, int kind, unsigned blocks, unsigned threads, unsigned unroll, void *stream);
int gpq_set_device(int device);
int gpq_stream_create(void **stream);
int gpq_stream_destroy(void *stream);
int gpq_malloc_host(void **hptr, size_t bytes);
int gpq_free_host(void *hptr);
int gpq_bind_thread_to_device(int device);
int gpq_device_local_cpus(int device, const char *sysfs_root, char *cpulist, size_t cap);


int gpq_ntt(gpq_ctx *ctx, uint64_t *slab, unsigned dim, unsigned batch, void *stream);
int gpq_invntt(gpq_ctx *ctx, uint64_t *slab, unsigned dim, unsigned batch, void *stream);
int gpq_ntt_reference(gpq_ctx *ctx, uint64_t *slab, unsigned dim, unsigned batch, int inverse, void *stream);

int gpq_rns_mul(gpq_ctx *ctx, uint64_t *r, const uint64_t *a, const uint64_t *b, unsigned dim, unsigned batch, void *stream);
int gpq_rns_add(gpq_ctx *ctx, uint64_t *r, const uint64_t *a, const uint64_t *b, unsigned dim, unsigned batch, void *stream);

int gpq_poly_mul_rns(gpq_ctx *ctx, uint64_t *r, uint64_t *a, uint64_t *b, unsigned dim, unsigned batch, void *stream);
int gpq_mulpt_rns(gpq_ctx *ctx, uint64_t *r0, uint64_t *r1, uint64_t *m, uint64_t *x0, uint64_t *x1, unsigned dim, unsigned batch,
                  void *stream);

int gpq_set_chunk(gpq_ctx *ctx, unsigned chunk);
int gpq_set_limb_block(gpq_ctx *ctx, unsigned limbs);
int gpq_set_limb_classes(gpq_ctx *ctx, unsigned wide, unsigned split);

size_t gpq_tensor_workspace_bytes(const gpq_ctx *ctx, unsigned dim, unsigned batch);
size_t gpq_keyswitch_workspace_bytes(const gpq_ctx *ctx, unsigned dim, unsigned batch);

int gpq_he_mul_tensor(gpq_ctx *ctx, uint64_t *d0, uint64_t *d1, uint64_t *d2,
                      const uint64_t *a0, const uint64_t *a1, const uint64_t *b0, const uint64_t *b1,
                      unsigned dim, unsigned batch, void *workspace, void *stream);

int gpq_keyswitch(gpq_ctx *ctx, uint64_t *c0, uint64_t *c1, const uint64_t *x,
                  const uint64_t *evk0, const uint64_t *evk1,
                  unsigned dim, unsigned batch, void *workspace, void *stream);

unsigned gpq_big_words(unsigned bits);
uint64_t gpq_ctx_phat_invmp(gpq_ctx *ctx, unsigned dim, unsigned d);
unsigned gpq_ctx_pbits(gpq_ctx *ctx, unsigned dim);

int gpq_rns_decompose(gpq_ctx *ctx, uint64_t *slab, const uint64_t *big, unsigned W, unsigned dim, unsigned batch, void *stream);
int gpq_rns_decompose_limbs(gpq_ctx *ctx, uint64_t *slab, const uint64_t *big, unsigned W, unsigned first, unsigned count,
                            unsigned batch, void *stream);
int gpq_rns_reconstruct_one(gpq_ctx *ctx, uint64_t *words, unsigned Wout, const uint64_t *residues, unsigned dim);
int gpq_rns_reconstruct(gpq_ctx *ctx, uint64_t *big, unsigned Wout, const uint64_t *slab, unsigned dim, unsigned batch,
                        unsigned logq, void *stream);
int gpq_set_exact_crt(gpq_ctx *ctx, int on);
int gpq_set_stream_bridge(gpq_ctx *ctx, int on);
int gpq_set_overlap(gpq_ctx *ctx, int on);
unsigned gpq_last_lanes(const gpq_ctx *ctx);
int gpq_debug_fail_peer(gpq_ctx *ctx, int on);
size_t gpq_debug_table_bytes(const gpq_ctx *ctx, int which);
int gpq_set_lazy_decompose(gpq_ctx *ctx, int on);
int gpq_set_nt_policy(gpq_ctx *ctx, int mode);
int gpq_debug_force_redo(gpq_ctx *ctx, unsigned every);
int gpq_debug_zero_watch(gpq_ctx *ctx, int on);
long gpq_debug_zero_flags(gpq_ctx *ctx, unsigned *before, unsigned *after, size_t capacity);
int gpq_set_fused_tail(gpq_ctx *ctx, int on);
int gpq_set_prescale(gpq_ctx *ctx, int on);
int gpq_set_bridge_mfma(gpq_ctx *ctx, int on);

size_t gpq_poly_mul_workspace_bytes(const gpq_ctx *ctx, unsigned dim, unsigned batch);
int gpq_poly_mul(gpq_ctx *ctx, uint64_t *r, const uint64_t *a, const uint64_t *b, unsigned W, unsigned dim, unsigned logq,
                 unsigned batch, void *workspace, void *stream);
size_t gpq_poly_mul_general_workspace_bytes(gpq_ctx *ctx, unsigned dim, unsigned batch);
int gpq_rns_reconstruct_general(gpq_ctx *ctx, uint64_t *big, unsigned Wout, const uint64_t *slab, unsigned dim, unsigned batch,
                                const uint64_t *q_words, unsigned Lq, void *scratch, void *stream);
int gpq_poly_mul_general(gpq_ctx *ctx, uint64_t *r, const uint64_t *a, const uint64_t *b, unsigned W, unsigned dim,
                         const uint64_t *q_words, unsigned Lq, unsigned batch, void *workspace, void *stream);

int gpq_he_rs(gpq_ctx *ctx, uint64_t *c0, uint64_t *c1, unsigned W, unsigned logDelta, unsigned logql, unsigned batch, void *stream);
int gpq_he_rescale(gpq_ctx *ctx, uint64_t *c0, uint64_t *c1, unsigned W, unsigned logDelta, unsigned logql, unsigned batch, void *stream);

int gpq_he_dims(gpq_ctx *ctx, unsigned logqL, unsigned logql, unsigned *dimP, unsigned *dimA, unsigned *dimB, unsigned *dimevk);

size_t gpq_he_mul_workspace_bytes(gpq_ctx *ctx, unsigned W, unsigned dimA, unsigned dimB, unsigned dimP, unsigned batch);
int gpq_he_mul(gpq_ctx *ctx, uint64_t *out_c0, uint64_t *out_c1, const uint64_t *ct1c0, const uint64_t *ct1c1,
               const uint64_t *ct2c0, const uint64_t *ct2c1, const uint64_t *rlk0, const uint64_t *rlk1, unsigned W,
               unsigned logql, unsigned dimA, unsigned dimB, unsigned dimP, unsigned batch, void *workspace, void *stream);
int gpq_he_mul_rs(gpq_ctx *ctx, uint64_t *out_c0, uint64_t *out_c1, const uint64_t *ct1c0, const uint64_t *ct1c1,
                  const uint64_t *ct2c0, const uint64_t *ct2c1, const uint64_t *rlk0, const uint64_t *rlk1, unsigned W,
                  unsigned logql, unsigned dimA, unsigned dimB, unsigned dimP, unsigned logDelta, unsigned batch, void *workspace, void *stream);

size_t gpq_relin_tail_workspace_bytes(gpq_ctx *ctx, unsigned W, unsigned dimB, unsigned dimP, unsigned batch);
int gpq_relin_tail(gpq_ctx *ctx, uint64_t *out, const uint64_t *chat, const uint64_t *d, unsigned W, unsigned logql,
                   unsigned dimB, unsigned dimP, unsigned batch, void *workspace, void *stream);
int gpq_big_transpose(gpq_ctx *ctx, uint64_t *dst, const uint64_t *src, unsigned W, unsigned batch, int to_rows, void *stream);
int gpq_big_addsub(gpq_ctx *ctx, uint64_t *out, const uint64_t *a, const uint64_t *b, unsigned W, unsigned polys, int mode, void *stream);
int gpq_relin_tail_overwriting(gpq_ctx *ctx, uint64_t *out, uint64_t *chat, const uint64_t *d, unsigned W, unsigned logql,
                               unsigned dimB, unsigned dimP, unsigned batch, void *workspace, void *stream);

size_t gpq_he_swk_workspace_bytes(gpq_ctx *ctx, unsigned W, unsigned dimB, unsigned dimP, unsigned batch);
int gpq_he_swk(gpq_ctx *ctx, uint64_t *out_c0, uint64_t *out_c1, const uint64_t *d0, const uint64_t *d1,
               const uint64_t *swk0, const uint64_t *swk1, unsigned W, unsigned logql, unsigned dimB, unsigned dimP,
               unsigned batch, void *workspace, void *stream);

size_t gpq_he_mulpt_workspace_bytes(const gpq_ctx *ctx, unsigned dim, unsigned batch);
int gpq_he_mulpt(gpq_ctx *ctx, uint64_t *out_c0, uint64_t *out_c1, const uint64_t *c0, const uint64_t *c1, const uint64_t *m,
                 unsigned W, unsigned logql, unsigned dim, unsigned batch, void *workspace, void *stream);
int gpq_poly_rot(gpq_ctx *ctx, uint64_t *r, const uint64_t *a, unsigned W, unsigned rot, unsigned batch, void *stream);
int gpq_poly_conj(gpq_ctx *ctx, uint64_t *r, const uint64_t *a, unsigned W, unsigned batch, void *stream);

int gpq_automorphism_index(unsigned logn, uint64_t g, uint32_t *idx);
size_t gpq_he_rot_hoisted_workspace_bytes(gpq_ctx *ctx, unsigned W, unsigned dimB, unsigned dimP, unsigned nrot, unsigned batch);
int gpq_he_rot_hoisted(gpq_ctx *ctx, uint64_t *out_c0, uint64_t *out_c1, const uint64_t *c0, const uint64_t *c1,
                       const unsigned *rots, const uint64_t *const *rk0, const uint64_t *const *rk1, unsigned nrot,
                       unsigned W, unsigned logql, unsigned dimB, unsigned dimP, unsigned batch, void *workspace, void *stream);
size_t gpq_he_gemv_workspace_bytes(gpq_ctx *ctx, unsigned W, unsigned slots, unsigned dimB, unsigned dimP, unsigned dimpt, unsigned batch);
int gpq_he_gemv(gpq_ctx *ctx, uint64_t *out_c0, uint64_t *out_c1, const uint64_t *c0, const uint64_t *c1, const uint64_t *diag,
                const uint64_t *const *rk0, const uint64_t *const *rk1, unsigned slots, unsigned W, unsigned logql,
                unsigned logDelta, unsigned dimB, unsigned dimP, unsigned dimpt, unsigned batch, void *workspace, void *stream);

typedef struct gpq_gemv_plan gpq_gemv_plan;
unsigned gpq_gemv_acc_dim(unsigned logql, unsigned diag_bits, unsigned logn, unsigned n1);
int gpq_gemv_plan_create(gpq_ctx *ctx, gpq_gemv_plan **plan, const uint64_t *diag, unsigned slots, unsigned W, unsigned logql,
                         unsigned dimpt, void *stream);
void gpq_gemv_plan_destroy(gpq_gemv_plan *plan);
int gpq_gemv_plan_info(const gpq_gemv_plan *plan, unsigned *dim, size_t *bytes, unsigned *live, int *exact);
int gpq_gemv_plan_rotations(const gpq_gemv_plan *plan, unsigned char *needed);
size_t gpq_gemv_inner_workspace_bytes(gpq_ctx *ctx, const gpq_gemv_plan *plan, unsigned batch);
int gpq_gemv_inner(gpq_ctx *ctx, uint64_t *out_c0, uint64_t *out_c1, const uint64_t *R0, const uint64_t *R1, const gpq_gemv_plan *plan,
                   unsigned giant, unsigned W, unsigned batch, void *workspace, void *stream);
size_t gpq_he_gemv_planned_workspace_bytes(gpq_ctx *ctx, const gpq_gemv_plan *plan, unsigned W, unsigned dimB, unsigned dimP, unsigned batch);
int gpq_he_gemv_planned(gpq_ctx *ctx, uint64_t *out_c0, uint64_t *out_c1, const uint64_t *c0, const uint64_t *c1, const gpq_gemv_plan *plan,
                        const uint64_t *const *rk0, const uint64_t *const *rk1, unsigned W, unsigned logDelta, unsigned dimB, unsigned dimP,
                        unsigned batch, void *workspace, void *stream);

size_t gpq_he_general_workspace_bytes(gpq_ctx *ctx, unsigned W, unsigned dimA, unsigned dimB, unsigned dimP, unsigned batch);
int gpq_he_rs_general(gpq_ctx *ctx, uint64_t *c0, uint64_t *c1, unsigned W, unsigned long long delta, const uint64_t *ql_words,
                      unsigned Lq, unsigned batch, void *scratch , void *stream);
int gpq_relin_tail_general(gpq_ctx *ctx, uint64_t *out, const uint64_t *chat, const uint64_t *d, unsigned W, const uint64_t *ql_words,
                           unsigned Lq, unsigned dimB, unsigned dimP, unsigned batch, void *workspace, void *stream);
int gpq_he_mul_general(gpq_ctx *ctx, uint64_t *out_c0, uint64_t *out_c1, const uint64_t *ct1c0, const uint64_t *ct1c1,
                       const uint64_t *ct2c0, const uint64_t *ct2c1, const uint64_t *rlk0, const uint64_t *rlk1, unsigned W,
                       const uint64_t *ql_words, unsigned Lq, unsigned dimA, unsigned dimB, unsigned dimP, unsigned batch,
                       void *workspace, void *stream);
int gpq_he_mulpt_general(gpq_ctx *ctx, uint64_t *out_c0, uint64_t *out_c1, const uint64_t *c0, const uint64_t *c1, const uint64_t *m,
                         unsigned W, const uint64_t *ql_words, unsigned Lq, unsigned dim, unsigned batch, void *workspace, void *stream);
int gpq_he_swk_general(gpq_ctx *ctx, uint64_t *out_c0, uint64_t *out_c1, const uint64_t *d0, const uint64_t *d1,
                       const uint64_t *swk0, const uint64_t *swk1, unsigned W, const uint64_t *ql_words, unsigned Lq,
                       unsigned dimB, unsigned dimP, unsigned batch, void *workspace, void *stream);

int gpq_big_add(gpq_ctx *ctx, uint64_t *r, const uint64_t *a, const uint64_t *b, unsigned W, unsigned logql, unsigned batch, void *stream);
int gpq_big_sub(gpq_ctx *ctx, uint64_t *r, const uint64_t *a, const uint64_t *b, unsigned W, unsigned logql, unsigned batch, void *stream);
int gpq_big_neg(gpq_ctx *ctx, uint64_t *r, const uint64_t *a, unsigned W, unsigned logql, unsigned batch, void *stream);
int gpq_evk_pack(gpq_ctx *ctx, uint64_t *evk, const uint64_t *big, unsigned W, unsigned dimevk, unsigned batch, void *stream);
size_t gpq_he_genswk_workspace_bytes(gpq_ctx *ctx, unsigned W, unsigned dimP, unsigned logqL);
int gpq_he_genswk(gpq_ctx *ctx, uint64_t *evk0, uint64_t *evk1, const uint64_t *p1, const uint64_t *sk, const uint64_t *e,
                  const uint64_t *sp, unsigned W, unsigned dimP, unsigned logqL, unsigned dimevk, void *workspace, void *stream);

int gpq_profile_enable(gpq_ctx *ctx, int on);
int gpq_profile_kernels(void);
const char *gpq_profile_kernel_name(int kernel);
int gpq_profile_collect(gpq_ctx *ctx, double *total_ms, unsigned long long *launches);

typedef struct gpq_timer gpq_timer;
int gpq_timer_create(gpq_timer **t);
int gpq_timer_start(gpq_timer *t, void *stream);
int gpq_timer_stop(gpq_timer *t, void *stream);
int gpq_timer_elapsed_ms(gpq_timer *t, float *ms);
void gpq_timer_destroy(gpq_timer *t);

#ifdef __cplusplus
}
#endif
#endif
```

Baseline: 7551 he_mul/s.

## Fold the c+1 lazy-reduction offset into the Montgomery-free mulmod accumulator seed

Seeds the first 32x32 multiply-add of mulmod_raw and mulmod_split with the correction constant (c1, or 31c-1 plus a pinned 'one' in the upper word). This removes the separate '+ k.c1' add after every modular multiply and turns the butterfly offset constants into plain multiples of p. Because the seeded product can now overflow for some split/wide twiddle entries, host-side checks lower nwide when an entry does not fit, including per scaled table. It also raises the keyswitch mid-kernel occupancy hint to 4 for the TWO variant, which risks register pressure or spills.

```diff
diff --git a/gpqhe_amd/_native.py b/gpqhe_amd/_native.py
--- a/gpqhe_amd/_native.py
+++ b/gpqhe_amd/_native.py
@@ -69,6 +69,7 @@
     "gpq_set_exact_crt": (C.c_int, [vp, C.c_int]),
     "gpq_set_stream_bridge": (C.c_int, [vp, C.c_int]),
     "gpq_debug_force_redo": (C.c_int, [vp, C.c_uint]),
+    "gpq_debug_split_entry_fits_wide": (C.c_int, [u64, u64, u64]),
     "gpq_debug_zero_watch": (C.c_int, [vp, C.c_int]),
     "gpq_debug_zero_flags": (C.c_long, [vp, vp, vp, C.c_size_t]),
     "gpq_set_lazy_decompose": (C.c_int, [vp, C.c_int]),
diff --git a/gpqhe_amd/csrc/bridge.hip b/gpqhe_amd/csrc/bridge.hip
--- a/gpqhe_amd/csrc/bridge.hip
+++ b/gpqhe_amd/csrc/bridge.hip
@@ -152,6 +152,11 @@
   return GPQ_OK;
 }
 
+static unsigned first_unfit_wide_limb(const gpq_ctx *c, const std::vector<LimbTab> &t, unsigned first, unsigned count) {
+  for (unsigned d = first; d < first + count && d < c->nwide_max; ++d)
+    if (!split_entry_fits_wide(t[d].k.p, t[d].ninv_s.x, t[d].ninv_s.y) || !split_entry_fits_wide(t[d].k.p, t[d].winv1_ninv_s.x, t[d].winv1_ninv_s.y)) return d;
+  return ~0u;
+}
 int get_scaled_tabs(gpq_ctx *c, gpq_bridge_basis *b, const LimbTab **out) {
   if (!b->d_tabs_scaled) {
     std::vector<LimbTab> t = c->h_tabs;
@@ -163,16 +168,27 @@
       e.winv1_ninv = (uint64_t)((u128h)e.winv1_ninv * s % p);
       if (b->first + d < c->nsplit_tables) { e.ninv_s = pair_of(e.ninv, p); e.winv1_ninv_s = pair_of(e.winv1_ninv, p); }
     }
+    const unsigned unfit = first_unfit_wide_limb(c, t, b->first, b->dim);
     DeviceScope on_device(c->device);
     HIP_TRY(gpq_table_malloc(c, (void **)&b->d_tabs_scaled, t.size() * sizeof(LimbTab)));
     HIP_TRY(hipMemcpy(b->d_tabs_scaled, t.data(), t.size() * sizeof(LimbTab), hipMemcpyHostToDevice));
+    if (unfit != ~0u) c->cache->scaled_wide_limit[b->d_tabs_scaled] = unfit;
   }
   *out = b->d_tabs_scaled;
   return GPQ_OK;
 }
 struct ScaledInverse {
   gpq_ctx *c;
-  ScaledInverse(gpq_ctx *ctx, const LimbTab *tabs) : c(ctx) { c->inv_tabs_override = tabs; }
+  ScaledInverse(gpq_ctx *ctx, const LimbTab *tabs) : c(ctx) {
+    c->inv_tabs_override = tabs;
+    if (tabs && c->cache && !c->cache->scaled_wide_limit.empty()) {
+      const auto it = c->cache->scaled_wide_limit.find(tabs);
+      if (it != c->cache->scaled_wide_limit.end()) {
+        if (c->nwide_max > it->second) c->nwide_max = it->second;
+        if (c->nwide > it->second) c->nwide = it->second;
+      }
+    }
+  }
   ~ScaledInverse() { c->inv_tabs_override = nullptr; }
 };
 inline bool can_prescale(const gpq_ctx *c) { return c->prescale && c->logn > 12 && !c->h_tabs.empty(); }
@@ -888,6 +904,8 @@
     HIP_TRY(hipMemcpy(rt->d_pk_w, pkw.data(), pkw.size() * 8, hipMemcpyHostToDevice));
     HIP_TRY(hipMemcpy(rt->d_tkp_w, tkpw.data(), tkpw.size() * 8, hipMemcpyHostToDevice));
     HIP_TRY(hipMemcpy(rt->d_tabs_w, tw.data(), tw.size() * sizeof(LimbTab), hipMemcpyHostToDevice));
+    const unsigned unfit = first_unfit_wide_limb(c, tw, 0, dimB);
+    if (unfit != ~0u) c->cache->scaled_wide_limit[rt->d_tabs_w] = unfit;
   }
   rt->NT = NT; rt->KS = KS; rt->lds_bytes = lds;
   return GPQ_OK;
diff --git a/gpqhe_amd/csrc/engine.hip b/gpqhe_amd/csrc/engine.hip
--- a/gpqhe_amd/csrc/engine.hip
+++ b/gpqhe_amd/csrc/engine.hip
@@ -170,9 +170,8 @@
     }
     LimbTab &t = tabs[d];
     t.k.p = p; t.k.p2 = 2 * p; t.k.p4 = 4 * p; t.k.c = (uint32_t)(p - (1ull << 59)); t.k.c1 = t.k.c + 1;
-    t.k.kx0 = t.k.c1; t.k.kx1 = (uint64_t)t.k.c1 - 4 * p; t.k.ky = 4 * p - 2 * (uint64_t)t.k.c1;
-    t.k.kys = 2 * p - 2 * (uint64_t)t.k.c1;
-    t.k.p3 = 3 * p; t.k.np3 = (uint64_t)0 - 3 * p; t.k.kx1x = (uint64_t)t.k.c1 - 3 * p; t.k.kyx = 3 * p - 2 * (uint64_t)t.k.c1;
+    t.k.kinj = 31 * (uint64_t)t.k.c - 1; t.k.one = 1;
+    t.k.p3 = 3 * p; t.k.np3 = (uint64_t)0 - 3 * p;
     t.k.np = (uint64_t)0 - p; t.k.np2 = (uint64_t)0 - 2 * p; t.k.np4 = (uint64_t)0 - 4 * p;
     t.ninv = from_mont(c->ninv_mont[d]);
     t.winv1_ninv = n >= 2 ? mulm(wistd[d * n + 1], t.ninv, p) : t.ninv;
@@ -182,7 +181,7 @@
   while (c->nsplit < np && c->p[c->nsplit] - (1ull << 59) < GPQ_SPLIT_CMAX) ++c->nsplit;
   c->nwide = 0;
   while (c->nwide < c->nsplit && c->p[c->nwide] - (1ull << 59) < GPQ_WIDE_CMAX) ++c->nwide;
-  c->nsplit_tables = c->nsplit; c->nwide_max = c->nwide;
+  c->nsplit_tables = c->nsplit;
   c->low9 = c->logn == 17;
   if (c->nsplit) {
     const size_t ns = c->nsplit;
@@ -196,12 +195,19 @@
       }
       tabs[d].ninv_s = pair_of(tabs[d].ninv, p);
       tabs[d].winv1_ninv_s = pair_of(tabs[d].winv1_ninv, p);
+      if (d < c->nwide) {
+        bool ok = split_entry_fits_wide(p, tabs[d].ninv_s.x, tabs[d].ninv_s.y) && split_entry_fits_wide(p, tabs[d].winv1_ninv_s.x, tabs[d].winv1_ninv_s.y);
+        for (size_t i = 1; ok && i < n; ++i)
+          ok = split_entry_fits_wide(p, ws[d * n + i].x, ws[d * n + i].y) && split_entry_fits_wide(p, wis[d * n + i].x, wis[d * n + i].y);
+        if (!ok) c->nwide = (unsigned)d;
+      }
     }
     HIP_TRY(gpq_table_malloc(c, (void **)&c->d_ws, ns * n * sizeof(TwS)));
     HIP_TRY(gpq_table_malloc(c, (void **)&c->d_winvs, ns * n * sizeof(TwS)));
     HIP_TRY(hipMemcpy(c->d_ws, ws.data(), ns * n * sizeof(TwS), hipMemcpyHostToDevice));
     HIP_TRY(hipMemcpy(c->d_winvs, wis.data(), ns * n * sizeof(TwS), hipMemcpyHostToDevice));
   }
+  c->nwide_max = c->nwide;
   HIP_TRY(hipMemcpy(c->d_w, wstd.data(), np * n * 8, hipMemcpyHostToDevice));
   HIP_TRY(hipMemcpy(c->d_winv, wistd.data(), np * n * 8, hipMemcpyHostToDevice));
   HIP_TRY(hipMemcpy(c->d_tabs, tabs.data(), np * sizeof(LimbTab), hipMemcpyHostToDevice));
@@ -1025,6 +1031,11 @@
   return GPQ_OK;
 }
 
+extern "C" int gpq_debug_split_entry_fits_wide(uint64_t p, uint64_t x, uint64_t y) {
+  if (p <= (1ull << 59) || p - (1ull << 59) >= GPQ_WIDE_CMAX || x > p || y > p) return -1;
+  return split_entry_fits_wide(p, x, y) ? 1 : 0;
+}
+
 extern "C" int gpq_set_limb_block(gpq_ctx *c, unsigned limbs) {
   if (!c) return gpq_fail(GPQ_ERR_INVALID, "gpq_set_limb_block: null context");
   c->limb_block = limbs;
diff --git a/gpqhe_amd/csrc/engine_internal.hpp b/gpqhe_amd/csrc/engine_internal.hpp
--- a/gpqhe_amd/csrc/engine_internal.hpp
+++ b/gpqhe_amd/csrc/engine_internal.hpp
@@ -61,6 +61,7 @@
   std::map<std::pair<unsigned, unsigned>, gpq_relin_tables> relins;
   std::map<std::pair<std::pair<unsigned, unsigned>, unsigned>, gpq_decomp_mfma> decomps;
   size_t device_bytes = 0;
+  std::map<const gpq::LimbTab *, unsigned> scaled_wide_limit;
 };
 
 struct gpq_ctx {
diff --git a/gpqhe_amd/csrc/modarith.hpp b/gpqhe_amd/csrc/modarith.hpp
--- a/gpqhe_amd/csrc/modarith.hpp
+++ b/gpqhe_amd/csrc/modarith.hpp
@@ -5,7 +5,8 @@
 #define GPQ_FOLD_CMAX 319000000u
 #define GPQ_SPLIT_CMAX 306000000u
 #define GPQ_WIDE_CMAX 134217000u
-static_assert(7ull * (1ull << 29) * GPQ_SPLIT_CMAX < (1ull << 60), "GPQ_SPLIT_CMAX: the single fold of mulmod_split no longer finishes below 3p");
+static_assert((7ull * (1ull << 29) + 33) * GPQ_SPLIT_CMAX < (1ull << 60), "GPQ_SPLIT_CMAX: the single fold of mulmod_split no longer finishes below 3p");
+static_assert(31ull * GPQ_SPLIT_CMAX < (1ull << 33) + (1ull << 32), "GPQ_SPLIT_CMAX: the low column of mulmod_split (two 31 x 32 products + 31c - 1) no longer fits 64 bits");
 static_assert(12ull * GPQ_SPLIT_CMAX < (1ull << 32), "GPQ_SPLIT_CMAX: th of mulmod_lazy(left < 2p, right < 6p) no longer fits 32 bits");
 static_assert(12ull * GPQ_SPLIT_CMAX * GPQ_SPLIT_CMAX < (1ull << 60), "GPQ_SPLIT_CMAX: a product of the split class no longer leaves below 4p");
 static_assert(GPQ_WIDE_CMAX <= (1u << 27) && GPQ_WIDE_CMAX <= GPQ_SPLIT_CMAX && GPQ_SPLIT_CMAX <= GPQ_FOLD_CMAX, "butterfly classes must nest: wide <= split <= 7-mad");
@@ -21,15 +22,21 @@
 struct PrimeK {
   uint64_t p;
   uint64_t p2, p4;
-  uint64_t kx0, kx1;
-  uint64_t ky;
-  uint64_t kys;
   uint64_t p3, np3;
-  uint64_t kx1x, kyx;
   uint64_t np, np2, np4;
+  uint64_t kinj;
   uint32_t c;
   uint32_t c1;
+  uint32_t one;
 };
+
+__device__ __forceinline__ PrimeK pin_consts(const PrimeK &src) {
+  PrimeK k = src;
+  uint32_t one = 1;
+  asm("" : "+v"(one));
+  k.one = one;
+  return k;
+}
 
 __device__ __forceinline__ uint64_t mad_u64(uint32_t a, uint32_t b, uint64_t acc) {
   return (uint64_t)a * b + acc;
@@ -40,7 +47,7 @@
 template <bool PIN>
 __device__ __forceinline__ uint64_t mulmod_raw_t(uint64_t a, uint64_t w, const PrimeK &k) {
   const uint32_t a0 = (uint32_t)a, a1 = (uint32_t)(a >> 32), w0 = (uint32_t)w, w1 = (uint32_t)(w >> 32);
-  const uint64_t m00 = mad_u64(a0, w0, 0);
+  const uint64_t m00 = mad_u64(a0, w0, k.c1);
   uint64_t mid = mad_u64(a0, w1, (uint32_t)(m00 >> 32));
   if (PIN) asm GPQ_PIN_VOLATILE("" : "+v"(mid));
   mid = mad_u64(a1, w0, mid);
@@ -65,9 +72,7 @@
 #endif
 __device__ __forceinline__ uint64_t mulmod_raw(uint64_t a, uint64_t w, const PrimeK &k) { return mulmod_raw_t<false>(a, w, k); }
 
-__device__ __forceinline__ uint64_t mulmod_lazy(uint64_t a, uint64_t w, const PrimeK &k) {
-  return mulmod_raw(a, w, k) + k.c1;
-}
+__device__ __forceinline__ uint64_t mulmod_lazy(uint64_t a, uint64_t w, const PrimeK &k) { return mulmod_raw(a, w, k); }
 
 __device__ __forceinline__ uint64_t csub_by(uint64_t x, uint64_t m, uint64_t neg_m) { return x + (x >= m ? neg_m : (uint64_t)0); }
 __device__ __forceinline__ uint64_t csub1(uint64_t x, const PrimeK &k) { return csub_by(x, k.p, k.np); }
@@ -84,16 +89,16 @@
 
 __device__ __forceinline__ void ct_bfly(uint64_t &x, uint64_t &y, uint64_t w, const PrimeK &k) {
   const uint64_t t = mulmod_raw_t<GPQ_PIN_CT>(y, w, k);
-  const uint64_t xs = x + (x >= k.p4 ? k.kx1 : k.kx0);
+  const uint64_t xs = csub4(x, k);
   x = xs + t;
-  y = xs + k.ky - t;
+  y = xs + k.p4 - t;
 }
 
 __device__ __forceinline__ void gs_bfly(uint64_t &x, uint64_t &y, uint64_t w, const PrimeK &k) {
   const uint64_t v = x + y;
   const uint64_t d = x + k.p4 - y;
   x = csub4(v, k);
-  y = mulmod_raw_t<GPQ_PIN_GS>(d, w, k) + k.c1;
+  y = mulmod_raw_t<GPQ_PIN_GS>(d, w, k);
 }
 
 typedef ulonglong2 TwS;
@@ -104,10 +109,10 @@
 __device__ __forceinline__ uint64_t mulmod_split(uint64_t a, const W &w, const PrimeK &k) {
   const uint32_t al = (uint32_t)a & 0x7fffffffu;
   const uint32_t ah = __builtin_amdgcn_alignbit((uint32_t)(a >> 32), (uint32_t)a, 31);
-  uint64_t t0 = mad_u64(al, (uint32_t)w.x, 0);
+  uint64_t t0 = mad_u64(al, (uint32_t)w.x, k.kinj);
   t0 = mad_u64(ah, (uint32_t)w.y, t0);
   asm GPQ_PIN_VOLATILE("" : "+v"(t0));
-  uint64_t t1 = mad_u64(al, (uint32_t)(w.x >> 32), (uint32_t)(t0 >> 32));
+  uint64_t t1 = mad_u64(al, (uint32_t)(w.x >> 32), pack64((uint32_t)(t0 >> 32), k.one));
   asm GPQ_PIN_VOLATILE("" : "+v"(t1));
   t1 = mad_u64(ah, (uint32_t)(w.y >> 32), t1);
   const uint32_t t1lo = (uint32_t)t1, t1hi = (uint32_t)(t1 >> 32);
@@ -118,16 +123,16 @@
 
 __device__ __forceinline__ void ct_bfly(uint64_t &x, uint64_t &y, const TwS &w, const PrimeK &k) {
   const uint64_t t = mulmod_split(y, w, k);
-  const uint64_t xs = x + (x >= k.p3 ? k.kx1x : k.kx0);
+  const uint64_t xs = csub3(x, k);
   x = xs + t;
-  y = xs + k.kyx - t;
+  y = xs + k.p3 - t;
 }
 template <typename W>
 __device__ __forceinline__ void gs_bfly_split(uint64_t &x, uint64_t &y, const W &w, const PrimeK &k) {
   const uint64_t v = x + y;
   const uint64_t d = x + k.p3 - y;
   x = csub3(v, k);
-  y = mulmod_split(d, w, k) + k.c1;
+  y = mulmod_split(d, w, k);
 }
 __device__ __forceinline__ void gs_bfly(uint64_t &x, uint64_t &y, const TwS &w, const PrimeK &k) { gs_bfly_split(x, y, w, k); }
 
@@ -136,16 +141,23 @@
   const uint64_t v = x + y;
   const uint64_t d = x + k.p4 - y;
   x = CSUB ? csub4(v, k) : v;
-  y = mulmod_split(d, w, k) + k.c1;
+  y = mulmod_split(d, w, k);
 }
 __device__ __forceinline__ void gs_bfly(uint64_t &x, uint64_t &y, const TwW &w, const PrimeK &k) { gs_bfly_wide<true>(x, y, w, k); }
 
 template <bool CSUB>
 __device__ __forceinline__ void ct_bfly_wide(uint64_t &x, uint64_t &y, const TwW &w, const PrimeK &k) {
   const uint64_t t = mulmod_split(y, w, k);
-  const uint64_t xs = x + (CSUB ? (x >= k.p4 ? k.kx1 : k.kx0) : k.kx0);
+  const uint64_t xs = CSUB ? csub4(x, k) : x;
   x = xs + t;
-  y = xs + k.kys - t;
+  y = xs + k.p2 - t;
+}
+
+inline bool split_entry_fits_wide(uint64_t p, uint64_t X, uint64_t Y) {
+  const uint64_t amax = 8 * p - 1, c = p - (1ull << 59);
+  const u128 ah = amax >> 31, al = amax & 0x7fffffffu, K = ((u128)1 << 64) + 31 * c - 1;
+  const u128 top = al * X + ah * Y, below = (u128)0x7fffffffu * X + (ah - 1) * Y;
+  return (top > below ? top : below) + K < ((u128)1 << 91);
 }
 
 __device__ __forceinline__ uint64_t mulmod_canon(uint64_t a, uint64_t b, const PrimeK &k) {
diff --git a/gpqhe_amd/csrc/ntt_kernels.hpp b/gpqhe_amd/csrc/ntt_kernels.hpp
--- a/gpqhe_amd/csrc/ntt_kernels.hpp
+++ b/gpqhe_amd/csrc/ntt_kernels.hpp
@@ -92,8 +92,8 @@
 __device__ __forceinline__ void gs_last(uint64_t &x, uint64_t &y, const LastK<TwS> &t, const PrimeK &k) {
   const uint64_t s = x + y;
   const uint64_t d = x + k.p3 - y;
-  x = canon4(mulmod_split(s, t.ninv, k) + k.c1, k);
-  y = canon4(mulmod_split(d, t.winv1_ninv, k) + k.c1, k);
+  x = canon4(mulmod_split(s, t.ninv, k), k);
+  y = canon4(mulmod_split(d, t.winv1_ninv, k), k);
 }
 
 template <typename TW> struct TwTraits;
@@ -122,8 +122,8 @@
 __device__ __forceinline__ void gs_last(uint64_t &x, uint64_t &y, const LastK<TwW> &t, const PrimeK &k) {
   const uint64_t s = x + y;
   const uint64_t d = x + k.p4 - y;
-  x = csub1(mulmod_split(s, t.ninv, k) + k.c1, k);
-  y = csub1(mulmod_split(d, t.winv1_ninv, k) + k.c1, k);
+  x = csub1(mulmod_split(s, t.ninv, k), k);
+  y = csub1(mulmod_split(d, t.winv1_ninv, k), k);
 }
 template <> struct TwTraits<TwW> {
   __device__ static __forceinline__ const TwW *table(const PassArgs &a, bool inv) { return reinterpret_cast<const TwW *>(inv ? a.winvs : a.ws); }
@@ -173,7 +173,7 @@
   }
   const unsigned limb = a.limb0 + bz;
   const LimbTab &tab = a.tabs[limb];
-  const PrimeK k = tab.k;
+  const PrimeK k = pin_consts(tab.k);
   const LastK<TW> last(tab);
   const TW *__restrict__ wt = TwTraits<TW>::table(a, INV) + ((size_t)limb << logn);
   const unsigned slab = by % a.nslab, poly = by / a.nslab;
@@ -330,7 +330,7 @@
   const unsigned wave0 = (blockIdx.x * CONTIG_WAVES + (threadIdx.x >> 6)) << 10;
   const unsigned limb = a.limb0 + blockIdx.z;
   const LimbTab &tab = a.tabs[limb];
-  const PrimeK k = tab.k;
+  const PrimeK k = pin_consts(tab.k);
   const unsigned p0 = blockIdx.y * CONTIG_POLYS;
   const unsigned cnt = polys - p0 < CONTIG_POLYS ? polys - p0 : CONTIG_POLYS;
   const size_t off = (size_t)p0 * a.poly_stride + ((size_t)blockIdx.z << a.logn) + wave0;
@@ -540,7 +540,7 @@
   __shared__ uint64_t lds[CONTIG_WAVES * LANE8_LDS_PER_WAVE];
   L8 ln(lds + (threadIdx.x >> 6) * LANE8_LDS_PER_WAVE);
   const Block8 cb(a);
-  const PrimeK k = a.tabs[cb.limb].k;
+  const PrimeK k = pin_consts(a.tabs[cb.limb].k);
   const TW *__restrict__ wf = TT::table(a, false) + cb.toff, *__restrict__ wi = TT::table(a, true) + cb.toff;
   uint64_t a0[8], a1[8], b0[8], b1[8];
   Tw8<TW, LOW> tw;
@@ -596,7 +596,7 @@
   __shared__ uint64_t lds[CONTIG_WAVES * LANE8_LDS_PER_WAVE];
   L8 ln(lds + (threadIdx.x >> 6) * LANE8_LDS_PER_WAVE);
   const Block8 cb(a);
-  const PrimeK k = a.tabs[cb.limb].k;
+  const PrimeK k = pin_consts(a.tabs[cb.limb].k);
   const TW *__restrict__ wf = TT::table(a, false) + cb.toff, *__restrict__ wi = TT::table(a, true) + cb.toff;
   uint64_t a0[8], a1[8];
   Tw8<TW, LOW> tw;
@@ -645,7 +645,7 @@
   __shared__ uint64_t lds[CONTIG_WAVES * LANE8_LDS_PER_WAVE];
   L8 ln(lds + (threadIdx.x >> 6) * LANE8_LDS_PER_WAVE);
   const Block8 cb(a);
-  const PrimeK k = a.tabs[cb.limb].k;
+  const PrimeK k = pin_consts(a.tabs[cb.limb].k);
   const TW *__restrict__ wf = TT::table(a, false) + cb.toff, *__restrict__ wi = TT::table(a, true) + cb.toff;
   uint64_t x[8], y[8];
   Tw8<TW, LOW> tw;
@@ -678,7 +678,7 @@
   __shared__ uint64_t lds[CONTIG_WAVES * LANE8_LDS_PER_WAVE];
   L8 ln(lds + (threadIdx.x >> 6) * LANE8_LDS_PER_WAVE);
   const Block8 cb(a);
-  const PrimeK k = a.tabs[cb.limb].k;
+  const PrimeK k = pin_consts(a.tabs[cb.limb].k);
   const TW *__restrict__ wf = TT::table(a, false) + cb.toff, *__restrict__ wi = TT::table(a, true) + cb.toff;
   uint64_t m[8], x[8], y[8];
   Tw8<TW, LOW> tw;
@@ -717,7 +717,7 @@
 }
 
 template <typename TW, int LOW, bool TWO = true, bool NT = false>
-__global__ __launch_bounds__(CONTIG_WAVES * 64, 3) void keyswitch_mid8x2(KeyswitchArgs ka, unsigned first) {
+__global__ __launch_bounds__(CONTIG_WAVES * 64, TWO ? 4 : 3) void keyswitch_mid8x2(KeyswitchArgs ka, unsigned first) {
   using TT = TwTraits<TW>;
   using L8 = Lane8N<LOW, NT>;
   __shared__ uint64_t lds[CONTIG_WAVES * LANE8_LDS_PER_WAVE];
@@ -725,7 +725,7 @@
   L8 ln(lds + (threadIdx.x >> 6) * LANE8_LDS_PER_WAVE);
   const unsigned wave0 = (blockIdx.x * CONTIG_WAVES + (threadIdx.x >> 6)) << 9;
   const unsigned limb = a.limb0 + blockIdx.z;
-  const PrimeK k = a.tabs[limb].k;
+  const PrimeK k = pin_consts(a.tabs[limb].k);
   const size_t toff = (size_t)limb << a.logn;
   const TW *__restrict__ wf = TT::table(a, false) + toff, *__restrict__ wi = TT::table(a, true) + toff;
   const unsigned p0 = first + 2 * blockIdx.y;
@@ -797,7 +797,7 @@
 }
 
 template <typename TW, int LOW, bool TWO = true, bool NT = false>
-__global__ __launch_bounds__(CONTIG_WAVES * 64, 3) void keyswitch_rot_mid8x2(KeyswitchArgs ka, unsigned first, unsigned g) {
+__global__ __launch_bounds__(CONTIG_WAVES * 64, TWO ? 4 : 3) void keyswitch_rot_mid8x2(KeyswitchArgs ka, unsigned first, unsigned g) {
   using TT = TwTraits<TW>;
   using L8 = Lane8N<LOW, NT>;
   __shared__ uint64_t lds[CONTIG_WAVES * LANE8_LDS_PER_WAVE];
@@ -805,7 +805,7 @@
   L8 ln(lds + (threadIdx.x >> 6) * LANE8_LDS_PER_WAVE);
   const unsigned wave0 = (blockIdx.x * CONTIG_WAVES + (threadIdx.x >> 6)) << 9;
   const unsigned limb = a.limb0 + blockIdx.z;
-  const PrimeK k = a.tabs[limb].k;
+  const PrimeK k = pin_consts(a.tabs[limb].k);
   const size_t toff = (size_t)limb << a.logn;
   const TW *__restrict__ wi = TT::table(a, true) + toff;
   const unsigned p0 = first + 2 * blockIdx.y;
@@ -898,7 +898,7 @@
 }
 template <int BT, bool NT>
 __global__ __launch_bounds__(256) void gemv_mac(GemvMacArgs a) {
-  const PrimeK k = a.tabs[blockIdx.z].k;
+  const PrimeK k = pin_consts(a.tabs[blockIdx.z].k);
   const unsigned i2 = 2 * (blockIdx.y * 256 + threadIdx.x);
   if (i2 >= (1u << a.logn)) return;
   const unsigned b0 = blockIdx.x * BT, cnt = a.polys - b0 < (unsigned)BT ? a.polys - b0 : (unsigned)BT;
@@ -939,7 +939,7 @@
   L8 ln(lds + (threadIdx.x >> 6) * LANE8_LDS_PER_WAVE);
   const unsigned wave0 = (blockIdx.x * CONTIG_WAVES + (threadIdx.x >> 6)) << 9;
   const unsigned limb = a.limb0 + blockIdx.z;
-  const PrimeK k = a.tabs[limb].k;
+  const PrimeK k = pin_consts(a.tabs[limb].k);
   const unsigned p0 = blockIdx.y * CONTIG8_POLYS;
   const unsigned cnt = polys - p0 < CONTIG8_POLYS ? polys - p0 : CONTIG8_POLYS;
   const size_t off = (size_t)p0 * a.poly_stride + ((size_t)blockIdx.z << a.logn) + wave0;
@@ -992,7 +992,7 @@
 template <bool MUL>
 __global__ __launch_bounds__(256) void pointwise(PassArgs a) {
   const LimbTab &tab = a.tabs[a.limb0 + blockIdx.z];
-  const PrimeK k = tab.k;
+  const PrimeK k = pin_consts(tab.k);
   const unsigned i2 = 2 * (blockIdx.x * 256 + threadIdx.x);
   if (i2 >= (1u << a.logn)) return;
   const size_t off = (size_t)blockIdx.y * a.poly_stride + ((size_t)blockIdx.z << a.logn) + i2;
@@ -1011,7 +1011,7 @@
   using TT = TwTraits<TW>;
   __shared__ uint64_t s[1 << SMALL_MAX_LOGN];
   const LimbTab &tab = a.tabs[a.limb0 + blockIdx.z];
-  const PrimeK k = tab.k;
+  const PrimeK k = pin_consts(tab.k);
   const LastK<TW> last(tab);
   const unsigned n = 1u << a.logn;
   const TW *__restrict__ wt = TT::table(a, INV) + ((size_t)(a.limb0 + blockIdx.z) << a.logn);
@@ -1061,7 +1061,7 @@
 }
 template <bool INV>
 __device__ void ref_transform_limb(uint64_t *__restrict__ v, unsigned logn, const uint64_t *__restrict__ w, const LimbTab &tab) {
-  const PrimeK k = tab.k;
+  const PrimeK k = pin_consts(tab.k);
   const uint64_t q = k.p;
   const unsigned n = 1u << logn, half = n >> 1, T = blockDim.x;
   if (!INV) {
diff --git a/include/gpqhe_hip.h b/include/gpqhe_hip.h
--- a/include/gpqhe_hip.h
+++ b/include/gpqhe_hip.h
@@ -95,6 +95,7 @@
 int gpq_set_lazy_decompose(gpq_ctx *ctx, int on);
 int gpq_set_nt_policy(gpq_ctx *ctx, int mode);
 int gpq_debug_force_redo(gpq_ctx *ctx, unsigned every);
+int gpq_debug_split_entry_fits_wide(uint64_t p, uint64_t x, uint64_t y);
 int gpq_debug_zero_watch(gpq_ctx *ctx, int on);
 long gpq_debug_zero_flags(gpq_ctx *ctx, unsigned *before, unsigned *after, size_t capacity);
 int gpq_set_fused_tail(gpq_ctx *ctx, int on);
```

Result: faster. 7722 he_mul/s, median of 6 (+2.3%).
